# liu-wei2021/IV_INTERPOLATION

Measured on AMD Instinct MI355X. Metric: IV surfaces/sec (1M-batch, 64x16 grid), higher is better.
Workload: dtype f64

## Files before the change

### include/ivs.h

```cpp
#ifndef IVS_H
#define IVS_H

#include <stddef.h>
#include <stdint.h>

#ifdef __cplusplus
extern "C" {
#endif

#define IVS_ABI_VERSION 5

enum {
    IVS_LINEAR      = 0,
    IVS_CUBIC       = 1,
    IVS_CUBICSPLINE = 2,
    IVS_SLINEAR     = 3,
    IVS_NEAREST     = 4,
    IVS_ZERO        = 5,
    IVS_PCHIP       = 6,
    IVS_AKIMA       = 7,
    IVS_FROM_DERIVATIVES = 8,
    IVS_QUADRATIC   = 9,
    IVS_BARYCENTRIC = 10,
    IVS_KROGH       = 11,
    IVS_PAD         = 12,
    IVS_BFILL       = 13
};
#define IVS_POLY_MAX_KNOTS 32

enum {
    IVS_OK            = 0,
    IVS_EINVAL        = -22,
    IVS_ERANGE        = -34,
    IVS_ENOMEM        = -12,
    IVS_ELAUNCH       = -5
};

enum {
    IVS_ST_OK            = 0,
    IVS_ST_TOO_FEW_KNOTS = 1,
    IVS_ST_BAD_SHAPE     = 2,
    IVS_ST_ILL_CONDITIONED = 4
};

int         ivs_version(void);
const char* ivs_last_error(void);
int         ivs_device_count(void);

size_t ivs_interp1d_workspace_bytes(int64_t total_knots, int64_t n_series, int32_t n_channels);
int ivs_interp1d_batch_f64(const double* xk, const double* yk, int64_t yk_stride, const int64_t* knot_off,
                           int64_t n_series, int32_t n_channels, int64_t total_knots,
                           const double* xq, const int64_t* q_off, int64_t total_queries,
                           double* out, int64_t out_stride, int32_t* status, int32_t method,
                           void* workspace, size_t workspace_bytes, void* stream);

int ivs_interp1d_greeks_batch_f64(const double* xk, const double* yk, int64_t yk_stride, const int64_t* knot_off,
                                  int64_t n_series, int32_t n_channels, int64_t total_knots,
                                  const double* xq, const int64_t* q_off, int64_t total_queries,
                                  double* out, int64_t out_stride, int32_t* status, int32_t method,
                                  int32_t ch_iv, int32_t ch_underlying, int32_t ch_ttm,
                                  const int32_t* fill_idx, int64_t fill_stride, int32_t row_strike, int32_t row_rate,
                                  int32_t row_callput, const double* strike_src, const double* rate_src,
                                  const uint8_t* is_put_src, double* greeks, int64_t greeks_stride,
                                  void* workspace, size_t workspace_bytes, void* stream);

int ivs_ffill_index_batch(const int64_t* src_pos, const int64_t* src_off, const uint8_t* valid, int64_t valid_stride,
                          int32_t n_cols, const int64_t* q_off, int64_t n_series, int64_t total_queries,
                          int32_t* idx_out, int64_t out_stride, void* stream);

int ivs_gather_rows_f64(const double* src, int64_t src_stride, const int32_t* idx, int64_t idx_stride, const int32_t* idx_row,
                        int32_t n_cols, int64_t n, double* out, int64_t out_stride, void* stream);
int ivs_gather_rows_i32(const int32_t* src, int64_t src_stride, const int32_t* idx, int64_t idx_stride, const int32_t* idx_row,
                        int32_t n_cols, int64_t n, int32_t* out, int64_t out_stride, void* stream);

int ivs_frame_rows(const int64_t* q_off, int64_t n_series, int64_t total_queries, const int64_t* first_ns,
                   const double* chan, int64_t chan_stride, int32_t n_channels, const int32_t* sym_code,
                   const int32_t* status, const uint8_t* needs, int64_t* date_ns, uint8_t* keep, void* stream);

typedef struct ivs_frame_args {
    const int64_t* src_pos; const int64_t* src_off; const int64_t* q_off;
    int64_t n_series, total_src, total_queries;
    const double* yk; int64_t yk_stride; int32_t n_channels; int32_t method;
    double* chan_out; int64_t chan_stride; int32_t* status;
    const uint8_t* valid; int64_t valid_stride; int32_t n_valid;
    const double* fsrc; int64_t fsrc_stride; const int32_t* f_rows; int32_t n_f; double* f_out; int64_t f_stride;
    const int32_t* csrc; int64_t csrc_stride; const int32_t* c_rows; int32_t n_c; int32_t* c_out; int64_t c_stride;
    const int32_t* idx_rows; int32_t n_idx; int32_t* idx_out; int64_t idx_stride;
    const int64_t* first_ns; const uint8_t* needs; int32_t sym_col; int64_t* date_ns; uint8_t* keep;
    int32_t g_strike, g_rate, g_put; const double* strike_src; const double* rate_src; const uint8_t* put_src;
    int32_t ch_iv, ch_underlying, ch_ttm; double* greeks; int64_t greeks_stride;
} ivs_frame_args;
size_t ivs_frame_workspace_bytes(int64_t total_src, int64_t n_series, int32_t n_channels);
int ivs_frame_columns_f64(const ivs_frame_args* args , void* workspace, size_t workspace_bytes, void* stream);

enum { IVS_FLAG_FORCE_GENERIC = 1, IVS_FLAG_ONE_PASS = 2  };
#define IVS_FLAG_MAP_GROUPS(n) (((n) & 0xff) << 8)
size_t ivs_surface_workspace_bytes(int64_t B, int32_t ragged);
int ivs_surface_batch_f64(const double* K, const int64_t* k_off, int64_t k_stride, int32_t nK,
                          const double* T, int64_t t_stride, int32_t nT,
                          const double* sigma, int64_t B,
                          const double* Kq, int64_t kq_stride, int32_t mK,
                          const double* Tq, int64_t tq_stride, int32_t mT,
                          double* out, int32_t* status, int32_t method, int32_t flags,
                          void* workspace, size_t workspace_bytes, void* stream);

typedef struct ivs_snapshot_args {
    const int64_t* date_ns; const double* iv; const double* underlying; int64_t n_rows;
    const int64_t* row_off; int64_t n_contracts;
    const int32_t* cells; const double* strike; const int64_t* expiry_ns; int32_t nT, nK;
    int64_t t0_ns, n_snapshots;
    const double* moneyness; int32_t mK; double kq_empty;
    double* sigma; double* T; double* spot; int32_t* quotes; double* Kq;
} ivs_snapshot_args;
int ivs_snapshot_assemble_f64(const ivs_snapshot_args* args , void* workspace, size_t workspace_bytes, void* stream);

enum {
    IVS_SM_OK          = 0,
    IVS_SM_NO_CROSSING = 1,
    IVS_SM_AMBIGUOUS   = 2,
    IVS_SM_DEAD        = 4
};
typedef struct ivs_smile_args {
    const double* vol;
    const double* Kq; int64_t kq_stride;
    const double* Tq; int64_t tq_stride;
    const double* spot; double rate;
    const double* z;
    int32_t mK, mT, nD; int64_t B;
    double* q_vol; double* q_strike; int32_t* q_flags;
    int32_t rows_per_wave;
} ivs_smile_args;
int ivs_smile_delta_points_f64(const ivs_smile_args* args , void* workspace, size_t workspace_bytes, void* stream);

int ivs_bs_greeks_f64(const double* S, const double* K, const double* T, const double* r, const double* sigma,
                      const uint8_t* is_put, int32_t default_is_put, int64_t n, double* delta, double* gamma,
                      double* theta, double* vega, double* rho, void* stream);

int ivs_candle_aggregate_f64(const int64_t* ts_ns, const double* open, const double* high, const double* low,
                             const double* close, const double* volume, const int64_t* series_off, int64_t n_series,
                             int64_t n_rows, int64_t freq_ns, int64_t* out_ts, double* out_open, double* out_high,
                             double* out_low, double* out_close, double* out_volume, int32_t* out_count, void* stream);

size_t  ivs_bridge_workspace_bytes(int64_t total_rows);
int     ivs_mt19937_words_u32(uint32_t seed, uint32_t* words, int64_t n_words, void* stream);
int     ivs_bridge_candles_f64(const double* price, const double* volume, const int64_t* row_off, int64_t S,
                               int64_t total_rows, int32_t strategy, double base_spread_pct, double vol_factor,
                               const uint32_t* words, int64_t n_words, double* out, uint8_t* valid, int64_t* rng_tail,
                               void* workspace, size_t workspace_bytes, void* stream);

const char* ivs_last_kernel(void);

int     ivs_debug_stamps(void* device_buf, int64_t n_u64);
int64_t ivs_debug_last_grid(void);
int64_t ivs_debug_mode_offset(void);

#ifdef __cplusplus
}
#endif
#endif
```

### iv_interpolation_amd/_lib.py

```python
from __future__ import annotations

import ctypes as C
import os

LIB_PATH = os.path.join(os.path.dirname(os.path.abspath(__file__)), "libivs.so")

LINEAR, CUBIC, CUBICSPLINE, SLINEAR = 0, 1, 2, 3
ST_OK, ST_TOO_FEW_KNOTS, ST_BAD_SHAPE, ST_ILL_CONDITIONED = 0, 1, 2, 4
SM_OK, SM_NO_CROSSING, SM_AMBIGUOUS, SM_DEAD = 0, 1, 2, 4
SM_MAX_TARGETS = 16
FLAG_FORCE_GENERIC = 1
FLAG_ONE_PASS = 2


def flag_map_groups(n: int) -> int:
    return (int(n) & 0xff) << 8

ABI_VERSION = 5

NEAREST, ZERO, PCHIP, AKIMA, FROM_DERIVATIVES = 4, 5, 6, 7, 8
QUADRATIC = 9
BARYCENTRIC, KROGH = 10, 11
PAD, BFILL = 12, 13
POLY_MAX_KNOTS = 32
METHOD_CODES = {"linear": LINEAR, "index": LINEAR, "values": LINEAR,
                "cubic": CUBIC, "cubicspline": CUBICSPLINE, "slinear": SLINEAR,
                "nearest": NEAREST, "zero": ZERO, "pchip": PCHIP, "akima": AKIMA,
                "from_derivatives": FROM_DERIVATIVES, "piecewise_polynomial": FROM_DERIVATIVES, "quadratic": QUADRATIC,
                "barycentric": BARYCENTRIC, "krogh": KROGH,
                "pad": PAD, "ffill": PAD, "bfill": BFILL, "backfill": BFILL}


def method_code(name) -> int:
    if name in METHOD_CODES:
        return METHOD_CODES[name]
    if isinstance(name, str) and name.lower() in ("pad", "ffill", "bfill", "backfill"):
        return METHOD_CODES[name.lower()]
    raise KeyError(name)


class EngineUnavailable(RuntimeError):
    """libivs.so missing / not loadable / no MI355X visible.  Never swallowed by the host code."""


class EngineError(RuntimeError):
    """A C-ABI call returned a negative code."""


_p = C.c_void_p
_i64, _i32, _sz = C.c_int64, C.c_int32, C.c_size_t



class FrameArgs(C.Structure):
    _fields_ = [("src_pos", _p), ("src_off", _p), ("q_off", _p),
                ("n_series", _i64), ("total_src", _i64), ("total_queries", _i64),
                ("yk", _p), ("yk_stride", _i64), ("n_channels", _i32), ("method", _i32),
                ("chan_out", _p), ("chan_stride", _i64), ("status", _p),
                ("valid", _p), ("valid_stride", _i64), ("n_valid", _i32),
                ("fsrc", _p), ("fsrc_stride", _i64), ("f_rows", _p), ("n_f", _i32), ("f_out", _p), ("f_stride", _i64),
                ("csrc", _p), ("csrc_stride", _i64), ("c_rows", _p), ("n_c", _i32), ("c_out", _p), ("c_stride", _i64),
                ("idx_rows", _p), ("n_idx", _i32), ("idx_out", _p), ("idx_stride", _i64),
                ("first_ns", _p), ("needs", _p), ("sym_col", _i32), ("date_ns", _p), ("keep", _p),
                ("g_strike", _i32), ("g_rate", _i32), ("g_put", _i32), ("strike_src", _p), ("rate_src", _p), ("put_src", _p),
                ("ch_iv", _i32), ("ch_underlying", _i32), ("ch_ttm", _i32), ("greeks", _p), ("greeks_stride", _i64)]


class SnapshotArgs(C.Structure):
    _fields_ = [("date_ns", _p), ("iv", _p), ("underlying", _p), ("n_rows", _i64),
                ("row_off", _p), ("n_contracts", _i64),
                ("cells", _p), ("strike", _p), ("expiry_ns", _p), ("nT", _i32), ("nK", _i32),
                ("t0_ns", _i64), ("n_snapshots", _i64),
                ("moneyness", _p), ("mK", _i32), ("kq_empty", C.c_double),
                ("sigma", _p), ("T", _p), ("spot", _p), ("quotes", _p), ("Kq", _p)]


class SmileArgs(C.Structure):
    _fields_ = [("vol", _p), ("Kq", _p), ("kq_stride", _i64), ("Tq", _p), ("tq_stride", _i64),
                ("spot", _p), ("rate", C.c_double), ("z", C.POINTER(C.c_double)),
                ("mK", _i32), ("mT", _i32), ("nD", _i32), ("B", _i64),
                ("q_vol", _p), ("q_strike", _p), ("q_flags", _p), ("rows_per_wave", _i32)]


SIGNATURES = {
    "ivs_version": (C.c_int, []),
    "ivs_last_error": (C.c_char_p, []),
    "ivs_last_kernel": (C.c_char_p, []),
    "ivs_device_count": (C.c_int, []),
    "ivs_interp1d_workspace_bytes": (_sz, [_i64, _i64, _i32]),
    "ivs_interp1d_batch_f64": (C.c_int, [_p, _p, _i64, _p, _i64, _i32, _i64, _p, _p, _i64, _p, _i64, _p, _i32,
                                         _p, _sz, _p]),
    "ivs_interp1d_greeks_batch_f64": (C.c_int, [_p, _p, _i64, _p, _i64, _i32, _i64, _p, _p, _i64, _p, _i64, _p, _i32,
                                                _i32, _i32, _i32, _p, _i64, _i32, _i32, _i32, _p, _p, _p, _p, _i64,
                                                _p, _sz, _p]),
    "ivs_ffill_index_batch": (C.c_int, [_p, _p, _p, _i64, _i32, _p, _i64, _i64, _p, _i64, _p]),
    "ivs_gather_rows_f64": (C.c_int, [_p, _i64, _p, _i64, _p, _i32, _i64, _p, _i64, _p]),
    "ivs_gather_rows_i32": (C.c_int, [_p, _i64, _p, _i64, _p, _i32, _i64, _p, _i64, _p]),
    "ivs_frame_rows": (C.c_int, [_p, _i64, _i64, _p, _p, _i64, _i32, _p, _p, _p, _p, _p, _p]),
    "ivs_frame_workspace_bytes": (_sz, [_i64, _i64, _i32]),
    "ivs_frame_columns_f64": (C.c_int, [C.POINTER(FrameArgs), _p, _sz, _p]),
    "ivs_bs_greeks_f64": (C.c_int, [_p, _p, _p, _p, _p, _p, _i32, _i64, _p, _p, _p, _p, _p, _p]),
    "ivs_candle_aggregate_f64": (C.c_int, [_p] * 7 + [_i64, _i64, _i64] + [_p] * 8),
    "ivs_bridge_workspace_bytes": (C.c_size_t, [_i64]),
    "ivs_mt19937_words_u32": (C.c_int, [C.c_uint32, _p, _i64, _p]),
    "ivs_bridge_candles_f64": (C.c_int, [_p, _p, _p, _i64, _i64, _i32, C.c_double, C.c_double, _p, _i64, _p, _p, _p,
                                         _p, C.c_size_t, _p]),
    "ivs_debug_stamps": (C.c_int, [_p, _i64]),
    "ivs_debug_last_grid": (_i64, []),
    "ivs_debug_mode_offset": (_i64, []),
    "ivs_surface_workspace_bytes": (_sz, [_i64, _i32]),
    "ivs_snapshot_assemble_f64": (C.c_int, [C.POINTER(SnapshotArgs), _p, _sz, _p]),
    "ivs_smile_delta_points_f64": (C.c_int, [C.POINTER(SmileArgs), _p, _sz, _p]),
    "ivs_surface_batch_f64": (C.c_int, [_p, _p, _i64, _i32, _p, _i64, _i32, _p, _i64, _p, _i64, _i32, _p, _i64, _i32,
                                        _p, _p, _i32, _i32, _p, _sz, _p]),
}

_lib = None


def load():
    global _lib
    if _lib is not None:
        return _lib
    if not os.path.exists(LIB_PATH):
        raise EngineUnavailable(
            f"{LIB_PATH} not found: build it with `python -c 'import __graft_entry__ as g; g.build()'` "
            "(hipcc --offload-arch=gfx950). There is no CPU fallback.")
    try:
        import torch
    except ImportError:
        pass
    try:
        lib = C.CDLL(LIB_PATH)
    except OSError as e:
        raise EngineUnavailable(f"cannot load {LIB_PATH}: {e}") from e
    for name, (res, args) in SIGNATURES.items():
        try:
            fn = getattr(lib, name)
        except AttributeError as e:
            raise EngineUnavailable(f"{LIB_PATH} does not export {name}") from e
        fn.restype = res
        fn.argtypes = args
    if lib.ivs_version() != ABI_VERSION:
        raise EngineUnavailable(f"libivs.so ABI {lib.ivs_version()} != expected {ABI_VERSION}")
    _lib = lib
    return lib


def check(rc: int, what: str):
    if rc != 0:
        raise EngineError(f"{what} failed ({rc}): {load().ivs_last_error().decode()}")
```

### iv_interpolation_amd/csrc/ivs_api.hip

```cpp
#include <hip/hip_runtime.h>

#include <atomic>
#include <cstdarg>
#include <cstdio>
#include <cstring>

#include "../../include/ivs.h"
#include "ivs_bridge.hpp"
#include "ivs_candles.hpp"
#include "ivs_interp1d.hpp"
#include "ivs_frame.hpp"
#include "ivs_smile.hpp"
#include "ivs_snapshot.hpp"
#include "ivs_surface_dense.hpp"
#include "ivs_surface_dense_var2.hpp"
#include "ivs_surface_pass.hpp"
#include "ivs_surface_generic.hpp"

namespace {

thread_local char g_err[512] = "";
thread_local const char* g_last_kernel = "";
thread_local unsigned long long* g_stamp_buf = nullptr;
thread_local int64_t g_stamp_cap = 0;
thread_local int64_t g_last_grid = 0;

int fail(int code, const char* fmt, ...) {
    va_list ap;
    va_start(ap, fmt);
    vsnprintf(g_err, sizeof(g_err), fmt, ap);
    va_end(ap);
    return code;
}

int check_launch(const char* what) {
    hipError_t e = hipGetLastError();
    if (e != hipSuccess) return fail(IVS_ELAUNCH, "%s: %s", what, hipGetErrorString(e));
    return IVS_OK;
}

bool valid_method(int m) { return m >= IVS_LINEAR && m <= IVS_BFILL; }

std::atomic<int> g_cu[ivs::IVS_MAX_DEV];
void current_device(int& dev, int& cus) {
    dev = 0;
    if (hipGetDevice(&dev) != hipSuccess) { (void)hipGetLastError(); dev = 0; }
    const bool cached = dev >= 0 && dev < ivs::IVS_MAX_DEV;
    cus = cached ? g_cu[dev].load(std::memory_order_relaxed) : 0;
    if (cus <= 0) {
        int v = 0;
        if (hipDeviceGetAttribute(&v, hipDeviceAttributeMultiprocessorCount, dev) != hipSuccess) { (void)hipGetLastError(); v = 0; }
        cus = v > 0 ? v : 256;
        if (cached) g_cu[dev].store(cus, std::memory_order_relaxed);
    }
}
int num_cu() { int d, c; current_device(d, c); return c; }

}

extern "C" {

int ivs_version(void) { return IVS_ABI_VERSION; }

const char* ivs_last_error(void) { return g_err; }

const char* ivs_last_kernel(void) { return g_last_kernel; }

int ivs_debug_stamps(void* device_buf, int64_t n_u64) {
    g_stamp_buf = static_cast<unsigned long long*>(device_buf);
    g_stamp_cap = device_buf ? n_u64 : 0;
    return (int)ivs::D_NSTAMP;
}

int64_t ivs_debug_last_grid(void) { return g_last_grid; }
int64_t ivs_debug_mode_offset(void) { return (int64_t)offsetof(ivs::TqShared, mode); }

int ivs_device_count(void) {
    int n = 0;
    if (hipGetDeviceCount(&n) != hipSuccess) { (void)hipGetLastError(); return 0; }
    return n;
}

size_t ivs_interp1d_workspace_bytes(int64_t total_knots, int64_t n_series, int32_t n_channels) {
    if (total_knots < 0 || n_series < 0 || n_channels < 0) return 0;
    return ivs::interp1d_ws_bytes(total_knots, n_series, n_channels);
}

namespace {
int interp1d_impl(const char* fn, const double* xk, const double* yk, int64_t yk_stride, const int64_t* knot_off,
                  int64_t n_series, int32_t n_channels, int64_t total_knots, const double* xq, const int64_t* q_off,
                  int64_t total_queries, double* out, int64_t out_stride, int32_t* status, int32_t method, void* workspace,
                  size_t workspace_bytes, void* stream, ivs::Interp1dParams& p) {
    g_err[0] = 0;
    if (!valid_method(method)) return fail(IVS_EINVAL, "%s: unknown method %d", fn, method);
    if (n_series < 0 || n_channels < 0 || total_knots < 0 || total_queries < 0) return fail(IVS_EINVAL, "%s: negative size", fn);
    if (n_series == 0 || n_channels == 0) return IVS_OK;
    if (!knot_off || !q_off || !status) return fail(IVS_EINVAL, "%s: null offsets/status", fn);
    if (total_knots > 0 && (!xk || !yk)) return fail(IVS_EINVAL, "%s: null knots", fn);
    if (total_queries > 0 && !out) return fail(IVS_EINVAL, "%s: null out", fn);
    if (yk_stride < total_knots || out_stride < total_queries)
        return fail(IVS_EINVAL, "%s: channel stride smaller than row length", fn);
    if (n_series * (int64_t)n_channels > 0x7fffffffLL || (total_queries + 255) / 256 > 0x7fffffffLL)
        return fail(IVS_ERANGE, "%s: batch too large for one launch", fn);
    size_t need = ivs::interp1d_ws_bytes(total_knots, n_series, n_channels);
    if (!workspace || workspace_bytes < need) return fail(IVS_ENOMEM, "%s: workspace %zu < %zu bytes", fn, workspace_bytes, need);
    p.xk = xk; p.yk = yk; p.yk_stride = yk_stride; p.knot_off = knot_off;
    p.S = n_series; p.C = n_channels; p.total_knots = total_knots;
    p.xq = xq; p.q_off = q_off; p.total_q = total_queries;
    p.out = out; p.out_stride = out_stride; p.status = status; p.method = method;
    double* w = static_cast<double*>(workspace);
    size_t plane = (size_t)n_channels * (size_t)total_knots;
    p.wx = w; p.wy = w + plane; p.ws = w + 2 * plane; p.wcp = w + 3 * plane;
    p.wn = reinterpret_cast<int32_t*>(w + 4 * plane);
    hipStream_t st = static_cast<hipStream_t>(stream);
    hipLaunchKernelGGL(ivs::interp1d_prepare_kernel, dim3((unsigned)(n_series * n_channels)), dim3(256), 0, st, p);
    int rc = check_launch("interp1d_prepare_kernel");
    if (rc) return rc;
    if (total_queries > 0) {
        hipLaunchKernelGGL(ivs::interp1d_eval_kernel, dim3((unsigned)((total_queries + ivs::E1_ROWS - 1) / ivs::E1_ROWS)), dim3(256), 0, st, p);
        rc = check_launch("interp1d_eval_kernel");
    }
    return rc;
}
}

int ivs_interp1d_batch_f64(const double* xk, const double* yk, int64_t yk_stride, const int64_t* knot_off,
                           int64_t n_series, int32_t n_channels, int64_t total_knots,
                           const double* xq, const int64_t* q_off, int64_t total_queries,
                           double* out, int64_t out_stride, int32_t* status, int32_t method,
                           void* workspace, size_t workspace_bytes, void* stream) {
    ivs::Interp1dParams p{};
    p.greeks = nullptr;
    return interp1d_impl("ivs_interp1d_batch_f64", xk, yk, yk_stride, knot_off, n_series, n_channels, total_knots, xq, q_off,
                         total_queries, out, out_stride, status, method, workspace, workspace_bytes, stream, p);
}

int ivs_interp1d_greeks_batch_f64(const double* xk, const double* yk, int64_t yk_stride, const int64_t* knot_off,
                                  int64_t n_series, int32_t n_channels, int64_t total_knots,
                                  const double* xq, const int64_t* q_off, int64_t total_queries,
                                  double* out, int64_t out_stride, int32_t* status, int32_t method,
                                  int32_t ch_iv, int32_t ch_underlying, int32_t ch_ttm,
                                  const int32_t* fill_idx, int64_t fill_stride, int32_t row_strike, int32_t row_rate,
                                  int32_t row_callput, const double* strike_src, const double* rate_src,
                                  const uint8_t* is_put_src, double* greeks, int64_t greeks_stride,
                                  void* workspace, size_t workspace_bytes, void* stream) {
    const char* fn = "ivs_interp1d_greeks_batch_f64";
    g_err[0] = 0;
    if (n_series > 0 && n_channels > 0 && total_queries > 0) {
        if (!greeks || greeks_stride < total_queries) return fail(IVS_EINVAL, "%s: null / short greeks output", fn);
        if (ch_iv < 0 || ch_iv >= n_channels || ch_underlying < 0 || ch_underlying >= n_channels || ch_ttm < 0 || ch_ttm >= n_channels)
            return fail(IVS_EINVAL, "%s: channel numbers outside [0, %d)", fn, n_channels);
        if ((row_strike >= 0 || row_rate >= 0 || row_callput >= 0) && (!fill_idx || fill_stride < total_queries))
            return fail(IVS_EINVAL, "%s: null / short fill index", fn);
        if ((row_strike >= 0 && !strike_src) || (row_rate >= 0 && !rate_src) || (row_callput >= 0 && !is_put_src))
            return fail(IVS_EINVAL, "%s: a present column needs its source array", fn);
    }
    ivs::Interp1dParams p{};
    p.fidx = fill_idx; p.fidx_stride = fill_stride; p.fi_strike = row_strike; p.fi_rate = row_rate; p.fi_put = row_callput;
    p.strike_src = strike_src; p.rate_src = rate_src; p.put_src = is_put_src;
    p.ch_iv = ch_iv; p.ch_S = ch_underlying; p.ch_T = ch_ttm;
    p.greeks = greeks; p.greeks_stride = greeks_stride;
    return interp1d_impl(fn, xk, yk, yk_stride, knot_off, n_series, n_channels, total_knots, xq, q_off, total_queries, out,
                         out_stride, status, method, workspace, workspace_bytes, stream, p);
}

int ivs_ffill_index_batch(const int64_t* src_pos, const int64_t* src_off, const uint8_t* valid, int64_t valid_stride,
                          int32_t n_cols, const int64_t* q_off, int64_t n_series, int64_t total_queries,
                          int32_t* idx_out, int64_t out_stride, void* stream) {
    g_err[0] = 0;
    if (n_cols < 0 || n_series < 0 || total_queries < 0) return fail(IVS_EINVAL, "ivs_ffill_index_batch: negative size");
    if (n_cols == 0 || n_series == 0 || total_queries == 0) return IVS_OK;
    if (!src_pos || !src_off || !valid || !q_off || !idx_out) return fail(IVS_EINVAL, "ivs_ffill_index_batch: null pointer");
    if (out_stride < total_queries) return fail(IVS_EINVAL, "ivs_ffill_index_batch: out_stride < total_queries");
    if ((total_queries + 255) / 256 > 0x7fffffffLL) return fail(IVS_ERANGE, "ivs_ffill_index_batch: too many rows");
    if (valid_stride > 0x7fffffffLL) return fail(IVS_ERANGE, "ivs_ffill_index_batch: %lld source rows exceed the int32 gather index", (long long)valid_stride);
    ivs::FfillParams p{src_pos, src_off, valid, valid_stride, n_cols, q_off, n_series, total_queries, idx_out, out_stride};
    hipLaunchKernelGGL(ivs::ffill_index_kernel, dim3((unsigned)((total_queries + ivs::F1_ROWS - 1) / ivs::F1_ROWS)), dim3(256), 0,
                       static_cast<hipStream_t>(stream), p);
    return check_launch("ffill_index_kernel");
}

extern "C++" {
namespace {
template <class T>
int gather_impl(const char* fn, const void* src, int64_t src_stride, const int32_t* idx, int64_t idx_stride, const int32_t* idx_row,
                int32_t n_cols, int64_t n, void* out, int64_t out_stride, T missing, void* stream) {
    g_err[0] = 0;
    if (n_cols < 0 || n < 0) return fail(IVS_EINVAL, "%s: negative size", fn);
    if (n_cols == 0 || n == 0) return IVS_OK;
    if (!src || !idx || !idx_row || !out) return fail(IVS_EINVAL, "%s: null pointer", fn);
    if (idx_stride < n || out_stride < n) return fail(IVS_EINVAL, "%s: stride smaller than row count", fn);
    if (src_stride > 0x7fffffffLL) return fail(IVS_ERANGE, "%s: %lld source rows exceed the int32 gather index", fn, (long long)src_stride);
    ivs::GatherParams p{src, src_stride, idx, idx_stride, idx_row, n_cols, n, out, out_stride};
    int64_t blocks = (n + 255) / 256;
    const int64_t cap = (int64_t)num_cu() * 16;
    if (blocks > cap) blocks = cap;
    hipLaunchKernelGGL(ivs::gather_rows_kernel<T>, dim3((unsigned)blocks), dim3(256), 0, static_cast<hipStream_t>(stream), p, missing);
    return check_launch(fn);
}
}
}

int ivs_gather_rows_f64(const double* src, int64_t src_stride, const int32_t* idx, int64_t idx_stride, const int32_t* idx_row,
                        int32_t n_cols, int64_t n, double* out, int64_t out_stride, void* stream) {
    return gather_impl<double>("ivs_gather_rows_f64", src, src_stride, idx, idx_stride, idx_row, n_cols, n, out, out_stride,
                               __builtin_nan(""), stream);
}

int ivs_gather_rows_i32(const int32_t* src, int64_t src_stride, const int32_t* idx, int64_t idx_stride, const int32_t* idx_row,
                        int32_t n_cols, int64_t n, int32_t* out, int64_t out_stride, void* stream) {
    return gather_impl<int32_t>("ivs_gather_rows_i32", src, src_stride, idx, idx_stride, idx_row, n_cols, n, out, out_stride,
                                (int32_t)-1, stream);
}

int ivs_frame_rows(const int64_t* q_off, int64_t n_series, int64_t total_queries, const int64_t* first_ns,
                   const double* chan, int64_t chan_stride, int32_t n_channels, const int32_t* sym_code,
                   const int32_t* status, const uint8_t* needs, int64_t* date_ns, uint8_t* keep, void* stream) {
    g_err[0] = 0;
    if (n_series < 0 || total_queries < 0 || n_channels < 0) return fail(IVS_EINVAL, "ivs_frame_rows: negative size");
// ... 140 lines not shown

int ivs_smile_delta_points_f64(const ivs_smile_args* a, void* workspace, size_t workspace_bytes, void* stream) {
    const char* fn = "ivs_smile_delta_points_f64";
    (void)workspace; (void)workspace_bytes;
    g_err[0] = 0;
    g_last_kernel = "";
    if (!a) return fail(IVS_EINVAL, "%s: null args", fn);
    if (a->B < 0 || a->mT < 0 || a->mK < 0 || a->kq_stride < 0 || a->tq_stride < 0) return fail(IVS_EINVAL, "%s: negative size", fn);
    if (a->nD < 1 || a->nD > ivs::SM_MAX_D) return fail(IVS_ERANGE, "%s: nD=%d outside [1,%d]", fn, a->nD, ivs::SM_MAX_D);
    if (a->mK < 2) return fail(IVS_ERANGE, "%s: mK=%d < 2: a bracket needs two nodes", fn, a->mK);
    if (a->rows_per_wave < 0 || a->rows_per_wave > 64 / a->nD)
        return fail(IVS_ERANGE, "%s: rows_per_wave=%d outside [0,%d] for nD=%d", fn, a->rows_per_wave, 64 / a->nD, a->nD);
    if (a->B == 0 || a->mT == 0) return IVS_OK;
    if (!a->vol || !a->Kq || !a->Tq || !a->spot || !a->z || !a->q_vol || !a->q_strike || !a->q_flags)
        return fail(IVS_EINVAL, "%s: null pointer", fn);
    if ((a->kq_stride != 0 && a->kq_stride < a->mK) || (a->tq_stride != 0 && a->tq_stride < a->mT))
        return fail(IVS_EINVAL, "%s: grid stride smaller than the grid", fn);
    if (a->B > 0x7fffffffLL / a->mT)
        return fail(IVS_ERANGE, "%s: %lld x %d rows exceed one launch", fn, (long long)a->B, a->mT);
    ivs::SmileParams p{};
    p.vol = a->vol; p.Kq = a->Kq; p.Tq = a->Tq; p.spot = a->spot;
    p.kq_stride = a->kq_stride; p.tq_stride = a->tq_stride; p.rate = a->rate;
    for (int t = 0; t < a->nD; ++t) p.z[t] = a->z[t];
    p.mK = a->mK; p.mT = a->mT; p.nD = a->nD; p.rows = a->B * a->mT;
    p.q_vol = a->q_vol; p.q_strike = a->q_strike; p.q_flags = a->q_flags;
    int dev, cus;
    current_device(dev, cus);
    int64_t group = p.rows / ((int64_t)cus * 16);
    group = group < 1 ? 1 : (group > 64 / a->nD ? 64 / a->nD : group);
    if (a->rows_per_wave > 0) group = a->rows_per_wave;
    p.group = (int32_t)group;
    const int64_t waves = (p.rows + group - 1) / group;
    hipLaunchKernelGGL(ivs::smile_delta_kernel, dim3((unsigned)((waves + ivs::SM_WAVES - 1) / ivs::SM_WAVES)),
                       dim3(ivs::SM_WAVES * 64), 0, static_cast<hipStream_t>(stream), p);
    g_last_kernel = "smile_delta_kernel";
    return check_launch("smile_delta_kernel");
}

int ivs_candle_aggregate_f64(const int64_t* ts_ns, const double* open, const double* high, const double* low,
                             const double* close, const double* volume, const int64_t* series_off, int64_t n_series,
                             int64_t n_rows, int64_t freq_ns, int64_t* out_ts, double* out_open, double* out_high,
                             double* out_low, double* out_close, double* out_volume, int32_t* out_count, void* stream) {
    g_err[0] = 0;
    if (n_rows < 0 || n_series < 0 || freq_ns <= 0) return fail(IVS_EINVAL, "ivs_candle_aggregate_f64: bad size / frequency");
    if (n_rows == 0 || n_series == 0) return IVS_OK;
    if (!ts_ns || !open || !high || !low || !close || !volume || !series_off || !out_ts || !out_open || !out_high ||
        !out_low || !out_close || !out_volume || !out_count)
        return fail(IVS_EINVAL, "ivs_candle_aggregate_f64: null pointer");
    if ((n_rows + 255) / 256 > 0x7fffffffLL) return fail(IVS_ERANGE, "ivs_candle_aggregate_f64: too many rows");
    ivs::CandleParams p{ts_ns, open, high, low, close, volume, series_off, n_series, n_rows, freq_ns,
                        out_ts, out_open, out_high, out_low, out_close, out_volume, out_count};
    hipLaunchKernelGGL(ivs::candle_kernel, dim3((unsigned)((n_rows + 255) / 256)), dim3(256), 0,
                       static_cast<hipStream_t>(stream), p);
    return check_launch("candle_kernel");
}

size_t ivs_bridge_workspace_bytes(int64_t total_rows) { return ivs::bridge_ws_bytes(total_rows < 0 ? 0 : total_rows); }

int ivs_mt19937_words_u32(uint32_t seed, uint32_t* words, int64_t n_words, void* stream) {
    g_err[0] = 0;
    if (n_words < 0) return fail(IVS_EINVAL, "ivs_mt19937_words_u32: negative size");
    if (n_words == 0) return IVS_OK;
    if (!words) return fail(IVS_EINVAL, "ivs_mt19937_words_u32: null pointer");
    hipLaunchKernelGGL(ivs::mt19937_words_kernel, dim3(1), dim3(ivs::MT_THREADS), 0, static_cast<hipStream_t>(stream), seed, words, n_words);
    return check_launch("mt19937_words_kernel");
}

int ivs_bridge_candles_f64(const double* price, const double* volume, const int64_t* row_off, int64_t S,
                           int64_t total_rows, int32_t strategy, double base_spread_pct, double vol_factor,
                           const uint32_t* words, int64_t n_words, double* out, uint8_t* valid, int64_t* rng_tail,
                           void* workspace, size_t workspace_bytes, void* stream) {
    g_err[0] = 0;
    if (S < 0 || total_rows < 0 || n_words < 0) return fail(IVS_EINVAL, "ivs_bridge_candles_f64: negative size");
    if (strategy < 0 || strategy > 4) return fail(IVS_EINVAL, "ivs_bridge_candles_f64: unknown strategy %d", strategy);
    if (!rng_tail) return fail(IVS_EINVAL, "ivs_bridge_candles_f64: null rng_tail");
    hipStream_t st = static_cast<hipStream_t>(stream);
    if (S == 0 || total_rows == 0) {
        if (hipMemsetAsync(rng_tail, 0, 8, st) != hipSuccess || hipMemsetAsync(rng_tail + 3, 0, 8, st) != hipSuccess)
            return fail(IVS_ELAUNCH, "ivs_bridge_candles_f64: memset failed");
        return IVS_OK;
    }
    if (!price || !row_off || !words || !out || !valid || !workspace)
        return fail(IVS_EINVAL, "ivs_bridge_candles_f64: null pointer");
    if (workspace_bytes < ivs::bridge_ws_bytes(total_rows)) return fail(IVS_ENOMEM, "ivs_bridge_candles_f64: workspace too small");
    const int64_t nb = ivs::bridge_blocks(total_rows);
    if (nb > 0x7fffffffLL) return fail(IVS_ERANGE, "ivs_bridge_candles_f64: too many rows");
    if (n_words > 0x7fffffffLL) return fail(IVS_ERANGE, "ivs_bridge_candles_f64: %lld words exceed the int32 per-row stream offsets", (long long)n_words);
    auto align64 = [](uintptr_t a) { return (a + 63) & ~(uintptr_t)63; };
    uintptr_t w = align64(reinterpret_cast<uintptr_t>(workspace));
    ivs::BridgeParams p;
    p.price = price; p.volume = volume; p.row_off = row_off; p.S = S; p.total_rows = total_rows;
    p.strategy = strategy; p.base_spread_pct = base_spread_pct; p.vol_factor = vol_factor;
    p.words = words; p.n_words = n_words; p.out = out; p.valid = valid; p.rng_tail = rng_tail;
    p.woff = reinterpret_cast<int32_t*>(w); w = align64(w + (size_t)total_rows * 4);
    p.bbase = reinterpret_cast<int64_t*>(w); w = align64(w + (size_t)(nb + 1) * 8);
    p.gauss = reinterpret_cast<double*>(w); w = align64(w + (size_t)total_rows * 8);
    p.expu = reinterpret_cast<double*>(w); w = align64(w + (size_t)total_rows * 8);
    p.acc = reinterpret_cast<uint8_t*>(w); w = align64(w + ivs::bridge_acc_capacity(total_rows));
    p.gauss0 = reinterpret_cast<double*>(w);
    if (hipMemsetAsync(rng_tail + 3, 0, 8, st) != hipSuccess) return fail(IVS_ELAUNCH, "ivs_bridge_candles_f64: memset failed");
    if (strategy == ivs::BR_TREND) {
        int64_t nd = n_words / 2;
        const int64_t cap = (int64_t)ivs::bridge_acc_capacity(total_rows);
        if (nd > cap) { nd = cap; p.n_words = 2 * nd; }
        int64_t ab = (nd + 255) / 256;
        const int64_t abcap = (int64_t)num_cu() * 16;
        if (ab > abcap) ab = abcap;
        if (ab < 1) ab = 1;
        hipLaunchKernelGGL(ivs::bridge_accept_kernel, dim3((unsigned)ab), dim3(256), 0, st, p, nd);
        hipLaunchKernelGGL(ivs::bridge_gauss_walk_kernel, dim3(1), dim3(64), 0, st, p, nd);
    } else {
        hipLaunchKernelGGL(ivs::bridge_count_kernel, dim3((unsigned)nb), dim3(256), 0, st, p);
        hipLaunchKernelGGL(ivs::bridge_scan_blocks_kernel, dim3(1), dim3(256), 0, st, p, nb);
    }
    int64_t grid = (int64_t)num_cu() * 8;
    if (grid > S) grid = S;
    switch (strategy) {
        case ivs::BR_SPREAD: hipLaunchKernelGGL(ivs::bridge_candles_kernel<ivs::BR_SPREAD>, dim3((unsigned)grid), dim3(64), 0, st, p); break;
        case ivs::BR_MIDPOINT: hipLaunchKernelGGL(ivs::bridge_candles_kernel<ivs::BR_MIDPOINT>, dim3((unsigned)grid), dim3(64), 0, st, p); break;
        case ivs::BR_TREND: hipLaunchKernelGGL(ivs::bridge_candles_kernel<ivs::BR_TREND>, dim3((unsigned)grid), dim3(64), 0, st, p); break;
        case ivs::BR_PIPELINE: hipLaunchKernelGGL(ivs::bridge_candles_kernel<ivs::BR_PIPELINE>, dim3((unsigned)grid), dim3(64), 0, st, p); break;
        default: hipLaunchKernelGGL(ivs::bridge_candles_kernel<ivs::BR_SIMPLE>, dim3((unsigned)grid), dim3(64), 0, st, p); break;
    }
    return check_launch("bridge_candles_kernel");
}

int ivs_bs_greeks_f64(const double* S, const double* K, const double* T, const double* r, const double* sigma,
                      const uint8_t* is_put, int32_t default_is_put, int64_t n, double* delta, double* gamma,
                      double* theta, double* vega, double* rho, void* stream) {
    g_err[0] = 0;
    if (n < 0) return fail(IVS_EINVAL, "ivs_bs_greeks_f64: negative size");
    if (n == 0) return IVS_OK;
    if (!S || !K || !T || !r || !sigma || !delta || !gamma || !theta || !vega || !rho)
        return fail(IVS_EINVAL, "ivs_bs_greeks_f64: null pointer");
    ivs::GreeksParams p{S, K, T, r, sigma, is_put, default_is_put, n, delta, gamma, theta, vega, rho};
    int64_t blocks = (n + 255) / 256;
    int64_t cap = (int64_t)num_cu() * 16;
    if (blocks > cap) blocks = cap;
    hipLaunchKernelGGL(ivs::greeks_kernel, dim3((unsigned)blocks), dim3(256), 0, static_cast<hipStream_t>(stream), p);
    return check_launch("greeks_kernel");
}

size_t ivs_surface_workspace_bytes(int64_t B, int32_t ragged) { return ivs::surface_ws_bytes(B, ragged != 0); }

int ivs_surface_batch_f64(const double* K, const int64_t* k_off, int64_t k_stride, int32_t nK,
                          const double* T, int64_t t_stride, int32_t nT,
                          const double* sigma, int64_t B,
                          const double* Kq, int64_t kq_stride, int32_t mK,
                          const double* Tq, int64_t tq_stride, int32_t mT,
                          double* out, int32_t* status, int32_t method, int32_t flags,
                          void* workspace, size_t workspace_bytes, void* stream) {
    g_err[0] = 0;
    g_last_kernel = "";
    if (!valid_method(method)) return fail(IVS_EINVAL, "ivs_surface_batch_f64: unknown method %d", method);
    if (ivs::method_is_poly(method)) return fail(IVS_EINVAL, "ivs_surface_batch_f64: method %d ('barycentric' / 'krogh') is 1-D only", method);
    if (B < 0 || nK < 0 || nT < 0 || mK < 0 || mT < 0) return fail(IVS_EINVAL, "ivs_surface_batch_f64: negative size");
    if (B == 0 || mK == 0 || mT == 0) return IVS_OK;
    if (!K || !T || !sigma || !Kq || !Tq || !out) return fail(IVS_EINVAL, "ivs_surface_batch_f64: null pointer");
    if (nT < 1 || nT > ivs::GEN_NTMAX) return fail(IVS_ERANGE, "ivs_surface_batch_f64: nT=%d outside [1,%d]", nT, ivs::GEN_NTMAX);
    if (nK < 1) return fail(IVS_ERANGE, "ivs_surface_batch_f64: nK=%d < 1", nK);
    if (!k_off && k_stride != 0 && k_stride < nK) return fail(IVS_EINVAL, "ivs_surface_batch_f64: k_stride < nK");
    if (t_stride < 0 || kq_stride < 0 || tq_stride < 0 || k_stride < 0)
        return fail(IVS_EINVAL, "ivs_surface_batch_f64: negative stride");
    if (ivs::generic_lds_bytes(nK, nT, ivs::method_is_cubic(method)) > 160 * 1024)
        return fail(IVS_ERANGE, "ivs_surface_batch_f64: nK=%d x nT=%d needs %zu B of LDS (> 160 KiB)", nK, nT,
                    ivs::generic_lds_bytes(nK, nT, ivs::method_is_cubic(method)));
    const size_t need = ivs::surface_ws_bytes(B, k_off != nullptr);
    if (!workspace || workspace_bytes < need)
        return fail(IVS_ENOMEM, "ivs_surface_batch_f64: workspace %zu < %zu bytes (ivs_surface_workspace_bytes)",
                    workspace ? workspace_bytes : (size_t)0, need);
    if (reinterpret_cast<uintptr_t>(workspace) & 255)
        return fail(IVS_EINVAL, "ivs_surface_batch_f64: workspace must be 256-byte aligned");

    ivs::SurfaceParams p;
    p.K = K; p.k_off = k_off; p.k_stride = k_off ? 0 : k_stride; p.nK = nK; p.k_total = k_off ? k_stride : 0;
    p.T = T; p.t_stride = t_stride; p.nT = nT;
    p.sigma = sigma; p.B = B; p.map_groups = 1; p.tqs = nullptr; p.redo = nullptr; p.queue = nullptr; p.mode = nullptr;
    p.Kq = Kq; p.kq_stride = kq_stride; p.mK = mK;
    p.Tq = Tq; p.tq_stride = tq_stride; p.mT = mT;
    p.out = out; p.status = status; p.method = method;
    ivs::LaunchCtx cx;
    current_device(cx.dev, cx.num_cu);
    cx.st = static_cast<hipStream_t>(stream);
    cx.ws = static_cast<unsigned char*>(workspace);
    cx.ws_bytes = workspace_bytes;
    cx.map_groups = (flags >> 8) & 0xff;

    if (!(flags & IVS_FLAG_FORCE_GENERIC)) {
        const char* name = nullptr;
        int64_t need_blocks = (int64_t)cx.num_cu * 8;
        unsigned long long* dbg = (g_stamp_buf && g_stamp_cap >= need_blocks * ivs::D_NSTAMP) ? g_stamp_buf : nullptr;
        int rc = (dbg || (flags & IVS_FLAG_ONE_PASS)) ? 0 : ivs::launch_surface_pass(p, cx, &name);
        if (rc == 1) {
            g_last_kernel = name;
            return check_launch(name);
        }
        if (rc < 0) return fail(IVS_ELAUNCH, "ivs_surface_batch_f64: row-pass dispatch failed");
        rc = ivs::launch_surface_dense(p, cx, &name, dbg, &g_last_grid);
        if (rc == 1) {
            g_last_kernel = name;
            return check_launch(name);
        }
        if (rc < 0) return fail(IVS_ELAUNCH, "ivs_surface_batch_f64: dense dispatch failed");
        if (!g_stamp_buf) {
            rc = ivs::launch_surface_dense_var(p, cx, &name);
            if (rc == 1) {
                g_last_kernel = name;
                return check_launch(name);
            }
            if (rc < 0) return fail(IVS_ELAUNCH, "ivs_surface_batch_f64: dense-var dispatch failed");
        }
    }

    if (!ivs::launch_surface_generic<false>(p, cx))
        return fail(IVS_ERANGE, "ivs_surface_batch_f64: nK=%d x nT=%d needs %zu B of LDS (> 160 KiB)", nK, nT,
                    ivs::generic_lds_bytes(nK, nT, ivs::method_is_cubic(method)));
    g_last_kernel = "surface_generic_kernel";
    return check_launch("surface_generic_kernel");
}

}
```

### iv_interpolation_amd/csrc/ivs_device.hpp

```cpp
#pragma once
#include <hip/hip_runtime.h>
#include <stdint.h>

#include "../../include/ivs.h"

namespace ivs {

constexpr int WAVE = 64;

__device__ __forceinline__ double qnan() { return __builtin_nan(""); }

template <class XA>
__device__ __forceinline__ int find_interval(const XA& x, int n, double xq) {
    int lo = 0, hi = n;
    while (lo < hi) {
        int mid = (lo + hi) >> 1;
        if (x(mid) <= xq) lo = mid + 1; else hi = mid;
    }
    return lo - 1;
}

__device__ __forceinline__ double lerp_np(double xq, double x0, double y0, double x1, double y1) {
#pragma clang fp contract(off)
    if (x0 == xq) return y0;
    double slope = (y1 - y0) / (x1 - x0);
    double r = slope * (xq - x0) + y0;
    if (__builtin_isnan(r)) {
        r = slope * (xq - x1) + y1;
        if (__builtin_isnan(r) && y0 == y1) r = y0;
    }
    return r;
}

template <class XA, class YA>
__device__ __forceinline__ double eval_linear(const XA& x, const YA& y, int n, int j, double xq, bool right_hold) {
    if (j < 0) return qnan();
    if (j >= n - 1) return (right_hold || xq == x(n - 1)) ? y(n - 1) : qnan();
    return lerp_np(xq, x(j), y(j), x(j + 1), y(j + 1));
}

__device__ __forceinline__ double refined_rcp(double b) {
    double y = __builtin_amdgcn_rcp(b);
    double e = __builtin_fma(-b, y, 1.0);
    y = __builtin_fma(y, e, y);
    e = __builtin_fma(-b, y, 1.0);
    return __builtin_fma(y, e, y);
}

template <class XA, class YA, class SA>
__device__ __forceinline__ double eval_linear_slopes(const XA& x, const YA& y, const SA& slope, int n, int j, double xq,
                                                     bool right_hold) {
#pragma clang fp contract(off)
    if (j < 0) return qnan();
    if (j >= n - 1) return (right_hold || xq == x(n - 1)) ? y(n - 1) : qnan();
    const double x0 = x(j), y0 = y(j);
    if (x0 == xq) return y0;
    const double sl = slope(j);
    double r = sl * (xq - x0) + y0;
    if (__builtin_isnan(r)) {
        r = sl * (xq - x(j + 1)) + y(j + 1);
        if (__builtin_isnan(r) && y0 == y(j + 1)) r = y0;
    }
    return r;
}

__device__ __forceinline__ double hermite_eval(double x0, double x1, double y0, double y1, double s0, double s1, double xq) {
    double h = x1 - x0;
    double rh = refined_rcp(h);
    double delta = (y1 - y0) * rh;
    double t = (s0 + s1 - 2.0 * delta) * rh;
    double c0 = t * rh;
    double c1 = (delta - s0) * rh - t;
    double u = xq - x0;
    return ((c0 * u + c1) * u + s0) * u + y0;
}
template <class XA, class YA, class SA>
__device__ __forceinline__ double eval_cubic(const XA& x, const YA& y, const SA& s, int n, int j, double xq,
                                             bool extrapolate_right) {
    if (j < 0) return qnan();
    if (!extrapolate_right && !(xq <= x(n - 1))) return qnan();
    int jj = j > n - 2 ? n - 2 : j;
    return hermite_eval(x(jj), x(jj + 1), y(jj), y(jj + 1), s(jj), s(jj + 1), xq);
}

template <class XA, class YA, class SW, class CW>
__device__ __forceinline__ void nak_slopes(const XA& x, const YA& y, SW& s, CW& cp, int n) {
    if (n == 2) {
        double d = (y(1) - y(0)) / (x(1) - x(0));
        s.set(0, d); s.set(1, d);
        return;
    }
    if (n == 3) {
        double dx0 = x(1) - x(0), dx1 = x(2) - x(1);
        double d0 = (y(1) - y(0)) / dx0, d1 = (y(2) - y(1)) / dx1;
        double b0 = 2.0 * d0, b1 = 3.0 * (dx0 * d1 + dx1 * d0), b2 = 2.0 * d1;
        double s1 = (b1 - dx1 * b0 - dx0 * b2) / (2.0 * (dx0 + dx1) - dx1 - dx0);
        s.set(0, b0 - s1); s.set(1, s1); s.set(2, b2 - s1);
        return;
    }
    double xm = x(0), xc = x(1), xp = x(2);
    double ym = y(0), yc = y(1), yp = y(2);
    double dxm = xc - xm, dxc = xp - xc;
    double dlm = (yc - ym) * refined_rcp(dxm), dlc = (yp - yc) * refined_rcp(dxc);
    double d = xp - xm;
    double rhs = ((dxm + 2.0 * d) * dxc * dlm + dxm * dxm * dlc) * refined_rcp(d);
    const double rdx1 = refined_rcp(dxc);
    double cprev = d * rdx1;
    double dprev = rhs * rdx1;
    cp.set(0, cprev); s.set(0, dprev);
    for (int i = 1; i <= n - 2; ++i) {
        rhs = 3.0 * (dxc * dlm + dxm * dlc);
        const double rw = refined_rcp(2.0 * (dxm + dxc) - dxc * cprev);
        cprev = dxm * rw;
        dprev = (rhs - dxc * dprev) * rw;
        cp.set(i, cprev); s.set(i, dprev);
        if (i < n - 2) {
            xm = xc; xc = xp; xp = x(i + 2);
            ym = yc; yc = yp; yp = y(i + 2);
            dxm = dxc; dxc = xp - xc;
            dlm = dlc; dlc = (yp - yc) * refined_rcp(dxc);
        }
    }
    d = xp - xm;
    rhs = (dxc * dxc * dlm + (2.0 * d + dxc) * dxm * dlc) * refined_rcp(d);
    dprev = (rhs - d * dprev) * refined_rcp(dxm - d * cprev);
    double sn = dprev;
    s.set(n - 1, sn);
    for (int i = n - 2; i >= 0; --i) {
        sn = s(i) - cp(i) * sn;
        s.set(i, sn);
    }
}

struct View {
    double* p; int stride;
    __device__ __forceinline__ double operator()(int i) const { return p[i * stride]; }
    __device__ __forceinline__ void set(int i, double v) { p[i * stride] = v; }
};
struct CView {
    const double* p; int stride;
    __device__ __forceinline__ double operator()(int i) const { return p[i * stride]; }
};

__host__ __device__ __forceinline__ bool method_is_cubic(int m) {
    return m == IVS_CUBIC || m == IVS_CUBICSPLINE || m == IVS_PCHIP || m == IVS_AKIMA || m == IVS_QUADRATIC;
}
__device__ __forceinline__ bool method_extrapolates_right(int m) { return m == IVS_CUBICSPLINE || m == IVS_PCHIP; }
__host__ __device__ __forceinline__ bool method_is_poly(int m) { return m == IVS_BARYCENTRIC || m == IVS_KROGH; }
__device__ __forceinline__ int method_min_knots(int m) {
    switch (m) {
        case IVS_LINEAR: case IVS_PAD: case IVS_BFILL: return 0;
        case IVS_CUBIC: return 4;
        case IVS_NEAREST: case IVS_ZERO: case IVS_BARYCENTRIC: case IVS_KROGH: return 1;
        case IVS_AKIMA: return 3;
        case IVS_QUADRATIC: return 3;
        default: return 2;
    }
}

// ... 206 lines not shown
```

### iv_interpolation_amd/csrc/ivs_surface_dense.hpp

```cpp
#pragma once
#include <atomic>
#include <cstddef>
#include <cstdlib>

#include "ivs_surface_generic.hpp"

namespace ivs {

#ifndef IVS_ABLATE
#define IVS_ABLATE 0
#endif
constexpr int ABL = IVS_ABLATE;

constexpr int DK = 64, DT = 16;
constexpr int D_RS = 72;
constexpr int D_MAX_MT = 64;
constexpr unsigned long long D_SENTINEL = REDO_SENTINEL;

__device__ __forceinline__ int d_sl(int k) { return (k >> 4) * 18 + (k & 15); }

constexpr int D_WLDS_MAX_MT = 16;
__host__ __device__ inline size_t dense_lds_bytes(int mT) {
    return (size_t)(2 * DT * D_RS + 64 + 64 + 64 + (mT <= D_WLDS_MAX_MT ? 4 * D_WLDS_MAX_MT : 0)) * 8;
}
// ... 689 lines not shown
                __builtin_amdgcn_sched_barrier(0);
            }
#pragma unroll
            for (int h = 1; h >= 0; --h) {
                double cp[8];
#pragma unroll
                for (int u = 0; u < 8; ++u) cp[u] = cCP[8 * h + u];
#pragma unroll
                for (int u = 7; u >= 0; --u) { const int i = 8 * h + u; if (i <= DT - 2) s[i] = s[i] - cp[u] * s[i + 1]; }
                __builtin_amdgcn_sched_barrier(0);
            }
        } else {
            constexpr int LA = 4;
            double2 tpq[4], tac[4];
#pragma unroll
            for (int i = 0; i < LA; ++i) {
                tpq[i] = *reinterpret_cast<const double2*>(TT + i * 4);
                tac[i] = *reinterpret_cast<const double2*>(TT + i * 4 + 2);
            }
            double cpv[DT];
#pragma unroll
            for (int i = 0; i < DT; ++i) {
                const double2 pq = tpq[i & 3], ac = tac[i & 3];
                __builtin_amdgcn_sched_barrier(0);
                if (i + LA < DT) {
                    tpq[i & 3] = *reinterpret_cast<const double2*>(TT + (i + LA) * 4);
                    tac[i & 3] = *reinterpret_cast<const double2*>(TT + (i + LA) * 4 + 2);
                }
                if (!NTR) {
                    const int ia = i == 0 ? 0 : (i == DT - 1 ? DT - 3 : i - 1), ib = i == 0 ? 1 : (i == DT - 1 ? DT - 2 : i);
                    const double dA = z[ia + 1] - z[ia], dB = z[ib + 1] - z[ib];
                    prev = (pq.x * dA + pq.y * dB) - ac.x * prev;
                } else {
                    const int ia = i == 0 ? 0 : i - 1, ib = i == 0 ? 1 : (i == DT - 1 ? DT - 2 : i);
                    const double dA = z[ia + 1] - z[ia], dB = z[ib + 1] - z[ib];
                    double r = pq.x * dA + pq.y * dB;
                    if (i >= 3) r += ((i == nT - 1) ? pm_last : 0.0) * (z[i - 1] - z[i - 2]);
                    prev = r - ac.x * prev;
                }
                s[i] = prev;
                cpv[i] = ac.y;
                __builtin_amdgcn_sched_barrier(0);
            }
#pragma unroll
            for (int i = DT - 2; i >= 0; --i) s[i] = s[i] - cpv[i] * s[i + 1];
        }
        stamp(4);
#pragma unroll
        for (int jv = 0; jv < DT - 1; ++jv) {
            for (int c = 0, n = n_iv(jv); c < n; ++c, adv()) {
                if (!mine(tq)) continue;
                double a0, a1, a2, a3;
                weights(tq, a0, a1, a2, a3);
                if (QUAD) put(tq, a0 * s[jv > 0 ? jv - 1 : 0] + a1 * s[jv] + a2 * s[jv + 1] + a3 * s[jv + 2 < DT ? jv + 2 : DT - 1]);
                else put(tq, a0 * z[jv] + a1 * z[jv + 1] + a2 * s[jv] + a3 * s[jv + 1]);
            }
        }
    } else {
#pragma unroll
        for (int jv = 0; jv < DT - 1; ++jv) {
            if (!WLDS) {
#pragma clang fp contract(off)
                const int n = n_iv(jv);
                if (n == 0) continue;
                double2 tj, tr;
                if (SM) { tj = double2{cTT[jv * 4], cTT[jv * 4 + 1]}; tr = double2{cTT[jv * 4 + 2], cTT[jv * 4 + 3]}; }
                else { tj = *reinterpret_cast<const double2*>(TT + jv * 4); tr = *reinterpret_cast<const double2*>(TT + jv * 4 + 2); }
                const double a = z[jv + 1] - z[jv];
                const double q = a * tr.x;
                const double rem = __builtin_fma(-q, tr.y, a);
                const double slope = __builtin_fma(rem, tr.x, q);
                const double aa = __builtin_fabs(a);
                const bool slow_iv = !div_safe(tr.y) || !((a == 0.0) || (aa >= 0x1p-500 && aa <= 0x1p500));
                for (int c = 0; c < n; ++c, adv()) {
                    if (!mine(tq)) continue;
                    const double xt = SM ? wp[0] : readlane_f64(tt.w0, tq);
                    const double res = slope * (xt - tj.x) + z[jv];
                    const bool slow = slow_iv || __builtin_isnan(res);
                    double r = (tj.x == xt) ? z[jv] : res;
                    if (__builtin_expect(__ballot(slow) != 0ull, 0)) {
                        if (slow) r = lerp_np(xt, tj.x, z[jv], tj.y, z[jv + 1]);
                    }
                    put(tq, r);
                }
                continue;
            }
            for (int c = 0, n = n_iv(jv); c < n; ++c, adv()) {
                if (!mine(tq)) continue;
                double xt, t0, t1, rdt;
                weights(tq, xt, t0, t1, rdt);
                if (d_is_step(METHOD)) { put(tq, step_eval<METHOD>(xt, t0, t1, z[jv], z[jv + 1])); continue; }
                const double dt = t1 - t0;
                bool slow = !div_safe(dt);
                double r = lerp_fast(xt, t0, z[jv], z[jv + 1], dt, rdt, slow);
                if (__builtin_expect(__ballot(slow) != 0ull, 0)) {
                    if (slow) r = lerp_np(xt, t0, z[jv], t1, z[jv + 1]);
                }
                put(tq, r);
            }
        }
    }
    double z_last = z[DT - 1];
    if (NTR) {
#pragma unroll
        for (int i = 3; i < DT - 1; ++i) {
            z_last = (i == nT - 1) ? z[i] : z_last;
            asm volatile("" : "+v"(z_last));
        }
    }
    for (int c = 0; c < tt.n_hold; ++c, adv()) if (mine(tq)) put(tq, z_last);
    for (int c = 0; c < tt.n_nan; ++c, adv()) if (mine(tq)) put(tq, nanv);
}

template <int METHOD, bool NTR>
__global__ __launch_bounds__(64) void tq_tables_kernel(SurfaceParams p, TqShared* o) {
    __shared__ __attribute__((aligned(16))) double sm[8 * 72 + 64 + 64];
    const int lane = threadIdx.x;
    double* scratch = sm;
    double* Tsh = sm + 8 * 72;
    double* TT = Tsh + 64;
    TqTables tt;
    const bool probe = !NTR && !p.k_off && p.nK == DK && p.mK <= 64 && p.B >= 4096;
    double q[64];
    if (probe) {
#pragma unroll
        for (int s = 0; s < 64; ++s) q[s] = p.sigma[(int64_t)s * (p.B / 64) * (int64_t)(DT * DK) + (s & (DT - 1)) * DK + lane];
    }
    dense_t_phase<METHOD, false, NTR>(p.T, p.Tq, p.mT, lane, Tsh, TT, nullptr, tt, p.nT, scratch);
    if (lane < DT) {
#pragma unroll
        for (int c = 0; c < 4; ++c) o->TT[lane * 4 + c] = TT[lane * 4 + c];
        o->CP[lane] = TT[lane * 4 + 3]; o->PP[lane] = TT[lane * 4]; o->QQ[lane] = TT[lane * 4 + 1]; o->AL[lane] = TT[lane * 4 + 2];
    }
    if (lane < p.mT) { o->W[lane * 4] = tt.w0; o->W[lane * 4 + 1] = tt.w1; o->W[lane * 4 + 2] = tt.w2; o->W[lane * 4 + 3] = tt.w3; }
    int mode = 0;
    if (probe) {
        int hit = 0, tot = 0;
#pragma unroll
        for (int s = 0; s < 64; ++s) {
            const int c = __popcll(__ballot(__builtin_isnan(q[s])));
            hit += c != 0 ? 1 : 0; tot += c;
        }
        mode = (hit >= 32 || (hit >= 5 && 2 * tot <= 3 * hit)) ? 1 : 0;
    }
    if (lane == 0) {
        o->pm_last = tt.pm_last; o->iv_lo = tt.iv_lo; o->iv_hi = tt.iv_hi;
        o->n_left = tt.n_left; o->n_hold = tt.n_hold; o->n_nan = tt.n_nan; o->unsorted = tt.unsorted;
        o->redo[0] = 0; o->redo[1] = 0; o->mode = mode;
    }
    if (lane < 24) o->queue[lane * QUEUE_STRIDE] = 0ull;
}
template <bool NTR>
inline void launch_tq_tables(const SurfaceParams& p, TqShared* o, hipStream_t st) {
#define IVS_TQ_CASE(M) case M: hipLaunchKernelGGL((tq_tables_kernel<M, NTR>), dim3(1), dim3(64), 0, st, p, o); break;
    switch (p.method) {
        IVS_TQ_CASE(IVS_LINEAR) IVS_TQ_CASE(IVS_CUBIC) IVS_TQ_CASE(IVS_CUBICSPLINE) IVS_TQ_CASE(IVS_SLINEAR)
        IVS_TQ_CASE(IVS_PCHIP) IVS_TQ_CASE(IVS_AKIMA) IVS_TQ_CASE(IVS_NEAREST) IVS_TQ_CASE(IVS_ZERO) IVS_TQ_CASE(IVS_FROM_DERIVATIVES)
        IVS_TQ_CASE(IVS_QUADRATIC)
        default: break;
    }
#undef IVS_TQ_CASE
}
__device__ __forceinline__ void tq_from_shared(const void* tqs, TqTables& tt, const double*& TT, const double*& W) {
    const TqShared* g = static_cast<const TqShared*>(tqs);
    const TqShared IVS_CONST* c = (const TqShared IVS_CONST*)g;
    tt.w0 = tt.w1 = tt.w2 = tt.w3 = 0.0;
    tt.pm_last = c->pm_last; tt.iv_lo = c->iv_lo; tt.iv_hi = c->iv_hi;
    tt.n_left = c->n_left; tt.n_hold = c->n_hold; tt.n_nan = c->n_nan; tt.unsorted = c->unsorted;
    TT = g->TT; W = g->W;
}

template <int METHOD, bool TSHARED, bool WLDS, bool STAMP = false>
__global__ __launch_bounds__(64, 2) void surface_dense_kernel(SurfaceParams p, unsigned long long* dbg = nullptr) {
    if (TSHARED && p.mode && *((const int IVS_CONST*)p.mode)) return;
    constexpr bool CUB = d_is_hermite(METHOD);
    unsigned long long acc[D_NSTAMP] = {0, 0, 0, 0, 0, 0, 0, 0};
    unsigned long long tprev = 0;
    auto stamp = [&](int i) {
        if (STAMP) {
            __builtin_amdgcn_sched_barrier(0);
            unsigned long long tn = __builtin_amdgcn_s_memtime();
            __builtin_amdgcn_s_waitcnt(0xC07F);
            if (i >= 0) acc[i] += tn - tprev;
            tprev = tn;
            __builtin_amdgcn_sched_barrier(0);
        }
    };
    extern __shared__ __attribute__((aligned(16))) unsigned char smem[];
    const int lane = threadIdx.x;
    const int mT = p.mT, mK = p.mK;
    double* Y = reinterpret_cast<double*>(smem);
    double* S = Y + DT * D_RS;
    double* Ksh = S + DT * D_RS;
    double* RDX = Ksh + 64;
    double* TT = RDX + 64;
    double* W = TT + 64;
    double* Tsh = TSHARED ? Y : S;

    constexpr bool t_shared = TSHARED;
    const double nanv = __builtin_nan("");

    TqTables tt;
    auto t_phase = [&](const double* Tb, const double* Tqb) { dense_t_phase<METHOD, WLDS>(Tb, Tqb, mT, lane, Tsh, TT, W, tt); };
    const double* TTp = TT;
    const double* Wp = W;
    if (t_shared) tq_from_shared(p.tqs, tt, TTp, Wp);

    double2 pre[8];
    double pre_k;
    auto prefetch = [&](int64_t b) {
        const double2* s2 = reinterpret_cast<const double2*>(p.sigma + b * (int64_t)(DT * DK));
#pragma unroll
        for (int i = 0; i < 8; ++i) pre[i] = s2[i * 64 + lane];
        pre_k = p.K[b * p.k_stride + lane];
    };
    constexpr int XQ_REG = 4;
    double xq_reg[XQ_REG];
    auto load_xq = [&](const double* Kqb) {
#pragma unroll
        for (int i = 0; i < XQ_REG; ++i) xq_reg[i] = (i * 64 + lane < mK) ? Kqb[i * 64 + lane] : nanv;
    };
    const bool kq_shared = p.kq_stride == 0;
    if (kq_shared) load_xq(p.Kq);
    bool told = false;
    WorkQueue wq;
    wq.init(p.queue, p.map_groups, p.B, WQ_CHUNK, lane);
    int64_t b = wq.take(), b_next = b >= 0 ? wq.take() : -1;
    if (b >= 0) prefetch(b);

    while (b >= 0) {
        const bool more = b_next >= 0;
        const WorkQueue::Pending pend = wq.begin(more);
        auto advance = [&]() { const int64_t n2 = wq.finish(pend, more); b = b_next; b_next = n2; };
        __syncthreads();
        stamp(-1);
        unsigned long long bad = 0ull;
#pragma unroll
        for (int i = 0; i < 8; ++i) {
            const int t = 2 * i + (lane >> 5), k = 2 * (lane & 31);
            *reinterpret_cast<double2*>(&Y[t * D_RS + d_sl(k)]) = pre[i];
            bad |= __ballot(pre[i].x != pre[i].x) | __ballot(pre[i].y != pre[i].y);
        }
        Ksh[lane] = pre_k;
        double* outb = p.out + b * (int64_t)mT * mK;
        if (!t_shared) t_phase(p.T + b * p.t_stride, p.Tq + b * p.tq_stride);
        if (bad != 0ull || tt.unsorted) {
            if (lane == 0) { reinterpret_cast<unsigned long long*>(outb)[0] = D_SENTINEL; count_redo(p, told); }
            prefetch(more ? b_next : b);
            advance();
            continue;
        }
        __syncthreads();
        stamp(0);
        const double* Kqb = p.Kq + b * p.kq_stride;
        if (!kq_shared) load_xq(Kqb);
        {
            if (ABL != 5) prefetch(more ? b_next : b);
        }
        if (d_is_nak(METHOD) && (ABL == 1 || ABL == 6)) {
            RDX[lane] = 1.0;
            __syncthreads();
        } else if (d_is_nak(METHOD)) {
            dense_strike_slopes<STAMP>(Y, S, Ksh, RDX, lane, stamp);
            __syncthreads();
            stamp(2);
        } else if (d_is_local(METHOD)) {
            dense_strike_slopes_local<METHOD>(Y, S, Ksh, RDX, lane);
            __syncthreads();
            stamp(2);
        }
#pragma unroll 1
        for (int q0 = 0, qb = 0; q0 < mK; q0 += 64, ++qb) {
            const int q = q0 + lane;
            const bool act = q < mK;
            double xq;
            if (qb < XQ_REG) xq = qb == 0 ? xq_reg[0] : (qb == 1 ? xq_reg[1] : (qb == 2 ? xq_reg[2] : xq_reg[3]));
            else xq = act ? Kqb[q] : nanv;
            int j = 0;
#pragma unroll
            for (int m = 1; m < 8; ++m) j += (Ksh[8 * m] <= xq) ? 8 : 0;
#pragma unroll
            for (int st = 4; st >= 1; st >>= 1) if (Ksh[j + st] <= xq) j += st;
            const double xl = Ksh[DK - 1];
            const bool left = !(Ksh[0] <= xq);
            const int jj = j > DK - 2 ? DK - 2 : j;
            const double x0 = Ksh[jj], x1 = Ksh[jj + 1];
            const int o0 = d_sl(jj), o1 = d_sl(jj + 1);
            double z[DT];
            if (ABL == 2 || ABL == 6) {
#pragma unroll
                for (int r = 0; r < DT; ++r) z[r] = Y[r * D_RS + d_sl(lane)] + xq;
            } else if (CUB) {
                const bool ok = !left && ((xq <= xl) || d_extrap_right(METHOD));
                const double u = xq - x0, t = u * RDX[jj], omt = 1.0 - t;
                const double w0 = ok ? (1.0 + 2.0 * t) * omt * omt : nanv;
                const double w1 = t * t * (3.0 - 2.0 * t);
                const double w2 = u * omt * omt;
                const double w3 = u * t * (t - 1.0);
                constexpr int LA = 3;
                double g0[4], g1[4], g2[4], g3[4];
#pragma unroll
                for (int r = 0; r < LA; ++r) {
                    g0[r] = Y[r * D_RS + o0]; g1[r] = Y[r * D_RS + o1]; g2[r] = S[r * D_RS + o0]; g3[r] = S[r * D_RS + o1];
                }
#pragma unroll
                for (int r = 0; r < DT; ++r) {
                    if (r + LA < DT) {
                        const int n = r + LA;
                        g0[n & 3] = Y[n * D_RS + o0]; g1[n & 3] = Y[n * D_RS + o1];
                        g2[n & 3] = S[n * D_RS + o0]; g3[n & 3] = S[n * D_RS + o1];
                    }
                    __builtin_amdgcn_sched_barrier(0);
                    z[r] = w0 * g0[r & 3] + w1 * g1[r & 3] + w2 * g2[r & 3] + w3 * g3[r & 3];
                    __builtin_amdgcn_sched_barrier(0);
                }
            } else {
                const bool right = j >= DK - 1;
                const bool hold = right && (METHOD == IVS_LINEAR || xq == xl);
                const double dx = x1 - x0, rdx = refined_rcp(dx);
                bool slow = !div_safe(dx);
                constexpr int LA = 6;
                double g0[8], g1[8];
#pragma unroll
                for (int r = 0; r < LA; ++r) { g0[r] = Y[r * D_RS + o0]; g1[r] = Y[r * D_RS + o1]; }
#pragma unroll
                for (int r = 0; r < DT; ++r) {
                    if (r + LA < DT) { const int n = r + LA; g0[n & 7] = Y[n * D_RS + o0]; g1[n & 7] = Y[n * D_RS + o1]; }
                    __builtin_amdgcn_sched_barrier(0);
                    const double y0 = g0[r & 7], y1 = g1[r & 7];
                    double v = lerp_fast(xq, x0, y0, y1, dx, rdx, slow);
                    if (right) v = hold ? y1 : nanv;
                    if (left) v = nanv;
                    z[r] = v;
                    __builtin_amdgcn_sched_barrier(0);
                }
                if (__builtin_expect(__ballot(slow && !right && !left) != 0ull, 0)) {
                    if (slow && !right && !left) {
#pragma unroll
                        for (int r = 0; r < DT; ++r) z[r] = lerp_np(xq, x0, Y[r * D_RS + o0], x1, Y[r * D_RS + o1]);
                    }
                }
            }
            stamp(3);
            if (d_is_local(METHOD)) {
#pragma unroll
                for (int r = 0; r < DT; ++r) asm volatile("" : "+v"(z[r]));
            }
            if (act) dense_maturity_pass<METHOD, WLDS, false, false, TSHARED>(z, tt, TTp, Wp, outb, q0, lane, true, mT, mK, stamp);
            stamp(5);
        }
        if (p.status && lane == 0) p.status[b] = IVS_ST_OK;
        if (STAMP) acc[7] += 1;
        advance();
    }
    if (STAMP && dbg && lane == 0) {
#pragma unroll
        for (int i = 0; i < D_NSTAMP; ++i) dbg[(size_t)blockIdx.x * D_NSTAMP + i] = acc[i];
    }
}

struct LaunchCtx {
    int dev = 0, num_cu = 256;
    hipStream_t st = nullptr;
    unsigned char* ws = nullptr;
    size_t ws_bytes = 0;
    int map_groups = 0;
};
constexpr int IVS_MAX_DEV = 64;
constexpr size_t WS_TQ_BYTES = 8192;
constexpr size_t WS_COUNTS_BYTES = 256;
constexpr int V_NCLASS = 4;
static_assert(sizeof(TqShared) <= WS_TQ_BYTES, "TqShared must fit its workspace slot");
inline size_t surface_ws_bytes(int64_t B, bool ragged) {
    return WS_TQ_BYTES + (ragged ? WS_COUNTS_BYTES + (size_t)V_NCLASS * (size_t)(B < 0 ? 0 : B) * 16 : 0);
}

inline void ensure_max_lds(const void* fn, int slot, int dev) {
    static std::atomic<unsigned long long> done[IVS_MAX_DEV];
    const int d = (dev >= 0 && dev < IVS_MAX_DEV) ? dev : 0;
    const unsigned long long bit = 1ull << (slot & 63);
    if (dev < 0 || dev >= IVS_MAX_DEV || !(done[d].load(std::memory_order_relaxed) & bit)) {
        (void)hipFuncSetAttribute(fn, hipFuncAttributeMaxDynamicSharedMemorySize, 160 * 1024);
        done[d].fetch_or(bit, std::memory_order_relaxed);
    }
}

template <bool FILTER>
inline bool launch_surface_generic(const SurfaceParams& p, const LaunchCtx& cx) {
    if (p.nK > 65535) return false;
    const size_t lds = generic_lds_bytes(p.nK, p.nT, method_is_cubic(p.method));
    if (lds > 160 * 1024) return false;
    if (lds > 64 * 1024) ensure_max_lds(reinterpret_cast<const void*>(surface_generic_kernel<FILTER>), FILTER ? 1 : 0, cx.dev);
    int per_cu = (int)((160 * 1024) / lds);
    per_cu = per_cu < 1 ? 1 : (per_cu > 16 ? 16 : per_cu);
    int64_t grid = (int64_t)cx.num_cu * per_cu * 2;
    const int64_t work = FILTER ? (p.B + 63) / 64 : p.B;
    if (grid > work) grid = work;
    hipLaunchKernelGGL(surface_generic_kernel<FILTER>, dim3((unsigned)grid), dim3(64), lds, cx.st, p);
    return true;
}

inline int dense_map_groups(int64_t grid, int64_t B, int forced) {
    int r = forced > 0 ? forced : 8;
    if (r > 16) r = 16;
    while (r > 1 && (B < (int64_t)r * 256 || grid < r)) r >>= 1;
    return r < 1 ? 1 : r;
}

template <bool NTR>
inline bool launch_tq_or_zero_queue(SurfaceParams& p, const LaunchCtx& cx, bool tsh, bool set_mode) {
    TqShared* tq = reinterpret_cast<TqShared*>(cx.ws);
    if (tsh) {
        launch_tq_tables<NTR>(p, tq, cx.st);
        p.tqs = tq;
        p.redo = tq->redo;
        p.mode = set_mode ? &tq->mode : nullptr;
    } else {
        if (hipMemsetAsync(tq->queue, 0, sizeof(TqShared::queue), cx.st) != hipSuccess) return false;
        p.tqs = nullptr;
        p.redo = nullptr;
    }
    p.queue = tq->queue;
    return true;
}

#ifndef IVS_DIAG_MINIMAL
inline bool launch_surface_masked(const SurfaceParams& p, const LaunchCtx& cx);
inline int launch_surface_dense(const SurfaceParams& p_in, const LaunchCtx& cx, const char** name,
                                unsigned long long* dbg = nullptr, int64_t* grid_out = nullptr) {
    SurfaceParams p = p_in;
    hipStream_t st = cx.st;
    if (p.k_off || p.nK != DK || p.nT != DT) return 0;
    if (p.k_stride != 0 && p.k_stride < DK) return 0;
    if (reinterpret_cast<uintptr_t>(p.sigma) & 15) return 0;
    if (p.mT > D_MAX_MT) return 0;
    const size_t lds = dense_lds_bytes(p.mT);
    if (generic_lds_bytes(p.nK, p.nT) > 160 * 1024) return 0;
    int per_cu = (int)((160 * 1024) / lds);
    per_cu = per_cu > 8 ? 8 : per_cu;
    int64_t grid = (int64_t)cx.num_cu * per_cu;
    if (grid > p.B) grid = p.B;
    if (grid_out) *grid_out = grid;
    p.map_groups = dense_map_groups(grid, p.B, cx.map_groups);
    const bool tsh = p.t_stride == 0 && p.tq_stride == 0;
    const bool wl = p.mT <= D_WLDS_MAX_MT;
    if (!launch_tq_or_zero_queue<false>(p, cx, tsh, true)) return -1;
    if (p.map_groups > 16) p.map_groups = 16;
    if (dbg) {
        if (!tsh) return 0;
        if (p.method == IVS_CUBIC) {
            if (wl) hipLaunchKernelGGL((surface_dense_kernel<IVS_CUBIC, true, true, true>), dim3((unsigned)grid), dim3(64), lds, st, p, dbg);
            else hipLaunchKernelGGL((surface_dense_kernel<IVS_CUBIC, true, false, true>), dim3((unsigned)grid), dim3(64), lds, st, p, dbg);
        } else {
            if (wl) hipLaunchKernelGGL((surface_dense_kernel<IVS_LINEAR, true, true, true>), dim3((unsigned)grid), dim3(64), lds, st, p, dbg);
            else hipLaunchKernelGGL((surface_dense_kernel<IVS_LINEAR, true, false, true>), dim3((unsigned)grid), dim3(64), lds, st, p, dbg);
        }
        *name = "surface_dense_kernel<stamp>";
        return hipGetLastError() == hipSuccess ? 1 : -1;
    }
#define IVS_DENSE_CASE(M, NAME)                                                                            \
    case M: {                                                                                              \
        if (tsh && wl) hipLaunchKernelGGL((surface_dense_kernel<M, true, true, false>), dim3((unsigned)grid), dim3(64), lds, st, p, nullptr);        \
        else if (tsh) hipLaunchKernelGGL((surface_dense_kernel<M, true, false, false>), dim3((unsigned)grid), dim3(64), lds, st, p, nullptr);        \
        else if (wl) hipLaunchKernelGGL((surface_dense_kernel<M, false, true, false>), dim3((unsigned)grid), dim3(64), lds, st, p, nullptr);         \
        else hipLaunchKernelGGL((surface_dense_kernel<M, false, false, false>), dim3((unsigned)grid), dim3(64), lds, st, p, nullptr);                \
        *name = NAME;                                                                                      \
        break;                                                                                             \
    }
    switch (p.method) {
        IVS_DENSE_CASE(IVS_LINEAR, "surface_dense_kernel<linear>")
        IVS_DENSE_CASE(IVS_CUBIC, "surface_dense_kernel<cubic>")
        IVS_DENSE_CASE(IVS_CUBICSPLINE, "surface_dense_kernel<cubicspline>")
        IVS_DENSE_CASE(IVS_SLINEAR, "surface_dense_kernel<slinear>")
        IVS_DENSE_CASE(IVS_PCHIP, "surface_dense_kernel<pchip>")
        IVS_DENSE_CASE(IVS_AKIMA, "surface_dense_kernel<akima>")
        default: return 0;
    }
#undef IVS_DENSE_CASE
    if (hipGetLastError() != hipSuccess) return -1;
    if (launch_surface_masked(p, cx) && p.redo) ++p.redo;
    launch_surface_generic<true>(p, cx);
    return 1;
}

#endif

}
```

### iv_interpolation_amd/csrc/ivs_surface_dense_var.hpp

```cpp
#pragma once
#include "ivs_surface_dense.hpp"

namespace ivs {

constexpr int DPP_QUAD_BCAST0 = 0x00, DPP_QUAD_BCAST3 = 0xFF;

template <int NKB>
__host__ __device__ inline size_t dense_var_lds_bytes(int mT) {
    return (size_t)(2 * DT * NKB * 72 + NKB * 64 + NKB * 64 + 64 + (mT <= D_WLDS_MAX_MT ? 4 * D_WLDS_MAX_MT : 0)) * 8;
}

template <int NKB>
__device__ __forceinline__ void factor_tables_var(const double* X, int n, int lane, double* AL, double* CP, double* PP,
                                                  double* QQ, double* PM, double* PI, double* PSI, double* RDX) {
    double c00 = 1.0, c01 = 0.0, c10 = 0.0, c11 = 1.0;
    double carry_crb = 0.0, carry_rdx = 0.0, carry_rdx_prev = 0.0;
#pragma unroll
    for (int blk = 0; blk < NKB; ++blk) {
        const int ir = blk * 64 + lane;
        const bool in = ir < n;
        const int i = in ? ir : n - 1;
        const double x0 = X[i];
        const double xp = X[i + 1 < n ? i + 1 : n - 1];
        const double xpp = X[i + 2 < n ? i + 2 : n - 1];
// ... 378 lines not shown
    };

    double pre[DT * NKB], pre_k[NKB];
    int n = 0, n_next = 0;
    int64_t koff = 0, koff_next = 0;
    auto sigma_of = [&](int64_t b, int64_t ko) -> const double* {
        return p.k_off ? p.sigma + (int64_t)nT * ko : p.sigma + b * (int64_t)nT * p.nK;
    };
    auto issue_loads = [&](int64_t b, int64_t ko, int nn) {
        const double* sb = sigma_of(b, ko);
        const double* Kb = p.K + ko;
#pragma unroll
        for (int t = 0; t < DT; ++t)
#pragma unroll
            for (int blk = 0; blk < NKB; ++blk) {
                const int k = blk * 64 + lane;
                pre[t * NKB + blk] = (t < nT && k < nn) ? sb[(int64_t)t * nn + k] : 0.0;
            }
#pragma unroll
        for (int blk = 0; blk < NKB; ++blk) { const int k = blk * 64 + lane; pre_k[blk] = k < nn ? Kb[k] : inf; }
    };

    WorkQueue wq;
    wq.init(p.queue + list.qslot * 8 * QUEUE_STRIDE, 8, limit, WQ_CHUNK, lane);
    int64_t it = wq.take(), it_next = it >= 0 ? wq.take() : -1, b = 0;
    if (it >= 0) { b = at(it, n, koff); issue_loads(b, koff, n); }

    while (it >= 0) {
        const bool more = it_next >= 0;
        const WorkQueue::Pending pend = wq.begin(more);
        __syncthreads();
        unsigned long long bad = 0ull;
#pragma unroll
        for (int t = 0; t < DT; ++t)
#pragma unroll
            for (int blk = 0; blk < NKB; ++blk) {
                const double v = pre[t * NKB + blk];
                Y[t * RS + d_sl(blk * 64 + lane)] = v;
                bad |= __ballot(v != v);
            }
#pragma unroll
        for (int blk = 0; blk < NKB; ++blk) Ksh[blk * 64 + lane] = pre_k[blk];
        double* outb = p.out + b * (int64_t)mT * mK;
        const double* Kqb = p.Kq + b * p.kq_stride;
        int64_t b_next = 0;
        if (more) b_next = at(it_next, n_next, koff_next);
        if (!TSHARED) dense_t_phase<METHOD, WLDS, true>(p.T + b * p.t_stride, p.Tq + b * p.tq_stride, mT, lane, S + 600, TT, W,
                                                        tt, nT, S);
        const bool redo = bad != 0ull || tt.unsorted;
        if (redo) {
            tag(b);
        } else {
            __syncthreads();
            if (d_is_nak(METHOD)) {
                dense_strike_slopes_var<NKB>(Y, S, Ksh, RDX, n, lane);
                __syncthreads();
            } else if (d_is_local(METHOD)) {
                dense_strike_slopes_local_var<METHOD>(Y, S, Ksh, RDX, n, lane);
                __syncthreads();
            }
            if (!kq_shared) load_xq(Kqb);
        }
        if (more) issue_loads(b_next, koff_next, n_next);
        if (!redo) {
#pragma unroll 1
            for (int q0 = 0, qb = 0; q0 < mK; q0 += 64, ++qb) {
                const int q = q0 + lane;
                const bool act = q < mK;
                double xq;
                if (qb < XQ_REG) xq = qb == 0 ? xq_reg[0] : (qb == 1 ? xq_reg[1] : (qb == 2 ? xq_reg[2] : xq_reg[3]));
                else xq = act ? Kqb[q] : nanv;
                int j = 0;
#pragma unroll
                for (int m = 1; m < 8 * NKB; ++m) j += (Ksh[8 * m] <= xq) ? 8 : 0;
#pragma unroll
                for (int st = 4; st >= 1; st >>= 1) if (Ksh[j + st] <= xq) j += st;
                const double xl = Ksh[n - 1];
                const bool left = !(Ksh[0] <= xq);
                const int jj = j > n - 2 ? n - 2 : j;
                const double x0 = Ksh[jj], x1 = Ksh[jj + 1];
                const int o0 = d_sl(jj), o1 = d_sl(jj + 1);
                double z[DT];
                if (CUB) {
                    const bool ok = !left && ((xq <= xl) || d_extrap_right(METHOD));
                    const double u = xq - x0, t = u * RDX[jj], omt = 1.0 - t;
                    const double w0 = ok ? (1.0 + 2.0 * t) * omt * omt : nanv;
                    const double w1 = t * t * (3.0 - 2.0 * t);
                    const double w2 = u * omt * omt;
                    const double w3 = u * t * (t - 1.0);
                    constexpr int LA = 3;
                    double g0[4], g1[4], g2[4], g3[4];
#pragma unroll
                    for (int r = 0; r < LA; ++r) {
                        g0[r] = Y[r * RS + o0]; g1[r] = Y[r * RS + o1]; g2[r] = S[r * RS + o0]; g3[r] = S[r * RS + o1];
                    }
#pragma unroll
                    for (int r = 0; r < DT; ++r) {
                        if (r + LA < DT) {
                            const int nn = r + LA;
                            g0[nn & 3] = Y[nn * RS + o0]; g1[nn & 3] = Y[nn * RS + o1];
                            g2[nn & 3] = S[nn * RS + o0]; g3[nn & 3] = S[nn * RS + o1];
                        }
                        __builtin_amdgcn_sched_barrier(0);
                        z[r] = w0 * g0[r & 3] + w1 * g1[r & 3] + w2 * g2[r & 3] + w3 * g3[r & 3];
                        __builtin_amdgcn_sched_barrier(0);
                    }
                } else {
                    const bool right = j >= n - 1;
                    const bool hold = right && (METHOD == IVS_LINEAR || xq == xl);
                    const double dx = x1 - x0, rdx = refined_rcp(dx);
                    bool slow = !div_safe(dx);
                    constexpr int LA = 6;
                    double g0[8], g1[8];
#pragma unroll
                    for (int r = 0; r < LA; ++r) { g0[r] = Y[r * RS + o0]; g1[r] = Y[r * RS + o1]; }
#pragma unroll
                    for (int r = 0; r < DT; ++r) {
                        if (r + LA < DT) { const int nn = r + LA; g0[nn & 7] = Y[nn * RS + o0]; g1[nn & 7] = Y[nn * RS + o1]; }
                        __builtin_amdgcn_sched_barrier(0);
                        const double y0 = g0[r & 7], y1 = g1[r & 7];
                        double v = lerp_fast(xq, x0, y0, y1, dx, rdx, slow);
                        if (right) v = hold ? y1 : nanv;
                        if (left) v = nanv;
                        z[r] = v;
                        __builtin_amdgcn_sched_barrier(0);
                    }
                    if (__builtin_expect(__ballot(slow && !right && !left) != 0ull, 0)) {
                        if (slow && !right && !left) {
#pragma unroll
                            for (int r = 0; r < DT; ++r) z[r] = lerp_np(xq, x0, Y[r * RS + o0], x1, Y[r * RS + o1]);
                        }
                    }
                }
                if (d_is_local(METHOD)) {
#pragma unroll
                    for (int r = 0; r < DT; ++r) asm volatile("" : "+v"(z[r]));
                }
                if (act) dense_maturity_pass<METHOD, WLDS, false, true, TSHARED>(z, tt, TTp, Wp, outb, q0, lane, true, mT, mK, nostamp, 0, 0, nT);
            }
            if (p.status && lane == 0) p.status[b] = IVS_ST_OK;
        }
        const int64_t it_next2 = wq.finish(pend, more);
        it = it_next; it_next = it_next2; b = b_next; n = n_next; koff = koff_next;
    }
}

struct VarWork { VarList wl1, wl2; bool need1, need2; };
inline bool var_work_lists(const SurfaceParams& p, const LaunchCtx& cx, VarWork& w) {
    VarItem* lists = nullptr;
    int32_t* counts = nullptr;
    if (p.k_off) {
        counts = reinterpret_cast<int32_t*>(cx.ws + WS_TQ_BYTES);
        lists = reinterpret_cast<VarItem*>(cx.ws + WS_TQ_BYTES + WS_COUNTS_BYTES);
        if (hipMemsetAsync(counts, 0, WS_COUNTS_BYTES, cx.st) != hipSuccess) return false;
        int64_t cb = (p.B + 1023) / 1024;
        const int64_t cap = (int64_t)cx.num_cu * 8;
        if (cb > cap) cb = cap;
        hipLaunchKernelGGL(var_classify_kernel, dim3((unsigned)cb), dim3(256), 0, cx.st, p, lists, lists + p.B, counts);
    }
    w.wl1 = VarList{lists, counts, 0};
    w.wl2 = VarList{lists ? lists + p.B : nullptr, counts ? counts + 1 : nullptr, 1};
    w.need1 = p.k_off ? true : p.nK <= 64;
    w.need2 = p.nK > 64;
    return true;
}

}
```

### iv_interpolation_amd/csrc/ivs_surface_dense_var2.hpp

```cpp
#pragma once
#include <type_traits>

#include "ivs_surface_dense_var.hpp"

namespace ivs {

constexpr int V2_RS = 144;
__device__ __forceinline__ int v2_row(int t) { return t * V2_RS + 8 * (t >> 1); }
constexpr int V2_PLANE = DT * V2_RS + 64;
constexpr int V2_XCH = 64;
constexpr int X_MAT = 0;
constexpr int X_FWD = 8;
constexpr int X_BWD = 24;
constexpr int X_BAD = 40;

__host__ __device__ inline size_t dense_var2_lds_bytes(int mT) {
    return (size_t)(2 * V2_PLANE + 128 + 64 + V2_XCH + (mT <= D_WLDS_MAX_MT ? 4 * D_WLDS_MAX_MT : 0)) * 8;
}

__device__ __forceinline__ void factor_tables_var2(const double* X, int n, int lane, int w, double* AL, double* CP,
                                                   double* PP, double* QQ, double* PM, double* PI, double* PSI,
                                                   double* XCH) {
    const int ir = w * 64 + lane;
    const bool in = ir < n;
// ... 275 lines not shown
        int64_t b_next = 0;
        if (it_next < limit) b_next = at(it_next, n_next, koff_next);
        if (!TSHARED) dense_t_phase<METHOD, WLDS, true>(p.T + b * p.t_stride, p.Tq + b * p.tq_stride, mT, lane, S + 600, TT, W,
                                                        tt, nT, S);
        __syncthreads();
        const bool redo = XCH[X_BAD] != 0.0 || XCH[X_BAD + 1] != 0.0 || tt.unsorted;
        if (redo) {
            tag(b);
        } else {
            if (d_is_nak(METHOD)) {
                dense_strike_slopes_var2(Y, S, Ksh, XCH, n, lane, w);
                __syncthreads();
            } else if (d_is_local(METHOD)) {
                dense_strike_slopes_local_var2<METHOD>(Y, S, Ksh, XCH, n, lane, w);
                __syncthreads();
            }
            if (!kq_shared) load_xq(Kqb);
        }
        if (it_next < limit) issue_loads(b_next, koff_next, n_next);
        if (!redo) {
            const bool split_rows = mK <= 64;
#pragma unroll 1
            for (int q0 = 0, qb = 0; q0 < mK; q0 += 64, ++qb) {
                if (!split_rows && (qb & 1) != w) continue;
                const int q = q0 + lane;
                const bool act = q < mK;
                double xq;
                if (qb < XQ_REG) xq = qb == 0 ? xq_reg[0] : (qb == 1 ? xq_reg[1] : (qb == 2 ? xq_reg[2] : xq_reg[3]));
                else xq = act ? Kqb[q] : nanv;
                int j = 0;
#pragma unroll
                for (int m = 1; m < 16; ++m) j += (Ksh[8 * m] <= xq) ? 8 : 0;
#pragma unroll
                for (int st = 4; st >= 1; st >>= 1) if (Ksh[j + st] <= xq) j += st;
                const double xl = Ksh[n - 1];
                const bool left = !(Ksh[0] <= xq);
                const int jj = j > n - 2 ? n - 2 : j;
                const double x0 = Ksh[jj], x1 = Ksh[jj + 1];
                const int o0 = d_sl(jj), o1 = d_sl(jj + 1);
                const int r_lo = split_rows ? 8 * w : 0;
                double z[DT];
                auto strike_rows = [&](auto NR_TAG, int rbase) {
                    constexpr int NR = decltype(NR_TAG)::value;
                    const double* Yb = Y;
                    const double* Sb = S;
                    if (CUB) {
                        const bool ok = !left && ((xq <= xl) || d_extrap_right(METHOD));
                        const double u = xq - x0, t = u * refined_rcp(x1 - x0), omt = 1.0 - t;
                        const double w0 = ok ? (1.0 + 2.0 * t) * omt * omt : nanv;
                        const double w1 = t * t * (3.0 - 2.0 * t);
                        const double w2 = u * omt * omt;
                        const double w3 = u * t * (t - 1.0);
                        constexpr int LA = 3;
                        double g0[4], g1[4], g2[4], g3[4];
#pragma unroll
                        for (int r = 0; r < LA; ++r) {
                            g0[r] = Yb[v2_row(rbase + r) + o0]; g1[r] = Yb[v2_row(rbase + r) + o1]; g2[r] = Sb[v2_row(rbase + r) + o0]; g3[r] = Sb[v2_row(rbase + r) + o1];
                        }
#pragma unroll
                        for (int r = 0; r < NR; ++r) {
                            if (r + LA < NR) {
                                const int nn = r + LA;
                                g0[nn & 3] = Yb[v2_row(rbase + nn) + o0]; g1[nn & 3] = Yb[v2_row(rbase + nn) + o1];
                                g2[nn & 3] = Sb[v2_row(rbase + nn) + o0]; g3[nn & 3] = Sb[v2_row(rbase + nn) + o1];
                            }
                            __builtin_amdgcn_sched_barrier(0);
                            z[r] = w0 * g0[r & 3] + w1 * g1[r & 3] + w2 * g2[r & 3] + w3 * g3[r & 3];
                            __builtin_amdgcn_sched_barrier(0);
                        }
                    } else {
                        const bool right = j >= n - 1;
                        const bool hold = right && (METHOD == IVS_LINEAR || xq == xl);
                        const double dx = x1 - x0, rdx = refined_rcp(dx);
                        bool slow = !div_safe(dx);
                        constexpr int LA = 6;
                        double g0[8], g1[8];
#pragma unroll
                        for (int r = 0; r < LA; ++r) { g0[r] = Yb[v2_row(rbase + r) + o0]; g1[r] = Yb[v2_row(rbase + r) + o1]; }
#pragma unroll
                        for (int r = 0; r < NR; ++r) {
                            if (r + LA < NR) { const int nn = r + LA; g0[nn & 7] = Yb[v2_row(rbase + nn) + o0]; g1[nn & 7] = Yb[v2_row(rbase + nn) + o1]; }
                            __builtin_amdgcn_sched_barrier(0);
                            const double y0 = g0[r & 7], y1 = g1[r & 7];
                            double v = lerp_fast(xq, x0, y0, y1, dx, rdx, slow);
                            if (right) v = hold ? y1 : nanv;
                            if (left) v = nanv;
                            z[r] = v;
                            __builtin_amdgcn_sched_barrier(0);
                        }
                        if (__builtin_expect(__ballot(slow && !right && !left) != 0ull, 0)) {
                            if (slow && !right && !left) {
#pragma unroll
                                for (int r = 0; r < NR; ++r) z[r] = lerp_np(xq, x0, Yb[v2_row(rbase + r) + o0], x1, Yb[v2_row(rbase + r) + o1]);
                            }
                        }
                    }
                };
                if (split_rows) {
                    strike_rows(std::integral_constant<int, 8>{}, r_lo);
                    __syncthreads();
                    double* ZX = Y;
#pragma unroll
                    for (int r = 0; r < 8; ++r) ZX[(r_lo + r) * 64 + lane] = z[r];
                    __syncthreads();
#pragma unroll
                    for (int r = 0; r < DT; ++r) z[r] = ZX[r * 64 + lane];
                    if (d_is_local(METHOD)) {
#pragma unroll
                        for (int r = 0; r < DT; ++r) asm volatile("" : "+v"(z[r]));
                    }
                    const int half = (mT + 1) >> 1;
                    if (act) dense_maturity_pass<METHOD, WLDS, true, true, TSHARED>(z, tt, TTp, Wp, outb, q0, lane, true, mT, mK, nostamp,
                                                                                    w == 0 ? 0 : half, w == 0 ? half : mT, nT);
                } else {
                    strike_rows(std::integral_constant<int, DT>{}, 0);
                    if (d_is_local(METHOD)) {
#pragma unroll
                        for (int r = 0; r < DT; ++r) asm volatile("" : "+v"(z[r]));
                    }
                    if (act) dense_maturity_pass<METHOD, WLDS, false, true, TSHARED>(z, tt, TTp, Wp, outb, q0, lane, true, mT, mK, nostamp, 0, 0, nT);
                }
            }
            if (p.status && threadIdx.x == 0) p.status[b] = IVS_ST_OK;
        }
        it = it_next; b = b_next; n = n_next; koff = koff_next;
    }
}

#ifndef IVS_DIAG_MINIMAL
inline int launch_surface_dense_var(const SurfaceParams& p_in, const LaunchCtx& cx, const char** name) {
    SurfaceParams p = p_in;
    hipStream_t st = cx.st;
    if (p.nT < 4 || p.nT > DT || p.mT > D_MAX_MT) return 0;
    const bool tsh = p.t_stride == 0 && p.tq_stride == 0;
    if (p.nK < 4 || p.nK > 128) return 0;
    if (!p.k_off && p.k_stride != 0 && p.k_stride < p.nK) return 0;
    if (generic_lds_bytes(p.nK, p.nT) > 160 * 1024) return 0;
    if (!(d_is_hermite(p.method) || p.method == IVS_LINEAR || p.method == IVS_SLINEAR)) return 0;
    const bool wl = p.mT <= D_WLDS_MAX_MT;
    if (!launch_tq_or_zero_queue<true>(p, cx, tsh, false)) return -1;
    if (p.k_off && p.B > 0x7fffffffLL) return 0;
    VarWork vw;
    if (!var_work_lists(p, cx, vw)) return -1;
    auto grid_for = [&](size_t lds) {
        int per_cu = (int)((160 * 1024) / lds);
        per_cu = per_cu > 8 ? 8 : (per_cu < 1 ? 1 : per_cu);
        int64_t g = (int64_t)cx.num_cu * per_cu;
        return g > p.B ? p.B : g;
    };
#define IVS_VAR_LAUNCH1(M)                                                                                           \
    {                                                                                                                \
        const size_t lds = dense_var_lds_bytes<1>(p.mT);                                                             \
        const int64_t grid = grid_for(lds);                                                                          \
        if (wl && tsh) hipLaunchKernelGGL((surface_dense_var_kernel<M, 1, true, true>), dim3((unsigned)grid), dim3(64), lds, st, p, vw.wl1);    \
        else if (tsh) hipLaunchKernelGGL((surface_dense_var_kernel<M, 1, false, true>), dim3((unsigned)grid), dim3(64), lds, st, p, vw.wl1);    \
        else if (wl) hipLaunchKernelGGL((surface_dense_var_kernel<M, 1, true, false>), dim3((unsigned)grid), dim3(64), lds, st, p, vw.wl1);     \
        else hipLaunchKernelGGL((surface_dense_var_kernel<M, 1, false, false>), dim3((unsigned)grid), dim3(64), lds, st, p, vw.wl1);            \
    }
#define IVS_VAR_LAUNCH2(M)                                                                                           \
    {                                                                                                                \
        const size_t lds = dense_var2_lds_bytes(p.mT);                    \
        const int64_t grid = grid_for(lds);                                                                          \
        if (wl && tsh) hipLaunchKernelGGL((surface_dense_var2_kernel<M, true, true>), dim3((unsigned)grid), dim3(128), lds, st, p, vw.wl2);     \
        else if (tsh) hipLaunchKernelGGL((surface_dense_var2_kernel<M, false, true>), dim3((unsigned)grid), dim3(128), lds, st, p, vw.wl2);     \
        else if (wl) hipLaunchKernelGGL((surface_dense_var2_kernel<M, true, false>), dim3((unsigned)grid), dim3(128), lds, st, p, vw.wl2);      \
        else hipLaunchKernelGGL((surface_dense_var2_kernel<M, false, false>), dim3((unsigned)grid), dim3(128), lds, st, p, vw.wl2);             \
    }
#define IVS_VAR_CASE(M, NAME)                                                  \
    case M:                                                                    \
        if (vw.need1) IVS_VAR_LAUNCH1(M)                                        \
        if (vw.need2) IVS_VAR_LAUNCH2(M)                                        \
        *name = NAME;                                                          \
        break;
    bool known = true;
    switch (p.method) {
        IVS_VAR_CASE(IVS_LINEAR, "surface_dense_var_kernel<linear>")
        IVS_VAR_CASE(IVS_CUBIC, "surface_dense_var_kernel<cubic>")
        IVS_VAR_CASE(IVS_CUBICSPLINE, "surface_dense_var_kernel<cubicspline>")
        IVS_VAR_CASE(IVS_SLINEAR, "surface_dense_var_kernel<slinear>")
        IVS_VAR_CASE(IVS_PCHIP, "surface_dense_var_kernel<pchip>")
        IVS_VAR_CASE(IVS_AKIMA, "surface_dense_var_kernel<akima>")
        default: known = false;
    }
#undef IVS_VAR_CASE
#undef IVS_VAR_LAUNCH1
#undef IVS_VAR_LAUNCH2
    if (!known) return 0;
    const bool launched = hipGetLastError() == hipSuccess;
    if (launched) launch_surface_generic<true>(p, cx);
    return launched ? 1 : -1;
}

#endif

}
```

### iv_interpolation_amd/csrc/ivs_surface_generic.hpp

```cpp
#pragma once
#include "ivs_device.hpp"

namespace ivs {

struct SurfaceParams {
    const double* K; const int64_t* k_off; int64_t k_stride; int nK;
    int64_t k_total;
    const double* T; int64_t t_stride; int nT;
    const double* sigma; int64_t B;
    const double* Kq; int64_t kq_stride; int mK;
    const double* Tq; int64_t tq_stride; int mT;
    double* out; int32_t* status; int method;
    int map_groups;
    const void* tqs;
    unsigned long long* queue;
    const int* mode;
    int* redo;
};
constexpr int QUEUE_STRIDE = 16;

struct WorkQueue {
    unsigned long long* q; int R, g0, goff, gcur, ch, lane; int64_t region, limit, cur_i, cur_end;
    struct Pending { unsigned long long t; int g; bool need; };
    __device__ __forceinline__ void init(unsigned long long* heads, int groups, int64_t n_items, int chunk, int lane_) {
        q = heads; R = groups; limit = n_items; ch = chunk; lane = lane_;
        g0 = blockIdx.x % R; goff = 0; gcur = g0; region = (limit + R - 1) / R; cur_i = 0; cur_end = 0;
    }
    __device__ __forceinline__ unsigned long long claim(int g) const {
        unsigned long long t = 0ull;
        if (lane == 0) t = atomicAdd(q + g * QUEUE_STRIDE, 1ull);
        return t;
    }
    __device__ __forceinline__ bool resolve(unsigned long long t0, int g) {
        const unsigned lo = __builtin_amdgcn_readfirstlane((unsigned)t0), hi = __builtin_amdgcn_readfirstlane((unsigned)(t0 >> 32));
        return resolve_ticket((int64_t)(((unsigned long long)hi << 32) | lo), g);
    }
    __device__ __forceinline__ void skip_group() { ++goff; gcur = (g0 + goff) % R; }
    __device__ __forceinline__ bool resolve_ticket(int64_t t, int g) {
        int64_t gend = (int64_t)(g + 1) * region;
        gend = gend < limit ? gend : limit;
        const int64_t s0 = (int64_t)g * region + t * ch;
        if (t * ch >= region || s0 >= gend) return false;
        cur_i = s0; cur_end = s0 + ch < gend ? s0 + ch : gend;
        return true;
    }
    __device__ __forceinline__ int64_t take() {
        while (cur_i >= cur_end) {
            if (goff >= R) return -1;
            if (resolve(claim(gcur), gcur)) break;
            ++goff; gcur = (g0 + goff) % R;
        }
        return cur_i++;
    }
    __device__ __forceinline__ Pending begin(bool more) const {
        Pending pd; pd.g = gcur; pd.need = more && cur_i >= cur_end && goff < R; pd.t = pd.need ? claim(pd.g) : 0ull;
        return pd;
    }
    __device__ __forceinline__ int64_t finish(const Pending& pd, bool more) {
        if (!more) return -1;
        if (pd.need && !resolve(pd.t, pd.g)) { ++goff; gcur = (g0 + goff) % R; }
        return take();
    }
};
constexpr int WQ_CHUNK = 4;

__device__ __forceinline__ void count_redo(const SurfaceParams& p) { if (p.redo) *reinterpret_cast<volatile int*>(p.redo) = 1; }
__device__ __forceinline__ void count_redo(const SurfaceParams& p, bool& told) { if (!told) { count_redo(p); told = true; } }

constexpr int GEN_NTMAX = 32;

__host__ __device__ inline size_t generic_lds_bytes(int nKmax, int nT, bool slopes = true) {
    size_t LK = (size_t)nKmax + 1;
    size_t rows = (size_t)nT * LK;
    size_t scratch = rows > (size_t)nT * 64 ? rows : (size_t)nT * 64;
    size_t doubles = (size_t)nKmax + GEN_NTMAX
                     + rows
                     + (size_t)nT * 64;
    if (slopes) doubles += 2 * rows + scratch + (size_t)nT * 64;
    return doubles * 8 + (slopes ? 0 : ((rows * 2 + 15) & ~(size_t)15))  + (size_t)nT * 64  + GEN_NTMAX * 4 ;
}

struct RowX {
    const uint16_t* idx; const double* K;
    __device__ __forceinline__ double operator()(int i) const { return K[idx[i]]; }
};
struct ColX {
    const uint8_t* idx; const double* T;
    __device__ __forceinline__ double operator()(int i) const { return T[idx[i * 64]]; }
};

constexpr unsigned long long REDO_SENTINEL = 0x7ff8dead00000001ull;

template <bool FILTER>
__global__ __launch_bounds__(64) void surface_generic_kernel(SurfaceParams p) {
    extern __shared__ __attribute__((aligned(16))) unsigned char smem[];
    const int lane = threadIdx.x;
    const int nT = p.nT, nKmax = p.nK, LK = nKmax + 1;
    const int method = p.method;
    const bool cubic = method_is_cubic(method);
    const int minkn = method_min_knots(method);

    const size_t rows = (size_t)nT * LK;
    const size_t scratch = rows > (size_t)nT * 64 ? rows : (size_t)nT * 64;
    double* Ksh = reinterpret_cast<double*>(smem);
    double* Tsh = Ksh + nKmax;
    double* ys = Tsh + GEN_NTMAX;
    double* cz = ys + rows;
    double* xs = cz + (size_t)nT * 64;
    double* ss = xs + (cubic ? rows : 0);
    double* cps = ss + (cubic ? rows : 0);
    double* cs = cps + (cubic ? scratch : 0);
    uint16_t* xi = reinterpret_cast<uint16_t*>(cs + (cubic ? (size_t)nT * 64 : 0));
    uint8_t* ctidx = reinterpret_cast<uint8_t*>(xi) + (cubic ? 0 : ((rows * 2 + 15) & ~(size_t)15));
    int* nrow = reinterpret_cast<int*>(ctidx + (size_t)nT * 64);

    if (FILTER && p.redo && *p.redo == 0) return;
    const int64_t n_outer = FILTER ? (p.B + 63) / 64 : p.B;
    for (int64_t ob = blockIdx.x; ob < n_outer; ob += gridDim.x) {
      unsigned long long todo = 1ull;
      if (FILTER) {
          const int64_t bi = ob * 64 + lane;
          const bool tagged = bi < p.B &&
              reinterpret_cast<const unsigned long long*>(p.out + bi * (int64_t)p.mT * p.mK)[0] == REDO_SENTINEL;
          todo = __ballot(tagged);
      }
      while (todo) {
        const int bit = FILTER ? __builtin_ctzll(todo) : 0;
        todo &= todo - 1;
        const int64_t b = FILTER ? ob * 64 + bit : ob;
        int64_t koff; int nKb;
        if (p.k_off) {
            koff = p.k_off[b];
            const int64_t span = p.k_off[b + 1] - koff;
            if (span < 0 || span > nKmax || koff < 0 || (p.k_total > 0 && koff + span > p.k_total)) {
                if (p.status && lane == 0) p.status[b] = IVS_ST_BAD_SHAPE;
                continue;
            }
            nKb = (int)span;
        } else { koff = b * p.k_stride; nKb = nKmax; }
        const double* Kb = p.K + koff;
        const double* sb = p.k_off ? p.sigma + (int64_t)nT * koff : p.sigma + b * (int64_t)nT * nKmax;
        const double* Tb = p.T + b * p.t_stride;
        const double* Kqb = p.Kq + b * p.kq_stride;
        const double* Tqb = p.Tq + b * p.tq_stride;
        double* outb = p.out + b * (int64_t)p.mT * p.mK;
        int st = 0;

        __syncthreads();
        for (int k = lane; k < nKb; k += 64) Ksh[k] = Kb[k];
        if (lane < nT) Tsh[lane] = Tb[lane];
        if (lane < nT) nrow[lane] = 0;
        __syncthreads();
        for (int c0 = 0; c0 < nKb; c0 += 64) {
            const int k = c0 + lane;
            const bool in = k < nKb;
            double v[GEN_NTMAX];
            const double kx = in ? Kb[k] : 0.0;
#pragma unroll
            for (int t = 0; t < GEN_NTMAX; ++t) v[t] = (t < nT && in) ? sb[(int64_t)t * nKb + k] : qnan();
#pragma unroll
            for (int t = 0; t < GEN_NTMAX; ++t) {
                if (t < nT) {
                    const bool valid = !__builtin_isnan(v[t]);
                    const unsigned long long m = __ballot(valid);
                    const int cnt = nrow[t];
                    const int rank = cnt + __popcll(m & ((1ull << lane) - 1ull));
                    if (valid) {
                        if (cubic) xs[t * LK + rank] = kx; else xi[t * LK + rank] = (uint16_t)k;
                        ys[t * LK + rank] = v[t];
// ... 80 lines not shown
```

### iv_interpolation_amd/csrc/ivs_surface_masked.hpp

```cpp
#pragma once
#include "ivs_surface_dense.hpp"

namespace ivs {

constexpr int MK_RS = 66;
__host__ __device__ constexpr size_t masked_lds_bytes() { return (size_t)(DT * MK_RS + DK) * 8 + 2 * DT * DK + DT * 4; }

struct MaskedT { const double* T; const uint8_t* idx; __device__ __forceinline__ double operator()(int i) const { return T[idx[i]]; } };
constexpr int MK_MAXCOL = 8;
struct MaskedX { const double* Ksh; const uint8_t* idx; __device__ __forceinline__ double operator()(int i) const { return Ksh[idx[i]]; } };

template <int METHOD>
__global__ __launch_bounds__(64, 3) void surface_masked_kernel(SurfaceParams p) {
    constexpr bool STEP = d_is_step(METHOD);
    static_assert(METHOD == IVS_LINEAR || METHOD == IVS_SLINEAR || METHOD == IVS_NEAREST || METHOD == IVS_ZERO || METHOD == IVS_FROM_DERIVATIVES,
                  "linear, slinear, nearest, zero, from_derivatives (the other dense methods: surface_masked_pass_kernel)");
    constexpr int MINROW = 2;
    extern __shared__ __attribute__((aligned(16))) unsigned char smem[];
    const int lane = threadIdx.x;
    const int mT = p.mT, mK = p.mK;
    double* YC = reinterpret_cast<double*>(smem);
    double* Ksh = YC + DT * MK_RS;
    uint8_t* IDX = reinterpret_cast<uint8_t*>(Ksh + DK);
    uint8_t* RANK = IDX + DT * DK;
    int* NROW = reinterpret_cast<int*>(RANK + DT * DK);
    const double nanv = __builtin_nan("");
    auto nostamp = [](int) {};

    TqTables tt;
    const double* TTp = nullptr;
    const double* Wp = nullptr;
    tq_from_shared(p.tqs, tt, TTp, Wp);

    const bool kq_shared = p.kq_stride == 0;
    const bool act = lane < mK;
    double xq = (kq_shared && act) ? p.Kq[lane] : nanv;
    const unsigned long long lt_mask = (1ull << lane) - 1ull, le_mask = lt_mask | (1ull << lane);

    const bool all = p.mode && *p.mode != 0;
    if (!all && p.redo && *p.redo == 0) return;
    bool told = false;
    double* tag_at = nullptr;
    auto leave = [&]() {
        if (lane == 0) {
            if (all) reinterpret_cast<unsigned long long*>(tag_at)[0] = REDO_SENTINEL;
            if (p.redo && !told) { *reinterpret_cast<volatile int*>(p.redo + 1) = 1; told = true; }
        }
    };
    const int64_t n_outer = (p.B + 63) / 64;
    WorkQueue wq;
    wq.init(p.queue + 16 * QUEUE_STRIDE, 1, n_outer, 1, lane);
    for (int64_t ob = p.queue ? wq.take() : (int64_t)blockIdx.x; ob >= 0 && ob < n_outer; ob = p.queue ? wq.take() : ob + gridDim.x) {
      const int64_t bi = ob * 64 + lane;
      const bool tagged = bi < p.B &&
          (all || reinterpret_cast<const unsigned long long*>(p.out + bi * (int64_t)mT * mK)[0] == REDO_SENTINEL);
      unsigned long long todo = __ballot(tagged);
      double vn[DT], kn = 0.0;
      auto request = [&](int64_t bb) {
          const double* sb = p.sigma + bb * (int64_t)(DT * DK);
#pragma unroll
          for (int t = 0; t < DT; ++t) vn[t] = sb[t * DK + lane];
          kn = p.K[bb * p.k_stride + lane];
      };
      if (todo) request(ob * 64 + __builtin_ctzll(todo));
      while (todo) {
        const int bit = __builtin_ctzll(todo);
        todo &= todo - 1;
        const int64_t b = ob * 64 + bit;
        double* outb = p.out + b * (int64_t)mT * mK;
        tag_at = outb;
        double v[DT];
#pragma unroll
        for (int t = 0; t < DT; ++t) v[t] = vn[t];
        const double kx = kn;
        if (!kq_shared) xq = act ? p.Kq[b * p.kq_stride + lane] : nanv;
        if (todo) request(ob * 64 + __builtin_ctzll(todo));
        __syncthreads();
        Ksh[lane] = kx;
        bool give_up = tt.unsorted != 0;
#pragma unroll
        for (int t = 0; t < DT; ++t) {
            const bool valid = !__builtin_isnan(v[t]);
            const unsigned long long m = __ballot(valid);
            give_up = give_up || __ballot(__builtin_isinf(v[t])) != 0ull;
            const int rank = __popcll(m & lt_mask);
            if (valid) { YC[t * MK_RS + rank] = v[t]; IDX[t * DK + rank] = (uint8_t)lane; }
            RANK[t * DK + lane] = (uint8_t)__popcll(m & le_mask);
            const int nt = __popcll(m);
            if (lane == 0) NROW[t] = nt;
            give_up = give_up || nt < MINROW;
        }
        if (give_up) { leave(); continue; }
        __syncthreads();
        __syncthreads();
        int jf = -1;
        if (Ksh[0] <= xq) {
            jf = 0;
#pragma unroll
            for (int m = 1; m < 8; ++m) jf += (Ksh[8 * m] <= xq) ? 8 : 0;
#pragma unroll
            for (int st = 4; st >= 1; st >>= 1) if (Ksh[jf + st] <= xq) jf += st;
        }
        double z[DT];
        bool all_ok = true;
#pragma unroll
        for (int t = 0; t < DT; ++t) {
            const int n = NROW[t];
            const int j = jf >= 0 ? (int)RANK[t * DK + jf] - 1 : -1;
            const MaskedX X{Ksh, IDX + t * DK};
            const CView Y{YC + t * MK_RS, 1};
            if (METHOD == IVS_NEAREST) {
                double r = nanv;
                if (j >= 0 && xq <= X(n - 1)) {
                    const int jj = j > n - 2 ? n - 2 : j;
                    r = j > n - 2 ? Y(n - 1) : step_eval<IVS_NEAREST>(xq, X(jj), X(jj + 1), Y(jj), Y(jj + 1));
                }
                z[t] = r;
            } else if (STEP) z[t] = eval_method(METHOD, X, Y, Y, n, j, xq);
            else z[t] = eval_linear(X, Y, n, j, xq, METHOD == IVS_LINEAR);
            all_ok = all_ok && !__builtin_isnan(z[t]);
        }
        const bool col_masked = act && !all_ok;
        const unsigned long long mm = __ballot(col_masked);
        if (mm != 0ull) {
            if (__popcll(mm) > MK_MAXCOL) { leave(); continue; }
            __syncthreads();
            double* Tsh = Ksh;
            double* cz = YC;
            uint8_t* cti = IDX;
            if (lane < DT) Tsh[lane] = p.T[lane];
            const int slot = __popcll(mm & lt_mask);
            int cn = 0;
            if (col_masked) {
#pragma unroll
                for (int t = 0; t < DT; ++t)
                    if (!__builtin_isnan(z[t])) { cz[slot * DT + cn] = z[t]; cti[slot * DT + cn] = (uint8_t)t; ++cn; }
            }
            if (__ballot(col_masked && cn > 0 && cn < method_min_knots(METHOD)) != 0ull) { leave(); continue; }
            __syncthreads();
            if (col_masked) {
                const MaskedT cx{Tsh, cti + slot * DT};
                const CView cy{cz + slot * DT, 1};
                int jc = -1;
                for (int tq = 0; tq < mT; ++tq) {
                    const double x = p.Tq[tq];
                    double r = nanv;
                    if (cn > 0) {
                        while (jc + 1 < cn && cx(jc + 1) <= x) ++jc;
                        r = eval_method(METHOD, cx, cy, cy, cn, jc, x);
                    }
                    outb[(int64_t)tq * mK + lane] = r;
                }
            }
        }
        if (act && all_ok) dense_maturity_pass<METHOD, true, false, false, true>(z, tt, TTp, Wp, outb, 0, lane, true, mT, mK, nostamp);
        if (p.status && lane == 0) p.status[b] = IVS_ST_OK;
      }
    }
}

}
#include "ivs_surface_masked_pass.hpp"
namespace ivs {

#ifndef IVS_DIAG_MINIMAL
inline bool launch_surface_masked(const SurfaceParams& p, const LaunchCtx& cx) {
    if (p.k_off || p.nK != DK || p.nT != DT || p.mK > 64 || p.mT > D_MAX_MT) return false;
    if (p.t_stride != 0 || p.tq_stride != 0 || !p.tqs) return false;
    int64_t grid = (int64_t)cx.num_cu * 12;
    const int64_t work = (p.B + 63) / 64;
    if (grid > work) grid = work;
    switch (p.method) {
#define IVS_MASKED_CASE(KERNEL, LDS, M) case M: hipLaunchKernelGGL((KERNEL<M>), dim3((unsigned)grid), dim3(64), LDS, cx.st, p); break;
        IVS_MASKED_CASE(surface_masked_kernel, masked_lds_bytes(), IVS_LINEAR)
        IVS_MASKED_CASE(surface_masked_kernel, masked_lds_bytes(), IVS_SLINEAR)
        IVS_MASKED_CASE(surface_masked_kernel, masked_lds_bytes(), IVS_NEAREST)
        IVS_MASKED_CASE(surface_masked_kernel, masked_lds_bytes(), IVS_ZERO)
        IVS_MASKED_CASE(surface_masked_kernel, masked_lds_bytes(), IVS_FROM_DERIVATIVES)
        IVS_MASKED_CASE(surface_masked_pass_kernel, masked_pass_lds_bytes(), IVS_CUBIC)
        IVS_MASKED_CASE(surface_masked_pass_kernel, masked_pass_lds_bytes(), IVS_CUBICSPLINE)
        IVS_MASKED_CASE(surface_masked_pass_kernel, masked_pass_lds_bytes(), IVS_QUADRATIC)
        IVS_MASKED_CASE(surface_masked_pass_kernel, masked_pass_lds_bytes(), IVS_PCHIP)
        IVS_MASKED_CASE(surface_masked_pass_kernel, masked_pass_lds_bytes(), IVS_AKIMA)
#undef IVS_MASKED_CASE
        default: return false;
    }
    return true;
}
#endif

}
```

### iv_interpolation_amd/csrc/ivs_surface_masked_pass.hpp

```cpp
#pragma once
#include "ivs_surface_masked.hpp"

namespace ivs {

constexpr int MP_ROWS = 8;
__host__ __device__ constexpr size_t masked_pass_lds_bytes() { return (size_t)(2 * MP_ROWS * MK_RS + DK) * 8 + 2 * MP_ROWS * DK + DT * 4; }

template <bool QUAD = false>
__device__ __forceinline__ void masked_solve8(const double* YC, double* XS, const int* NROW, int lane) {
    const int r = lane >> 3, seg = lane & 7, i0 = seg * 8;
    const int n = NROW[r];
    double* xr = XS + r * MK_RS;
    const double* yr = YC + r * MK_RS;
    auto cl = [&](int i) { return i < 0 ? 0 : (i > n - 1 ? n - 1 : i); };
    double xa = xr[cl(i0 - 2)], xb = xr[cl(i0 - 1)], xc = xr[cl(i0)], xd = xr[cl(i0 + 1)], xe = xr[cl(i0 + 2)];
    double ya = yr[cl(i0 - 2)], yb = yr[cl(i0 - 1)], yc = yr[cl(i0)], yd = yr[cl(i0 + 1)], ye = yr[cl(i0 + 2)];
    double dx0 = xb - xa, dx1 = xc - xb, dx2 = xd - xc, dx3 = xe - xd;
    double dl0 = (yb - ya) * refined_rcp(dx0), dl1 = (yc - yb) * refined_rcp(dx1), dl2 = (yd - yc) * refined_rcp(dx2),
           dl3 = (ye - yd) * refined_rcp(dx3);
    double xl = xe, yl = ye;
    double u[8], l[8], rh[8];
    double m00 = 1.0, m01 = 0.0, m10 = 0.0, m11 = 1.0;
    double uF = 0.0, lF = 0.0, rF = 0.0, uL = 0.0, lL = 0.0, rL = 0.0;
    int kl = -1;
// ... 34 lines not shown
        double uu = c * rb, ll = a * rb, hh = rr * rb;
        if (!QUAD) {
            if (k == 0) { const bool first = seg == 0; uu = first ? uF : uu; ll = first ? lF : ll; hh = first ? rF : hh; }
            const bool last = k == kl;
            uu = last ? uL : uu; ll = last ? lL : ll; hh = last ? rL : hh;
        }
        u[k] = in ? uu : 0.0; l[k] = in ? ll : 0.0; rh[k] = in ? hh : 0.0;
        const double n00 = u[k] * m10, n01 = u[k] * m11, n10 = m10 - l[k] * m00, n11 = m11 - l[k] * m01;
        m00 = n00; m01 = n01; m10 = n10; m11 = n11;
        if (k < 7) {
            const int j = cl(i + 3);
            const double xn = xr[j], yn = yr[j];
            dx0 = dx1; dx1 = dx2; dx2 = dx3; dx3 = xn - xl;
            dl0 = dl1; dl1 = dl2; dl2 = dl3; dl3 = (yn - yl) * refined_rcp(dx3);
            xl = xn; yl = yn;
            if (QUAD) { qa = qb; qb = qc; qc = qd; qd = qe; qe = xn; qy0 = qy1; qy1 = qy2; qy2 = yn; }
        }
    }
#define IVS_MP_MAT_STEP(SH)                                                                                   \
    {                                                                                                         \
        const double e = dpp_f64<DPP_ROW_SHR(SH)>(1.0, m00), f = dpp_f64<DPP_ROW_SHR(SH)>(0.0, m01);          \
        const double g = dpp_f64<DPP_ROW_SHR(SH)>(0.0, m10), h = dpp_f64<DPP_ROW_SHR(SH)>(1.0, m11);          \
        const bool has = seg >= SH;                                                                           \
        const double n00 = m00 * e + m01 * g, n01 = m00 * f + m01 * h, n10 = m10 * e + m11 * g, n11 = m10 * f + m11 * h; \
        m00 = has ? n00 : m00; m01 = has ? n01 : m01; m10 = has ? n10 : m10; m11 = has ? n11 : m11;           \
    }
    IVS_MP_MAT_STEP(1) IVS_MP_MAT_STEP(2) IVS_MP_MAT_STEP(4)
#undef IVS_MP_MAT_STEP
    const double pin = dpp_f64<DPP_ROW_SHR(1)>(0.0, m01), qin = dpp_f64<DPP_ROW_SHR(1)>(1.0, m11);
    double cprev = seg == 0 ? 0.0 : pin * refined_rcp(qin);
    double dprev = 0.0, prod = 1.0;
#pragma unroll
    for (int k = 0; k < 8; ++k) {
        const double rw = refined_rcp(1.0 - l[k] * cprev);
        cprev = u[k] * rw;
        const double al = l[k] * rw;
        dprev = rh[k] * rw - al * dprev;
        prod *= -al;
        u[k] = cprev; rh[k] = dprev; l[k] = prod;
    }
    {
        double A = prod, B = dprev;
#define IVS_MP_AFF_STEP(SH)                                                                                   \
        { const double a_ = dpp_f64<DPP_ROW_SHR(SH)>(1.0, A), b_ = dpp_f64<DPP_ROW_SHR(SH)>(0.0, B);          \
          const bool has = seg >= SH; B = has ? __builtin_fma(A, b_, B) : B; A = has ? A * a_ : A; }
        IVS_MP_AFF_STEP(1) IVS_MP_AFF_STEP(2) IVS_MP_AFF_STEP(4)
#undef IVS_MP_AFF_STEP
        double din = dpp_f64<DPP_ROW_SHR(1)>(0.0, B);
        din = seg == 0 ? 0.0 : din;
#pragma unroll
        for (int k = 0; k < 8; ++k) rh[k] = __builtin_fma(l[k], din, rh[k]);
    }
    double nxt = 0.0;
    prod = 1.0;
#pragma unroll
    for (int k = 7; k >= 0; --k) {
        nxt = rh[k] - u[k] * nxt;
        prod *= -u[k];
        rh[k] = nxt; l[k] = prod;
    }
    {
        double A = prod, B = nxt;
#define IVS_MP_AFF_STEP(SH)                                                                                   \
        { const double a_ = dpp_f64<DPP_ROW_SHL(SH)>(1.0, A), b_ = dpp_f64<DPP_ROW_SHL(SH)>(0.0, B);          \
          const bool has = seg + SH <= 7; B = has ? __builtin_fma(A, b_, B) : B; A = has ? A * a_ : A; }
        IVS_MP_AFF_STEP(1) IVS_MP_AFF_STEP(2) IVS_MP_AFF_STEP(4)
#undef IVS_MP_AFF_STEP
        double sin_ = dpp_f64<DPP_ROW_SHL(1)>(0.0, B);
        sin_ = seg == 7 ? 0.0 : sin_;
#pragma unroll
        for (int k = 0; k < 8; ++k) rh[k] = __builtin_fma(l[k], sin_, rh[k]);
    }
    __builtin_amdgcn_wave_barrier();
#pragma unroll
    for (int k = 0; k < 8; ++k) if (i0 + k < n) xr[i0 + k] = rh[k];
}

template <int METHOD>
__device__ __forceinline__ void masked_local8(const double* YC, double* XS, const int* NROW, int lane) {
    constexpr bool AK = METHOD == IVS_AKIMA;
    const int r = lane >> 3, seg = lane & 7, i0 = seg * 8;
    const int n = NROW[r];
    double* xr = XS + r * MK_RS;
    const double* yr = YC + r * MK_RS;
    auto cl = [&](int i) { return i < 0 ? 0 : (i > n - 1 ? n - 1 : i); };
    double F[11], DX[11];
    {
        double xa = xr[cl(i0 - 2)], ya = yr[cl(i0 - 2)];
#pragma unroll
        for (int i = 0; i < 11; ++i) {
            const int idx = i0 - 2 + i;
            const double xb = xr[cl(idx + 1)], yb = yr[cl(idx + 1)];
            const bool in = idx >= 0 && idx <= n - 2;
            const double dx = xb - xa;
            DX[i] = in ? dx : 0.0;
            F[i] = in ? (yb - ya) * refined_rcp(dx) : 0.0;
            xa = xb; ya = yb;
        }
    }
    double d[8];
    if (AK) {
        const double x3 = xr[n - 3], x2 = xr[n - 2], x1 = xr[n - 1], y3 = yr[n - 3], y2 = yr[n - 2], y1 = yr[n - 1];
        const double mL1 = (y1 - y2) * refined_rcp(x1 - x2), mL2 = (y2 - y3) * refined_rcp(x2 - x3);
        const double en1 = 2.0 * mL1 - mL2, en = 2.0 * en1 - mL1;
        const double m0 = (yr[1] - yr[0]) * refined_rcp(xr[1] - xr[0]), m1 = (yr[2] - yr[1]) * refined_rcp(xr[2] - xr[1]);
        const double em1 = 2.0 * m0 - m1, em2 = 2.0 * em1 - m0;
#pragma unroll
        for (int i = 0; i < 11; ++i) {
            const int idx = i0 - 2 + i;
            F[i] = idx == -1 ? em1 : (idx == -2 ? em2 : (idx == n - 1 ? en1 : (idx == n ? en : F[i])));
        }
        double fmax = 0.0;
#pragma unroll
        for (int k = 0; k < 8; ++k) {
            const double f = akima_f12(F[k], F[k + 1], F[k + 2], F[k + 3]);
            fmax = (i0 + k < n) ? __builtin_fmax(fmax, f) : fmax;
        }
        fmax = __builtin_fmax(fmax, dpp_f64<DPP_QUAD_SWAP1>(fmax, fmax));
        fmax = __builtin_fmax(fmax, dpp_f64<DPP_QUAD_SWAP2>(fmax, fmax));
        fmax = __builtin_fmax(fmax, dpp_f64<0x141>(fmax, fmax));
        const double thr = 1e-9 * fmax;
#pragma unroll
        for (int k = 0; k < 8; ++k) d[k] = akima_knot(F[k], F[k + 1], F[k + 2], F[k + 3], thr);
    } else {
        double e_last = 0.0, m_only = 0.0;
        {
            const int a3 = n >= 3 ? n - 3 : 0, a2 = n >= 3 ? n - 2 : 0, a1 = n - 1;
            const double x3 = xr[a3], x2 = xr[a2], x1 = xr[a1], y3 = yr[a3], y2 = yr[a2], y1 = yr[a1];
            const double h0 = x1 - x2, h1 = x2 - x3;
            const double mp = (y1 - y2) * refined_rcp(h0), mpp = (y2 - y3) * refined_rcp(h1);
            const double rs = refined_rcp(h0 + h1);
            e_last = pchip_edge(mp, mpp, (2.0 * h0 + h1) * rs, h0 * rs);
            m_only = (yr[n - 1] - yr[0]) * refined_rcp(xr[n - 1] - xr[0]);
        }
#pragma unroll
        for (int k = 0; k < 8; ++k) {
            const int i = i0 + k;
            double v = pchip_knot(F[k + 1], F[k + 2], 2.0 * DX[k + 2] + DX[k + 1], DX[k + 2] + 2.0 * DX[k + 1]);
            if (k == 0) {
                const double h0 = DX[2], h1 = DX[3], rs = refined_rcp(h0 + h1);
                const double e = pchip_edge(F[2], F[3], (2.0 * h0 + h1) * rs, h0 * rs);
                v = seg == 0 ? e : v;
            }
            v = i == n - 1 ? e_last : v;
            d[k] = n == 2 ? m_only : v;
        }
    }
    __builtin_amdgcn_wave_barrier();
#pragma unroll
    for (int k = 0; k < 8; ++k) if (i0 + k < n) xr[i0 + k] = d[k];
}

template <int METHOD>
__global__ __launch_bounds__(64, 3) void surface_masked_pass_kernel(SurfaceParams p) {
    static_assert(METHOD == IVS_CUBIC || METHOD == IVS_CUBICSPLINE || METHOD == IVS_QUADRATIC || d_is_local(METHOD), "tridiagonal and local-slope methods");
    constexpr bool QUAD = METHOD == IVS_QUADRATIC;
    constexpr bool LOCAL = d_is_local(METHOD);
    constexpr int MINROW = LOCAL ? (METHOD == IVS_AKIMA ? 3 : 2) : (QUAD ? 3 : 4);
    extern __shared__ __attribute__((aligned(16))) unsigned char smem[];
    const int lane = threadIdx.x;
    const int mT = p.mT, mK = p.mK;
    double* YC = reinterpret_cast<double*>(smem);
    double* XS = YC + MP_ROWS * MK_RS;
    double* Ksh = XS + MP_ROWS * MK_RS;
    uint8_t* IDX = reinterpret_cast<uint8_t*>(Ksh + DK);
    uint8_t* RANK = IDX + MP_ROWS * DK;
    int* NROW = reinterpret_cast<int*>(RANK + MP_ROWS * DK);
    const double nanv = __builtin_nan("");
    auto nostamp = [](int) {};

    TqTables tt;
    const double* TTp = nullptr;
    const double* Wp = nullptr;
    tq_from_shared(p.tqs, tt, TTp, Wp);

    const bool kq_shared = p.kq_stride == 0;
    const bool act = lane < mK;
    double xq = (kq_shared && act) ? p.Kq[lane] : nanv;
    const unsigned long long lt_mask = (1ull << lane) - 1ull, le_mask = lt_mask | (1ull << lane);

    const bool all = p.mode && *p.mode != 0;
    if (!all && p.redo && *p.redo == 0) return;
    bool told = false;
    double* tag_at = nullptr;
    auto leave = [&]() {
        if (lane == 0) {
            if (all) reinterpret_cast<unsigned long long*>(tag_at)[0] = REDO_SENTINEL;
            if (p.redo && !told) { *reinterpret_cast<volatile int*>(p.redo + 1) = 1; told = true; }
        }
    };
    const int64_t n_outer = (p.B + 63) / 64;
    WorkQueue wq;
    wq.init(p.queue + 16 * QUEUE_STRIDE, 1, n_outer, 1, lane);
    for (int64_t ob = p.queue ? wq.take() : (int64_t)blockIdx.x; ob >= 0 && ob < n_outer; ob = p.queue ? wq.take() : ob + gridDim.x) {
      const int64_t bi = ob * 64 + lane;
      const bool tagged = bi < p.B &&
          (all || reinterpret_cast<const unsigned long long*>(p.out + bi * (int64_t)mT * mK)[0] == REDO_SENTINEL);
      unsigned long long todo = __ballot(tagged);
      double vn[DT], kn = 0.0;
      auto request = [&](int64_t bb) {
          const double* sb = p.sigma + bb * (int64_t)(DT * DK);
#pragma unroll
          for (int t = 0; t < DT; ++t) vn[t] = sb[t * DK + lane];
          kn = p.K[bb * p.k_stride + lane];
      };
      if (todo) request(ob * 64 + __builtin_ctzll(todo));
      while (todo) {
        const int bit = __builtin_ctzll(todo);
        todo &= todo - 1;
        const int64_t b = ob * 64 + bit;
        double* outb = p.out + b * (int64_t)mT * mK;
        tag_at = outb;
        double v[DT];
#pragma unroll
        for (int t = 0; t < DT; ++t) v[t] = vn[t];
        const double kx = kn;
        if (!kq_shared) xq = act ? p.Kq[b * p.kq_stride + lane] : nanv;
        if (todo) request(ob * 64 + __builtin_ctzll(todo));
        bool give_up = tt.unsorted != 0;
        unsigned long long vm[DT];
#pragma unroll
        for (int t = 0; t < DT; ++t) {
            vm[t] = __ballot(!__builtin_isnan(v[t]));
            give_up = give_up || __ballot(__builtin_isinf(v[t])) != 0ull || __popcll(vm[t]) < MINROW;
        }
        if (give_up) { leave(); continue; }
        __syncthreads();
        Ksh[lane] = kx;
        double z[DT];
        bool all_ok = true;
        int jf = -1;
#pragma unroll
        for (int ps = 0; ps < DT / MP_ROWS; ++ps) {
            if (ps) __syncthreads();
#pragma unroll
            for (int r = 0; r < MP_ROWS; ++r) {
                const int t = ps * MP_ROWS + r;
                const unsigned long long m = vm[t];
                const int rank = __popcll(m & lt_mask);
                if ((m >> lane) & 1ull) { YC[r * MK_RS + rank] = v[t]; XS[r * MK_RS + rank] = kx; IDX[r * DK + rank] = (uint8_t)lane; }
                RANK[r * DK + lane] = (uint8_t)__popcll(m & le_mask);
                if (lane == 0) NROW[r] = __popcll(m);
            }
            __syncthreads();
            if (ps == 0 && Ksh[0] <= xq) {
                jf = 0;
#pragma unroll
                for (int m = 1; m < 8; ++m) jf += (Ksh[8 * m] <= xq) ? 8 : 0;
#pragma unroll
                for (int st = 4; st >= 1; st >>= 1) if (Ksh[jf + st] <= xq) jf += st;
            }
            if (LOCAL) masked_local8<METHOD>(YC, XS, NROW, lane);
            else masked_solve8<QUAD>(YC, XS, NROW, lane);
            __syncthreads();
#pragma unroll
            for (int r = 0; r < MP_ROWS; ++r) {
                const unsigned long long rm = vm[ps * MP_ROWS + r];
                const int n = __popcll(rm);
                const double x_last = readlane_f64(kx, 63 - __builtin_clzll(rm));
                const int j = jf >= 0 ? (int)RANK[r * DK + jf] - 1 : -1;
                const MaskedX X{Ksh, IDX + r * DK};
                const CView Y{YC + r * MK_RS, 1}, S{XS + r * MK_RS, 1};
                double zz;
                if (QUAD) {
                    zz = nanv;
                    if (j >= 0 && xq <= x_last) {
                        const double x_first = readlane_f64(kx, __builtin_ctzll(rm));
                        const int je = j > n - 2 ? n - 2 : j;
                        auto cl = [&](int i) { return i < 0 ? 0 : (i > n - 1 ? n - 1 : i); };
                        double W[6];
#pragma unroll
                        for (int i = 0; i < 6; ++i) W[i] = X(cl(je - 2 + i));
                        int q = je - 1 + ((xq >= (W[3] + W[2]) / 2.0) ? 1 : 0);
                        q = j < n - 1 ? q : n - 3;
                        q = q < 0 ? 0 : (q > n - 3 ? n - 3 : q);
                        const bool hi = q == je;
                        const double xs0 = hi ? W[1] : W[0], xs1 = hi ? W[2] : W[1], xs2 = hi ? W[3] : W[2], xs3 = hi ? W[4] : W[3],
                                     xs4 = hi ? W[5] : W[4];
                        const double tm1 = q + 1 <= 2 ? x_first : (xs1 + xs0) / 2.0;
                        const double t0 = q + 2 <= 2 ? x_first : (xs2 + xs1) / 2.0;
                        const double t1 = q + 3 >= n ? x_last : (xs3 + xs2) / 2.0;
                        const double t2 = q + 4 >= n ? x_last : (xs4 + xs3) / 2.0;
                        double h0, h1, h2;
                        quad_basis_t(tm1, t0, t1, t2, xq, h0, h1, h2);
                        zz = h0 * S(q) + h1 * S(q + 1) + h2 * S(q + 2);
                    }
                }
                else {
                    zz = nanv;
                    if (j >= 0 && (d_extrap_right(METHOD) || xq <= x_last)) {
                        const int jj = j > n - 2 ? n - 2 : j;
                        zz = hermite_eval(X(jj), X(jj + 1), Y(jj), Y(jj + 1), S(jj), S(jj + 1), xq);
                    }
                }
                z[ps * MP_ROWS + r] = zz;
                all_ok = all_ok && !__builtin_isnan(zz);
            }
        }
        const bool col_masked = act && !all_ok;
        const unsigned long long mm = __ballot(col_masked);
        if (mm != 0ull) {
            if (__popcll(mm) > MK_MAXCOL) { leave(); continue; }
            __syncthreads();
            double* Tsh = Ksh;
            double* cz = YC; double* cs = YC + MK_MAXCOL * DT; double* ccp = YC + 2 * MK_MAXCOL * DT;
            uint8_t* cti = IDX;
            if (lane < DT) Tsh[lane] = p.T[lane];
            const int slot = __popcll(mm & lt_mask);
            int cn = 0;
            if (col_masked) {
#pragma unroll
                for (int t = 0; t < DT; ++t)
                    if (!__builtin_isnan(z[t])) { cz[slot * DT + cn] = z[t]; cti[slot * DT + cn] = (uint8_t)t; ++cn; }
            }
            if (__ballot(col_masked && cn > 0 && cn < method_min_knots(METHOD)) != 0ull) { leave(); continue; }
            __syncthreads();
            if (col_masked) {
                const MaskedT cx{Tsh, cti + slot * DT};
                const CView cy{cz + slot * DT, 1};
                View csv{cs + slot * DT, 1}, cpw{ccp + slot * DT, 1};
                if (cn >= 2) method_slopes(METHOD, cx, cy, csv, cpw, cn);
                const CView csr{cs + slot * DT, 1};
                int jc = -1;
                for (int tq = 0; tq < mT; ++tq) {
                    const double x = p.Tq[tq];
                    double r = nanv;
                    if (cn > 0) {
                        while (jc + 1 < cn && cx(jc + 1) <= x) ++jc;
                        r = eval_method(METHOD, cx, cy, csr, cn, jc, x);
                    }
                    outb[(int64_t)tq * mK + lane] = r;
                }
            }
        }
        if (act && all_ok) dense_maturity_pass<METHOD, true, false, false, true>(z, tt, TTp, Wp, outb, 0, lane, true, mT, mK, nostamp);
        if (p.status && lane == 0) p.status[b] = IVS_ST_OK;
      }
    }
}

}
```

### iv_interpolation_amd/csrc/ivs_surface_pass.hpp

```cpp
#pragma once
#include "ivs_surface_dense_var2.hpp"
#include "ivs_surface_masked.hpp"

namespace ivs {

constexpr int PASS_SL = 8;
constexpr int PASS_CAP2 = 12;
constexpr int PASS_CHUNK = 4;

template <int NKB>
struct PassGeom {
    static constexpr int SL = PASS_SL;
    static constexpr int NSEG = 64 * NKB / SL;
    static constexpr int RP = 64 / NSEG;
    static constexpr int NPASS = DT / RP;
    static constexpr int KCAP = 64 * NKB;
    static constexpr int RS = NKB == 2 ? KCAP : KCAP + 2;
    static constexpr int PLANE = RP * RS;
    static constexpr int TS = SL + 2;
    static constexpr int TN = NSEG * TS;
    static constexpr int NSCAN = NSEG == 8 ? 3 : 4;
    static_assert(NSEG == 8 || NSEG == 16, "a row's segments live in one DPP row");
};
template <int NKB> __host__ __device__ constexpr bool pass_runp() { return NKB == 2; }
constexpr int PASS_TQ_DOUBLES = DT * 4 + D_WLDS_MAX_MT * 4;
template <int NKB, int KIND = 0>
__host__ __device__ constexpr size_t pass_lds_bytes() {
    using G = PassGeom<NKB>;
    if (KIND == 0 && pass_runp<NKB>()) return (size_t)(2 * G::PLANE + 4 * G::TN + 2) * 8;
    return KIND == 1 ? (size_t)(G::PLANE + G::KCAP) * 8 : (size_t)(2 * G::PLANE + (KIND == 2 ? 3 : 6) * G::TN + G::KCAP) * 8;
}

__device__ __forceinline__ int p_tix(int k) { return (k / PASS_SL) * (PASS_SL + 2) + (k % PASS_SL); }
template <int NKB> __device__ __forceinline__ int p_swz(int k) {
    return NKB == 2 ? k ^ (((k >> 5) & 3) << 1) : k ^ (((k >> 4) & 3) << 1);
}
template <int NKB> __device__ __forceinline__ int y_swz(int k) { return NKB == 2 ? k ^ (((k >> 5) & 3) << 1) : k; }

__device__ __forceinline__ double seg_prefix_prod(double v, int lane) {
    static_assert(PASS_SL == 8, "three shift steps");
    const int i = lane & 7;
    double t = dpp_f64<DPP_ROW_SHR(1)>(1.0, v); v *= i >= 1 ? t : 1.0;
    t = dpp_f64<DPP_ROW_SHR(2)>(1.0, v); v *= i >= 2 ? t : 1.0;
    t = dpp_f64<DPP_ROW_SHR(4)>(1.0, v); v *= i >= 4 ? t : 1.0;
    return v;
}
__device__ __forceinline__ double seg_suffix_prod(double v, int lane) {
    const int i = lane & 7;
    double t = dpp_f64<DPP_ROW_SHL(1)>(1.0, v); v *= i <= 6 ? t : 1.0;
    t = dpp_f64<DPP_ROW_SHL(2)>(1.0, v); v *= i <= 5 ? t : 1.0;
    t = dpp_f64<DPP_ROW_SHL(4)>(1.0, v); v *= i <= 3 ? t : 1.0;
    return v;
}

template <int NKB, bool VAR, bool QUADM = false>
__device__ __forceinline__ void pass_factor_tables(const double* X, int n, int lane, double* TB, double* SCR = nullptr) {
    using G = PassGeom<NKB>;
    constexpr int SL = G::SL, TS = G::TS;
    constexpr int TN = G::TN, NSEG = G::NSEG;
    constexpr bool RUNP = pass_runp<NKB>();
    double* AL = TB; double* CP = TB + TN; double* PP = TB + 2 * TN; double* QQ = TB + 3 * TN;
    double* PI = TB + 4 * TN; double* PSI = TB + 5 * TN;
    double c00 = 1.0, c01 = 0.0, c10 = 0.0, c11 = 1.0;
    double carry_crb = 0.0, carry_rdx = 0.0, carry_rdx_prev = 0.0;
#pragma unroll
    for (int blk = 0; blk < NKB; ++blk) {
        const int ir = blk * 64 + lane;
        const bool in = ir < n;
        const int i = in ? ir : n - 1;
        const double x0 = X[i];
        const double xp = X[i + 1 < n ? i + 1 : n - 1];
        const double xpp = X[i + 2 < n ? i + 2 : n - 1];
        const double xm = X[i > 0 ? i - 1 : 0];
        const double xmm = X[i > 1 ? i - 2 : 0];
        const double dxc = xp - x0, dxm = x0 - xm, dxp = xpp - xp, dxmm = xm - xmm;
        const double rdxc = refined_rcp(dxc);
        const bool first = ir == 0, last = ir == n - 1;
        double a, b, c;
        if (QUADM) {
            const CView xv{X, 1};
            quad_row(xv, n, i, a, b, c);
        } else
        if (first) { a = 0.0; b = dxp; c = dxc + dxp; }
        else if (last) { a = dxmm + dxm; b = dxmm; c = 0.0; }
        else { a = dxc; b = 2.0 * (dxm + dxc); c = dxm; }
        if (!in) { a = 0.0; b = 1.0; c = 0.0; }
        const double rb = refined_rcp(b);
        const double crb = c * rb;
        double crb_prev = dpp0_f64<DPP_WAVE_SHR1>(crb);
        if (blk > 0 && lane == 0) crb_prev = carry_crb;
        const bool ident = first || !in;
        const double g = ident ? 0.0 : a * rb * crb_prev;
        double p00 = 1.0, p01 = ident ? 0.0 : -g, p10 = ident ? 0.0 : 1.0, p11 = ident ? 1.0 : 0.0;
        scan_mat2<64>(p00, p01, p10, p11, lane);
        if (blk > 0) {
            const double n00 = p00 * c00 + p01 * c10, n01 = p00 * c01 + p01 * c11;
            const double n10 = p10 * c00 + p11 * c10, n11 = p10 * c01 + p11 * c11;
            p00 = n00; p01 = n01; p10 = n10; p11 = n11;
        }
        const double num = p00 + p01, den = p10 + p11;
        const double rw = first ? rb : den * rb * refined_rcp(num);
        const double al = a * rw, cp = c * rw;
        double rdx_prev = dpp0_f64<DPP_WAVE_SHR1>(rdxc);
        if (blk > 0 && lane == 0) rdx_prev = carry_rdx;
        const double rdx_next = dpp0_f64<DPP_WAVE_SHL1>(rdxc);
        double rdxmm = dpp0_f64<DPP_WAVE_SHR1>(rdx_prev);
        if (blk > 0 && lane == 0) rdxmm = carry_rdx_prev;
        const double d = first ? dxc + dxp : dxmm + dxm;
        const double rd = refined_rcp(d);
        double pm = 0.0, pp, qq;
        if (QUADM) {
            pp = rw; qq = 0.0;
        } else
        if (first) {
            pp = (dxc + 2.0 * d) * dxp * rdxc * rd * rw;
            qq = dxc * dxc * rdx_next * rd * rw;
        } else if (last) {
            pm = dxm * dxm * rdxmm * rd * rw;
            pp = (2.0 * d + dxm) * dxmm * rdx_prev * rd * rw;
            qq = 0.0;
            if (!VAR) { qq = pp; pp = pm; }
        } else {
            pp = 3.0 * dxc * rdx_prev * rw;
            qq = 3.0 * dxm * rdxc * rw;
        }
        const double pi = seg_prefix_prod(in ? -al : 1.0, lane);
        const double psi = seg_suffix_prod(in ? -cp : 1.0, lane);
        {
            const int kl = p_tix(ir);
            AL[kl] = in ? al : -1.0; CP[kl] = in ? cp : 0.0; PP[kl] = in ? pp : 0.0; QQ[kl] = in ? qq : 0.0;
            if (RUNP) {
                if (VAR && last) TB[4 * TN] = pm;
                if ((lane & (SL - 1)) == SL - 1) SCR[ir / SL] = pi;
                if ((lane & (SL - 1)) == 0) SCR[NSEG + ir / SL] = in ? psi : 0.0;
            } else {
                if (VAR && last) PI[SL + 1] = pm;
                PI[kl] = pi; PSI[kl] = psi;
                if ((lane & (SL - 1)) == SL - 1) PI[(ir / SL) * TS + SL] = pi;
                if ((lane & (SL - 1)) == 0) PSI[(ir / SL) * TS + SL] = in ? psi : 0.0;
            }
        }
        if (blk + 1 < NKB) {
            c00 = readlane_f64(p00, 63); c01 = readlane_f64(p01, 63); c10 = readlane_f64(p10, 63); c11 = readlane_f64(p11, 63);
            carry_crb = readlane_f64(crb, 63); carry_rdx = readlane_f64(rdxc, 63); carry_rdx_prev = readlane_f64(rdx_prev, 63);
        }
    }
    __syncthreads();
    {
        const int j = lane < NSEG ? lane : NSEG - 1;
        double pw = lane < NSEG ? (RUNP ? SCR[j] : PI[j * TS + SL]) : 1.0, qw = lane < NSEG ? (RUNP ? SCR[NSEG + j] : PSI[j * TS + SL]) : 1.0;
        double fm[4], bm[4];
#pragma unroll
        for (int s = 0; s < G::NSCAN; ++s) {
            fm[s] = j >= (1 << s) ? pw : 0.0;
            bm[s] = j + (1 << s) <= NSEG - 1 ? qw : 0.0;
            if (s == 0) { pw *= dpp_f64<DPP_ROW_SHR(1)>(1.0, pw); qw *= dpp_f64<DPP_ROW_SHL(1)>(1.0, qw); }
            if (s == 1) { pw *= dpp_f64<DPP_ROW_SHR(2)>(1.0, pw); qw *= dpp_f64<DPP_ROW_SHL(2)>(1.0, qw); }
            if (s == 2) { pw *= dpp_f64<DPP_ROW_SHR(4)>(1.0, pw); qw *= dpp_f64<DPP_ROW_SHL(4)>(1.0, qw); }
        }
        if (lane < NSEG) {
            AL[j * TS + SL] = fm[0]; AL[j * TS + SL + 1] = fm[1]; CP[j * TS + SL] = fm[2];
            PP[j * TS + SL] = bm[0]; PP[j * TS + SL + 1] = bm[1]; QQ[j * TS + SL] = bm[2];
            if (NSEG > 8) { CP[j * TS + SL + 1] = fm[3]; QQ[j * TS + SL + 1] = bm[3]; }
        }
    }
    __syncthreads();
}

template <int NKB, bool VAR, bool QUADM = false>
__device__ __forceinline__ void pass_sweeps(const double* Yp, double* Sp, const double* TB, int lane, int n) {
    using G = PassGeom<NKB>;
    constexpr int SL = G::SL, TN = G::TN, NSEG = G::NSEG, RS = G::RS, TS = G::TS;
    const double* AL = TB; const double* CP = TB + TN; const double* PP = TB + 2 * TN; const double* QQ = TB + 3 * TN;
    constexpr bool RUNP = pass_runp<NKB>();
    const double* PI = TB + 4 * TN; const double* PSI = TB + 5 * TN;
    const double pm_last = VAR ? (RUNP ? TB[4 * TN] : PI[SL + 1]) : 0.0;
    const int tl = lane / NSEG, seg = lane % NSEG;
// ... 67 lines not shown
            const double dp = RUNP ? d[m] : d[m] + (u ? tpi.y : tpi.x) * din;
            nxt = dp - (u ? tcp.y : tcp.x) * nxt;
            d[m] = nxt;
        }
        if (mm == 4) __builtin_amdgcn_sched_barrier(0);
    }
    const double2 bm01 = *reinterpret_cast<const double2*>(PP + tb + SL);
    const double2 bm23 = *reinterpret_cast<const double2*>(QQ + tb + SL);
    double f = nxt;
    f = __builtin_fma(bm01.x, dpp0_f64<DPP_ROW_SHL(1)>(f), f);
    f = __builtin_fma(bm01.y, dpp0_f64<DPP_ROW_SHL(2)>(f), f);
    f = __builtin_fma(bm23.x, dpp0_f64<DPP_ROW_SHL(4)>(f), f);
    if (NSEG > 8) f = __builtin_fma(bm23.y, dpp0_f64<DPP_ROW_SHL(8)>(f), f);
    double sin_ = dpp0_f64<DPP_ROW_SHL(1)>(f);
    sin_ = s_last ? 0.0 : sin_;
    double* srow = Sp + tl * RS + kb;
    const int sx = NKB == 2 ? (seg >> 2) & 3 : (seg >> 1) & 3;
    if (RUNP) {
        double psi = 1.0;
#pragma unroll
        for (int c = SL / 2 - 1; c >= 0; --c) {
            const double2 tcp = tab2(CP, 2 * c);
            double2 v;
            psi *= -tcp.y; v.y = __builtin_fma(psi, sin_, d[2 * c + 1]);
            psi *= -tcp.x; v.x = __builtin_fma(psi, sin_, d[2 * c]);
            *reinterpret_cast<double2*>(srow + 2 * (c ^ sx)) = v;
        }
        return;
    }
#pragma unroll
    for (int c = 0; c < SL / 2; ++c) {
        const double2 tps = tab2(PSI, 2 * c);
        double2 v;
        v.x = d[2 * c] + tps.x * sin_; v.y = d[2 * c + 1] + tps.y * sin_;
        *reinterpret_cast<double2*>(srow + 2 * (c ^ sx)) = v;
    }
}

template <int NKB, bool VAR>
__device__ __forceinline__ void pass_local_tables(const double* X, int n, int lane, double* TB) {
    using G = PassGeom<NKB>;
#pragma unroll
    for (int blk = 0; blk < NKB; ++blk) {
        const int k = blk * 64 + lane;
        double r0, r1, r2;
        local_tables_rt(X, n, k, r0, r1, r2);
        const int kl = p_tix(k);
        TB[kl] = r0; TB[G::TN + kl] = r1; TB[2 * G::TN + kl] = r2;
    }
    __syncthreads();
}
template <int METHOD, int NKB, bool VAR>
__device__ __forceinline__ void pass_local_slopes(const double* Yp, double* Sp, const double* TB, int lane, int n) {
    using G = PassGeom<NKB>;
    constexpr bool AK = METHOD == IVS_AKIMA;
    constexpr int TN = G::TN, NSEG = G::NSEG, RS = G::RS, TS = G::TS;
    const double* R0 = TB; const double* R1 = TB + TN; const double* R2 = TB + 2 * TN;
    const int tl = lane / NSEG, seg = lane % NSEG;
    const int kb = seg * 8, tb = seg * TS;
    const bool s_first = seg == 0;
    const double* yrow = Yp + tl * RS;
    const double* yr = yrow + kb;
    const int fy = NKB == 2 ? (seg >> 2) & 3 : 0;
    double y[12];
#pragma unroll
    for (int c = 0; c < 4; ++c) {
        const double2 v = *reinterpret_cast<const double2*>(yr + 2 * (c ^ fy));
        y[2 + 2 * c] = v.x; y[3 + 2 * c] = v.y;
    }
    {
        const int fl = NKB == 2 ? ((seg - 1) >> 2) & 3 : 0, fn = NKB == 2 ? ((seg + 1) >> 2) & 3 : 0;
        const double2 l = *reinterpret_cast<const double2*>(s_first ? yr : yr - 8 + 2 * (3 ^ fl));
        const double2 r = *reinterpret_cast<const double2*>(yr + 8 + 2 * fn);
        y[0] = l.x; y[1] = l.y; y[10] = r.x; y[11] = r.y;
    }
    double F[11];
    {
        const double2 rl = *reinterpret_cast<const double2*>(R0 + (s_first ? tb : tb - TS + 6));
        F[0] = (y[1] - y[0]) * rl.x; F[1] = (y[2] - y[1]) * rl.y;
#pragma unroll
        for (int c = 0; c < 4; ++c) {
            const double2 rr = *reinterpret_cast<const double2*>(R0 + tb + 2 * c);
            F[2 + 2 * c] = (y[3 + 2 * c] - y[2 + 2 * c]) * rr.x; F[3 + 2 * c] = (y[4 + 2 * c] - y[3 + 2 * c]) * rr.y;
        }
        F[10] = (y[11] - y[10]) * R0[tb + TS];
    }
    double thr = 0.0;
    if (AK) {
        const double l1 = 2.0 * F[2] - F[3], l0 = 2.0 * l1 - F[2];
        F[1] = s_first ? l1 : F[1]; F[0] = s_first ? l0 : F[0];
#pragma unroll
        for (int i = 2; i < 11; ++i) {
            const int idx = kb - 2 + i;
            F[i] = (idx == n - 1 || idx == n) ? 2.0 * F[i - 1] - F[i - 2] : F[i];
        }
        double fmax = 0.0;
#pragma unroll
        for (int m = 0; m < 8; ++m) {
            const double f = akima_f12(F[m], F[m + 1], F[m + 2], F[m + 3]);
            fmax = (kb + m < n) ? __builtin_fmax(fmax, f) : fmax;
        }
        fmax = __builtin_fmax(fmax, dpp_f64<DPP_QUAD_SWAP1>(fmax, fmax));
        fmax = __builtin_fmax(fmax, dpp_f64<DPP_QUAD_SWAP2>(fmax, fmax));
        fmax = __builtin_fmax(fmax, dpp_f64<0x141>(fmax, fmax));
        if (NSEG > 8) fmax = __builtin_fmax(fmax, dpp_f64<0x140>(fmax, fmax));
        thr = 1e-9 * fmax;
    }
    const int mlast = n - 1 - kb;
    double e_last = 0.0;
    if (!AK) {
        const int k1 = y_swz<NKB>(n - 1), k2 = y_swz<NKB>(n - 2), k3 = y_swz<NKB>(n - 3);
        const int t1 = p_tix(n - 1), t2 = p_tix(n - 2), t3 = p_tix(n - 3);
        const double m2 = (yrow[k1] - yrow[k2]) * R0[t2], m3 = (yrow[k2] - yrow[k3]) * R0[t3];
        e_last = pchip_edge(m2, m3, R1[t1], R2[t1]);
    }
    double d[8];
#pragma unroll
    for (int mm = 0; mm < 8; mm += 2) {
        double2 w1 = double2{0.0, 0.0}, w2 = double2{0.0, 0.0};
        if (!AK) { w1 = *reinterpret_cast<const double2*>(R1 + tb + mm); w2 = *reinterpret_cast<const double2*>(R2 + tb + mm); }
#pragma unroll
        for (int u = 0; u < 2; ++u) {
            const int m = mm + u;
            double v;
            if (AK) v = akima_knot(F[m], F[m + 1], F[m + 2], F[m + 3], thr);
            else {
                v = pchip_knot(F[m + 1], F[m + 2], u ? w1.y : w1.x, u ? w2.y : w2.x);
                if (m == 0) { const double e = pchip_edge(F[2], F[3], w1.x, w2.x); v = s_first ? e : v; }
                v = (m == mlast) ? e_last : v;
            }
            d[m] = v;
        }
        if (mm == 2) __builtin_amdgcn_sched_barrier(0);
    }
    double* srow = Sp + tl * RS + kb;
    const int sx = NKB == 2 ? (seg >> 2) & 3 : (seg >> 1) & 3;
#pragma unroll
    for (int c = 0; c < 4; ++c) {
        double2 v; v.x = d[2 * c]; v.y = d[2 * c + 1];
        *reinterpret_cast<double2*>(srow + 2 * (c ^ sx)) = v;
    }
}

#ifdef IVS_PASS_ENDSTAMP
__device__ unsigned long long* d_pass_ends = nullptr;
#endif

template <int METHOD, int NKB, bool VAR, bool TSH = true, bool NT16 = false>
__global__ __launch_bounds__(64, (d_is_local(METHOD) && VAR && !NT16) ? 2 : 3)
void surface_pass_kernel(SurfaceParams p, VarList list) {
#ifdef IVS_PASS_ENDSTAMP
    if (threadIdx.x == 0 && d_pass_ends) d_pass_ends[blockIdx.x * 2] = wall_clock64();
#endif
    if (!VAR && p.mode && *((const int IVS_CONST*)p.mode)) return;
    using G = PassGeom<NKB>;
    constexpr int RP = G::RP, NPASS = G::NPASS, KCAP = G::KCAP, RS = G::RS, TN = G::TN;
    constexpr int PFP = (NKB > 1 || d_is_local(METHOD)) ? 1 : NPASS;
    constexpr int PPL = RP * NKB;
    static_assert(NPASS % PFP == 0, "prefetch slots rotate with the passes");
    constexpr bool STEP = d_is_step(METHOD);
    constexpr bool LERP = METHOD == IVS_LINEAR || METHOD == IVS_SLINEAR || STEP;
    constexpr bool LOCAL = d_is_local(METHOD);
    constexpr bool QUADK = d_is_quad(METHOD);
    static_assert(LERP || LOCAL || QUADK || METHOD == IVS_CUBIC || METHOD == IVS_CUBICSPLINE, "methods of the dense kernels");
    extern __shared__ __attribute__((aligned(16))) unsigned char smem[];
    const int lane = threadIdx.x;
    const int mT = p.mT, mK = p.mK;
    double* Yp = reinterpret_cast<double*>(smem);
    double* Sp = Yp + G::PLANE;
    double* TB = Sp + G::PLANE;
    constexpr bool RUNP = !LERP && !LOCAL && pass_runp<NKB>();
    double* Ksh = LERP ? Yp + G::PLANE : (RUNP ? Sp : TB + (LOCAL ? 3 : 6) * TN);
    const double nanv = __builtin_nan(""), inf = __builtin_inf();
    auto nostamp = [](int) {};

    static_assert(TSH || METHOD == IVS_LINEAR, "per-surface maturities: linear only (the not-a-knot instantiations spilled 70-80 registers)");
    double* TTl = (LERP ? Ksh + KCAP : (RUNP ? TB + 4 * TN + 2 : Ksh + KCAP));
    double* Wl = TTl + DT * 4;
    TqTables tt;
    const double* TTp = nullptr;
    const double* Wp = nullptr;
    if (TSH) tq_from_shared(p.tqs, tt, TTp, Wp);
    constexpr bool NTR = VAR && !NT16;
    const int nT = NTR ? p.nT : DT;

    for (int i = lane; i < (LERP ? 1 : 2) * G::PLANE; i += 64) Yp[i] = 0.0;

    const bool kq_shared = p.kq_stride == 0;
    const bool act = lane < mK;
    double xq = (kq_shared && act) ? p.Kq[lane] : nanv;

    bool told = false;
    WorkQueue wq;
    if (!VAR) wq.init(p.queue, p.map_groups, p.B, PASS_CHUNK, lane);
    else wq.init(p.queue + list.qslot * 8 * QUEUE_STRIDE, 8, list.items ? (int64_t)*list.count : p.B, PASS_CHUNK, lane);
    auto at = [&](int64_t i, int& n, int64_t& koff) -> int64_t {
        if (VAR && list.items) { const VarItem v = list.items[i]; n = v.n; koff = v.koff; return v.b; }
        n = p.nK; koff = i * p.k_stride; return i;
    };

    double pre[PFP * PPL], pre_k[NKB];
    auto issue_pass = [&](int64_t b, int64_t ko, int nn, int ps) {
        const int slot = ps % PFP;
        if (!VAR) {
            const double2* s2 = reinterpret_cast<const double2*>(p.sigma + b * (int64_t)(DT * DK));
#pragma unroll
            for (int c = 0; c < RP / 2; ++c) {
                const double2 v = s2[(ps * (RP / 2) + c) * 64 + lane];
                pre[slot * RP + 2 * c] = v.x; pre[slot * RP + 2 * c + 1] = v.y;
            }
        } else {
            const double* sb = p.k_off ? p.sigma + (int64_t)nT * ko : p.sigma + b * (int64_t)nT * p.nK;
#pragma unroll
            for (int r = 0; r < RP; ++r)
#pragma unroll
                for (int blk = 0; blk < NKB; ++blk) {
                    const int t = ps * RP + r, k = blk * 64 + lane;
                    pre[(slot * RP + r) * NKB + blk] = (t < nT && k < nn) ? sb[(int64_t)t * nn + k] : 0.0;
                }
        }
        if (ps == 0) {
#pragma unroll
            for (int blk = 0; blk < NKB; ++blk) {
                const int k = blk * 64 + lane;
                pre_k[blk] = VAR ? (k < nn ? p.K[ko + k] : inf) : p.K[b * p.k_stride + k];
            }
        }
    };

    int n = KCAP, n_next = KCAP;
    int64_t koff = 0, koff_next = 0, b = 0, b_next = 0;
    int64_t it = wq.take();
    int64_t it_next = it >= 0 ? wq.take() : -1;
    if (it >= 0) {
        b = at(it, n, koff);
#pragma unroll
        for (int ps = 0; ps < PFP; ++ps) issue_pass(b, koff, n, ps);
    }

    int j = 0, jj = 0;
    double w0 = 0.0, w1 = 0.0, w2 = 0.0, w3 = 0.0;
    bool l_left = false, l_right = false, l_hold = false, l_slow = false;
    double kprev[NKB];
#pragma unroll
    for (int blk = 0; blk < NKB; ++blk) kprev[blk] = nanv;
    int n_prev = -1;
    bool tables_ok = false;

    while (it >= 0) {
        double* outb = p.out + b * (int64_t)mT * mK;
        const bool more = it_next >= 0;
        if (more) b_next = at(it_next, n_next, koff_next);
        const WorkQueue::Pending pend = wq.begin(more);
        if (!kq_shared) xq = act ? p.Kq[b * p.kq_stride + lane] : nanv;
        if (!TSH) {
            __syncthreads();
            dense_t_phase<METHOD, true, NTR>(p.T + b * p.t_stride, p.Tq + b * p.tq_stride, mT, lane, LERP ? Yp : Yp + 600, TTl, Wl, tt, nT, Yp);
            if (NKB == 1 && !LERP && lane < 2 * RP) { Yp[(lane >> 1) * RS + KCAP + (lane & 1)] = 0.0; Sp[(lane >> 1) * RS + KCAP + (lane & 1)] = 0.0; }
        }
        bool ok = !tt.unsorted;
        double z[DT];
        bool same_k = false;
#pragma unroll
        for (int ps = 0; ps < NPASS; ++ps) {
            const int slot = ps % PFP;
            __syncthreads();
            double acc = 0.0;
            if (!VAR) {
#pragma unroll
                for (int c = 0; c < RP / 2; ++c) {
                    const int tl = 2 * c + (lane >> 5), k = 2 * (lane & 31);
                    double2 v; v.x = pre[slot * RP + 2 * c]; v.y = pre[slot * RP + 2 * c + 1];
                    *reinterpret_cast<double2*>(&Yp[tl * RS + k]) = v;
                }
#pragma unroll
                for (int c = 0; c < RP; ++c) acc = __builtin_fma(pre[slot * RP + c], 0.0, acc);
            } else {
#pragma unroll
                for (int r = 0; r < RP; ++r)
#pragma unroll
                    for (int blk = 0; blk < NKB; ++blk) {
                        const double v = pre[(slot * RP + r) * NKB + blk];
                        Yp[r * RS + y_swz<NKB>(blk * 64 + lane)] = v;
                        acc = __builtin_fma(v, 0.0, acc);
                    }
            }
            if (ps == 0) {
                bool same = tables_ok && n == n_prev;
#pragma unroll
                for (int blk = 0; blk < NKB; ++blk) {
                    Ksh[blk * 64 + lane] = pre_k[blk];
                    same = same && __ballot(pre_k[blk] != kprev[blk]) == 0ull;
                    kprev[blk] = pre_k[blk];
                }
                n_prev = n;
                same_k = same;
            }
            ok = ok && __ballot(acc != 0.0) == 0ull;
            if (ps == 0) tables_ok = ok;
            {
                const int nx = ps + PFP;
                if (nx < NPASS) issue_pass(b, koff, n, nx);
                else if (more) issue_pass(b_next, koff_next, n_next, nx - NPASS);
            }
            __syncthreads();
            if (ok) {
                if (ps == 0 && !same_k) {
                    if (LOCAL) pass_local_tables<NKB, VAR>(Ksh, n, lane, TB);
                    else if (!LERP && ABL != 1 && ABL != 6) pass_factor_tables<NKB, VAR, QUADK>(Ksh, n, lane, TB, Sp + KCAP);
                }
                if (ps == 0 && !(same_k && kq_shared)) {
                    j = 0;
#pragma unroll
                    for (int m = 1; m < 8 * NKB; ++m) j += (Ksh[8 * m] <= xq) ? 8 : 0;
#pragma unroll
                    for (int st = 4; st >= 1; st >>= 1) if (Ksh[j + st] <= xq) j += st;
                    const double xl = Ksh[n - 1];
                    const bool left = !(Ksh[0] <= xq);
                    jj = j > n - 2 ? n - 2 : j;
                    const double x0 = Ksh[jj], x1 = Ksh[jj + 1];
                    if (LERP) {
                        l_left = left; l_right = j >= n - 1;
                        l_hold = l_right && (METHOD == IVS_LINEAR || xq == xl);
                        w0 = x0; w1 = x1; w2 = x1 - x0; w3 = refined_rcp(w2);
                        l_slow = !STEP && !div_safe(w2);
                    } else if (QUADK) {
                        const CView kx{Ksh, 1};
                        quad_weights(kx, n, j, xq, w0, w1, w2, w3);
                        if (left || !(xq <= xl)) w0 = nanv;
                    } else {
                        const bool okq = !left && ((xq <= xl) || d_extrap_right(METHOD));
                        const double u = xq - x0, t = u * refined_rcp(x1 - x0), omt = 1.0 - t;
                        w0 = okq ? (1.0 + 2.0 * t) * omt * omt : nanv;
                        w1 = t * t * (3.0 - 2.0 * t);
                        w2 = u * omt * omt;
                        w3 = u * t * (t - 1.0);
                    }
                }
                const int o0 = y_swz<NKB>(jj), o1 = y_swz<NKB>(jj + 1), q0 = p_swz<NKB>(jj), q1 = p_swz<NKB>(jj + 1);
                if (LERP) {
                    double g0[RP], g1[RP];
#pragma unroll
                    for (int r = 0; r < RP; ++r) { g0[r] = Yp[r * RS + o0]; g1[r] = Yp[r * RS + o1]; }
                    bool slow = l_slow;
#pragma unroll
                    for (int r = 0; r < RP; ++r) {
                        double v;
                        if (STEP) {
                            v = step_eval<METHOD>(xq, w0, w1, g0[r], g1[r]);
                            if (l_right && !l_hold) v = nanv;
                        } else {
                            v = lerp_fast(xq, w0, g0[r], g1[r], w2, w3, slow);
                            if (l_right) v = l_hold ? g1[r] : nanv;
                        }
                        if (l_left) v = nanv;
                        z[ps * RP + r] = v;
                    }
                    if (STEP) continue;
                    if (__builtin_expect(__ballot(slow && !l_right && !l_left) != 0ull, 0)) {
                        if (slow && !l_right && !l_left) {
#pragma unroll
                            for (int r = 0; r < RP; ++r) z[ps * RP + r] = lerp_np(xq, w0, Yp[r * RS + o0], w1, Yp[r * RS + o1]);
                        }
                    }
                    continue;
                }
                if (LOCAL) pass_local_slopes<METHOD, NKB, VAR>(Yp, Sp, TB, lane, n);
                else if (ABL != 1 && ABL != 6) pass_sweeps<NKB, VAR, QUADK>(Yp, Sp, TB, lane, n);
                __syncthreads();
                if (ABL == 2 || ABL == 6) {
#pragma unroll
                    for (int r = 0; r < RP; ++r) z[ps * RP + r] = Yp[r * RS + lane] + w0;
                    continue;
                }
                constexpr int LA = RP < 4 ? RP - 1 : 3;
                double g0[4], g1[4], g2[4], g3[4];
                const double* PA = QUADK ? Sp : Yp;
                const int a0i = QUADK ? p_swz<NKB>(jj > 0 ? jj - 1 : 0) : o0, a1i = QUADK ? q0 : o1;
                const int b0i = QUADK ? q1 : q0, b1i = QUADK ? p_swz<NKB>(jj + 2 < KCAP ? jj + 2 : KCAP - 1) : q1;
#pragma unroll
                for (int r = 0; r < LA; ++r) {
                    g0[r] = PA[r * RS + a0i]; g1[r] = PA[r * RS + a1i]; g2[r] = Sp[r * RS + b0i]; g3[r] = Sp[r * RS + b1i];
                }
#pragma unroll
                for (int r = 0; r < RP; ++r) {
                    if (r + LA < RP) {
                        const int nn = r + LA;
                        g0[nn & 3] = PA[nn * RS + a0i]; g1[nn & 3] = PA[nn * RS + a1i];
                        g2[nn & 3] = Sp[nn * RS + b0i]; g3[nn & 3] = Sp[nn * RS + b1i];
                    }
                    __builtin_amdgcn_sched_barrier(0);
                    z[ps * RP + r] = w0 * g0[r & 3] + w1 * g1[r & 3] + w2 * g2[r & 3] + w3 * g3[r & 3];
                    __builtin_amdgcn_sched_barrier(0);
                }
            }
        }
        if (ok) {
            if (LOCAL) {
#pragma unroll
                for (int r = 0; r < DT; ++r) asm volatile("" : "+v"(z[r]));
            }
            if (act) dense_maturity_pass<METHOD, true, false, NTR, TSH>(z, tt, TSH ? TTp : TTl, TSH ? Wp : Wl, outb, 0, lane, true, mT, mK,
                                                                        nostamp, 0, 0, nT);
            if (p.status && lane == 0) p.status[b] = IVS_ST_OK;
        } else if (lane == 0) {
            reinterpret_cast<unsigned long long*>(outb)[0] = D_SENTINEL;
            count_redo(p, told);
        }
        const int64_t it_next2 = wq.finish(pend, more);
        it = it_next; it_next = it_next2; b = b_next; n = n_next; koff = koff_next;
    }
#ifdef IVS_PASS_ENDSTAMP
    if (threadIdx.x == 0 && d_pass_ends) d_pass_ends[blockIdx.x * 2 + 1] = wall_clock64();
#endif
}

template <int METHOD, int NKB, bool VAR>
inline void launch_pass_nt(bool nt16, int64_t grid, size_t lds, hipStream_t st, const SurfaceParams& p, const VarList& list) {
    if constexpr (VAR) {
        if (nt16) { hipLaunchKernelGGL((surface_pass_kernel<METHOD, NKB, true, true, true>), dim3((unsigned)grid), dim3(64), lds, st, p, list); return; }
    }
    hipLaunchKernelGGL((surface_pass_kernel<METHOD, NKB, VAR, true, false>), dim3((unsigned)grid), dim3(64), lds, st, p, list);
}
inline int launch_surface_pass(const SurfaceParams& p_in, const LaunchCtx& cx, const char** name) {
    SurfaceParams p = p_in;
    hipStream_t st = cx.st;
    const bool lerp = p.method == IVS_LINEAR || p.method == IVS_SLINEAR || d_is_step(p.method);
    const bool local = d_is_local(p.method);
    if (!(p.method == IVS_CUBIC || p.method == IVS_CUBICSPLINE || p.method == IVS_QUADRATIC || lerp || local)) return 0;
    const bool tsh = p.t_stride == 0 && p.tq_stride == 0;
    if (!tsh && !(p.method == IVS_LINEAR && p.mT <= D_WLDS_MAX_MT)) return 0;
    if (p.mK > 64 || p.mT > D_MAX_MT) return 0;
    if (p.nT < 4 || p.nT > DT || p.nK < 4 || p.nK > 128) return 0;
    if (!p.k_off && p.k_stride != 0 && p.k_stride < p.nK) return 0;
    if (p.k_off && p.B > 0x7fffffffLL) return 0;
    const bool fixed64 = !p.k_off && p.nK == DK && p.nT == DT && !(reinterpret_cast<uintptr_t>(p.sigma) & 15);
    const bool nt16 = p.nT == DT;
    if (!(fixed64 || nt16 ? launch_tq_or_zero_queue<false>(p, cx, tsh, fixed64)
                          : launch_tq_or_zero_queue<true>(p, cx, tsh, fixed64))) return -1;
    auto grid_for = [&](size_t lds, int64_t work, int wg_cap = 12) {
        int per_cu = (int)((160 * 1024) / (((lds + 1279) / 1280) * 1280));
        per_cu = per_cu > wg_cap ? wg_cap : (per_cu < 1 ? 1 : per_cu);
#ifdef IVS_PASS_PER_CU
        per_cu = IVS_PASS_PER_CU;
#endif
        const int64_t g = (int64_t)cx.num_cu * per_cu;
        return g > work ? work : g;
    };
    const VarList none{nullptr, nullptr};
    static const char* const names[2][10] = {
        {"surface_pass_kernel<cubic>", "surface_pass_kernel<cubicspline>", "surface_pass_kernel<linear>", "surface_pass_kernel<slinear>",
         "surface_pass_kernel<pchip>", "surface_pass_kernel<akima>", "surface_pass_kernel<nearest>", "surface_pass_kernel<zero>",
         "surface_pass_kernel<from_derivatives>", "surface_pass_kernel<quadratic>"},
        {"surface_pass_var_kernel<cubic>", "surface_pass_var_kernel<cubicspline>", "surface_pass_var_kernel<linear>",
         "surface_pass_var_kernel<slinear>", "surface_pass_var_kernel<pchip>", "surface_pass_var_kernel<akima>",
         "surface_pass_var_kernel<nearest>", "surface_pass_var_kernel<zero>", "surface_pass_var_kernel<from_derivatives>",
         "surface_pass_var_kernel<quadratic>"}};
    int mi = 0;
    switch (p.method) {
        case IVS_CUBIC: mi = 0; break; case IVS_CUBICSPLINE: mi = 1; break; case IVS_LINEAR: mi = 2; break; case IVS_SLINEAR: mi = 3; break;
        case IVS_PCHIP: mi = 4; break; case IVS_AKIMA: mi = 5; break; case IVS_NEAREST: mi = 6; break; case IVS_ZERO: mi = 7; break;
        case IVS_QUADRATIC: mi = 9; break;
        default: mi = 8; break;
    }
#ifdef IVS_DIAG_MINIMAL
#define IVS_PASS_LAUNCH(NKB_, VAR_, CAP, LIST)                                                                                           \
    {                                                                                                                                    \
        const size_t lds = pass_lds_bytes<NKB_, 0>();                                                                                    \
        const int64_t grid = grid_for(lds, p.B, CAP);                                                                                    \
        if (!(VAR_)) p.map_groups = dense_map_groups(grid, p.B, cx.map_groups);                                                          \
        hipLaunchKernelGGL((surface_pass_kernel<IVS_CUBIC, NKB_, VAR_>), dim3((unsigned)grid), dim3(64), lds, st, p, LIST);              \
    }
#else
#define IVS_PASS_LAUNCH(NKB_, VAR_, CAP, LIST)                                                                                           \
    {                                                                                                                                    \
        size_t lds = lerp ? pass_lds_bytes<NKB_, 1>() : (local ? pass_lds_bytes<NKB_, 2>() : pass_lds_bytes<NKB_, 0>());                 \
        if (!tsh) lds += PASS_TQ_DOUBLES * 8;                                                                                            \
        const int64_t grid = grid_for(lds, p.B, (local && (VAR_) && !nt16) ? 8 : (CAP));                      \
        if (!(VAR_)) p.map_groups = dense_map_groups(grid, p.B, cx.map_groups);                                                          \
        if (!tsh) {                                                                                                                      \
            hipLaunchKernelGGL((surface_pass_kernel<IVS_LINEAR, NKB_, VAR_, false>), dim3((unsigned)grid), dim3(64), lds, st, p, LIST);  \
        } else                                                                                                                           \
        switch (p.method) {                                                                                                              \
            case IVS_CUBIC: launch_pass_nt<IVS_CUBIC, NKB_, VAR_>(nt16, grid, lds, st, p, LIST); break;                                  \
            case IVS_CUBICSPLINE: launch_pass_nt<IVS_CUBICSPLINE, NKB_, VAR_>(nt16, grid, lds, st, p, LIST); break;                      \
            case IVS_LINEAR: launch_pass_nt<IVS_LINEAR, NKB_, VAR_>(nt16, grid, lds, st, p, LIST); break;                                \
            case IVS_NEAREST: launch_pass_nt<IVS_NEAREST, NKB_, VAR_>(nt16, grid, lds, st, p, LIST); break;                              \
            case IVS_ZERO: launch_pass_nt<IVS_ZERO, NKB_, VAR_>(nt16, grid, lds, st, p, LIST); break;                                    \
            case IVS_FROM_DERIVATIVES: launch_pass_nt<IVS_FROM_DERIVATIVES, NKB_, VAR_>(nt16, grid, lds, st, p, LIST); break;            \
            case IVS_QUADRATIC: launch_pass_nt<IVS_QUADRATIC, NKB_, VAR_>(nt16, grid, lds, st, p, LIST); break;                          \
            case IVS_PCHIP: launch_pass_nt<IVS_PCHIP, NKB_, VAR_>(nt16, grid, lds, st, p, LIST); break;                                  \
            case IVS_AKIMA: launch_pass_nt<IVS_AKIMA, NKB_, VAR_>(nt16, grid, lds, st, p, LIST); break;                                  \
            default: launch_pass_nt<IVS_SLINEAR, NKB_, VAR_>(nt16, grid, lds, st, p, LIST); break;                                       \
        }                                                                                                                                \
    }
#endif
    if (fixed64) {
        IVS_PASS_LAUNCH(1, false, 12, none)
        *name = names[0][mi];
    } else {
        VarWork vw;
        if (!var_work_lists(p, cx, vw)) return -1;
        if (vw.need1) IVS_PASS_LAUNCH(1, true, 12, vw.wl1)
        if (vw.need2) IVS_PASS_LAUNCH(2, true, PASS_CAP2, vw.wl2)
        *name = names[1][mi];
    }
#undef IVS_PASS_LAUNCH
    if (hipGetLastError() != hipSuccess) return -1;
#ifndef IVS_DIAG_MINIMAL
    if (fixed64 && launch_surface_masked(p, cx) && p.redo) ++p.redo;
#endif
    launch_surface_generic<true>(p, cx);
    return 1;
}

}
```

Before: 325.0 million.

## Fuse masked redo pass into dense pass kernel via per-block linked list

Rows that fail the fast pass are chained into a per-block linked list stored in their output slot. The same block then reprocesses them with the masked redo routine before it exits, so the separate masked-kernel launch is dropped for fixed 64x16 surfaces. This removes one kernel launch and the global scan for sentinel tags. The cost is that LDS may grow to the masked kernel's requirement, which can lower occupancy. A launch counter instrumentation API is also added.

```diff
diff --git a/include/ivs.h b/include/ivs.h
--- a/include/ivs.h
+++ b/include/ivs.h
@@ -149,6 +149,7 @@
                                void* workspace, size_t workspace_bytes, void* stream);
 
 const char* ivs_last_kernel(void);
+int         ivs_last_launch_count(void);
 
 int     ivs_debug_stamps(void* device_buf, int64_t n_u64);
 int64_t ivs_debug_last_grid(void);
diff --git a/iv_interpolation_amd/_lib.py b/iv_interpolation_amd/_lib.py
--- a/iv_interpolation_amd/_lib.py
+++ b/iv_interpolation_amd/_lib.py
@@ -86,6 +86,7 @@
     "ivs_version": (C.c_int, []),
     "ivs_last_error": (C.c_char_p, []),
     "ivs_last_kernel": (C.c_char_p, []),
+    "ivs_last_launch_count": (C.c_int, []),
     "ivs_device_count": (C.c_int, []),
     "ivs_interp1d_workspace_bytes": (_sz, [_i64, _i64, _i32]),
     "ivs_interp1d_batch_f64": (C.c_int, [_p, _p, _i64, _p, _i64, _i32, _i64, _p, _p, _i64, _p, _i64, _p, _i32,
diff --git a/iv_interpolation_amd/csrc/ivs_api.hip b/iv_interpolation_amd/csrc/ivs_api.hip
--- a/iv_interpolation_amd/csrc/ivs_api.hip
+++ b/iv_interpolation_amd/csrc/ivs_api.hip
@@ -65,6 +65,7 @@
 const char* ivs_last_error(void) { return g_err; }
 
 const char* ivs_last_kernel(void) { return g_last_kernel; }
+int ivs_last_launch_count(void) { return ivs::g_launch_count; }
 
 int ivs_debug_stamps(void* device_buf, int64_t n_u64) {
     g_stamp_buf = static_cast<unsigned long long*>(device_buf);
@@ -511,6 +512,7 @@
                           void* workspace, size_t workspace_bytes, void* stream) {
     g_err[0] = 0;
     g_last_kernel = "";
+    ivs::g_launch_count = 0;
     if (!valid_method(method)) return fail(IVS_EINVAL, "ivs_surface_batch_f64: unknown method %d", method);
     if (ivs::method_is_poly(method)) return fail(IVS_EINVAL, "ivs_surface_batch_f64: method %d ('barycentric' / 'krogh') is 1-D only", method);
     if (B < 0 || nK < 0 || nT < 0 || mK < 0 || mT < 0) return fail(IVS_EINVAL, "ivs_surface_batch_f64: negative size");
@@ -534,7 +536,7 @@
     ivs::SurfaceParams p;
     p.K = K; p.k_off = k_off; p.k_stride = k_off ? 0 : k_stride; p.nK = nK; p.k_total = k_off ? k_stride : 0;
     p.T = T; p.t_stride = t_stride; p.nT = nT;
-    p.sigma = sigma; p.B = B; p.map_groups = 1; p.tqs = nullptr; p.redo = nullptr; p.queue = nullptr; p.mode = nullptr;
+    p.sigma = sigma; p.B = B; p.map_groups = 1; p.tqs = nullptr; p.redo = nullptr; p.queue = nullptr; p.mode = nullptr; p.inline_redo = 0;
     p.Kq = Kq; p.kq_stride = kq_stride; p.mK = mK;
     p.Tq = Tq; p.tq_stride = tq_stride; p.mT = mT;
     p.out = out; p.status = status; p.method = method;
diff --git a/iv_interpolation_amd/csrc/ivs_device.hpp b/iv_interpolation_amd/csrc/ivs_device.hpp
--- a/iv_interpolation_amd/csrc/ivs_device.hpp
+++ b/iv_interpolation_amd/csrc/ivs_device.hpp
@@ -5,6 +5,9 @@
 #include "../../include/ivs.h"
 
 namespace ivs {
+
+inline thread_local int g_launch_count = 0;
+#define IVS_LAUNCH(...) do { ++ivs::g_launch_count; hipLaunchKernelGGL(__VA_ARGS__); } while (0)
 
 constexpr int WAVE = 64;
 
diff --git a/iv_interpolation_amd/csrc/ivs_surface_dense.hpp b/iv_interpolation_amd/csrc/ivs_surface_dense.hpp
--- a/iv_interpolation_amd/csrc/ivs_surface_dense.hpp
+++ b/iv_interpolation_amd/csrc/ivs_surface_dense.hpp
@@ -865,7 +865,7 @@
 }
 template <bool NTR>
 inline void launch_tq_tables(const SurfaceParams& p, TqShared* o, hipStream_t st) {
-#define IVS_TQ_CASE(M) case M: hipLaunchKernelGGL((tq_tables_kernel<M, NTR>), dim3(1), dim3(64), 0, st, p, o); break;
+#define IVS_TQ_CASE(M) case M: IVS_LAUNCH((tq_tables_kernel<M, NTR>), dim3(1), dim3(64), 0, st, p, o); break;
     switch (p.method) {
         IVS_TQ_CASE(IVS_LINEAR) IVS_TQ_CASE(IVS_CUBIC) IVS_TQ_CASE(IVS_CUBICSPLINE) IVS_TQ_CASE(IVS_SLINEAR)
         IVS_TQ_CASE(IVS_PCHIP) IVS_TQ_CASE(IVS_AKIMA) IVS_TQ_CASE(IVS_NEAREST) IVS_TQ_CASE(IVS_ZERO) IVS_TQ_CASE(IVS_FROM_DERIVATIVES)
@@ -1109,7 +1109,7 @@
     int64_t grid = (int64_t)cx.num_cu * per_cu * 2;
     const int64_t work = FILTER ? (p.B + 63) / 64 : p.B;
     if (grid > work) grid = work;
-    hipLaunchKernelGGL(surface_generic_kernel<FILTER>, dim3((unsigned)grid), dim3(64), lds, cx.st, p);
+    IVS_LAUNCH(surface_generic_kernel<FILTER>, dim3((unsigned)grid), dim3(64), lds, cx.st, p);
     return true;
 }
 
@@ -1129,7 +1129,7 @@
         p.redo = tq->redo;
         p.mode = set_mode ? &tq->mode : nullptr;
     } else {
-        if (hipMemsetAsync(tq->queue, 0, sizeof(TqShared::queue), cx.st) != hipSuccess) return false;
+        if (++g_launch_count, hipMemsetAsync(tq->queue, 0, sizeof(TqShared::queue), cx.st) != hipSuccess) return false;
         p.tqs = nullptr;
         p.redo = nullptr;
     }
@@ -1162,21 +1162,21 @@
     if (dbg) {
         if (!tsh) return 0;
         if (p.method == IVS_CUBIC) {
-            if (wl) hipLaunchKernelGGL((surface_dense_kernel<IVS_CUBIC, true, true, true>), dim3((unsigned)grid), dim3(64), lds, st, p, dbg);
-            else hipLaunchKernelGGL((surface_dense_kernel<IVS_CUBIC, true, false, true>), dim3((unsigned)grid), dim3(64), lds, st, p, dbg);
+            if (wl) IVS_LAUNCH((surface_dense_kernel<IVS_CUBIC, true, true, true>), dim3((unsigned)grid), dim3(64), lds, st, p, dbg);
+            else IVS_LAUNCH((surface_dense_kernel<IVS_CUBIC, true, false, true>), dim3((unsigned)grid), dim3(64), lds, st, p, dbg);
         } else {
-            if (wl) hipLaunchKernelGGL((surface_dense_kernel<IVS_LINEAR, true, true, true>), dim3((unsigned)grid), dim3(64), lds, st, p, dbg);
-            else hipLaunchKernelGGL((surface_dense_kernel<IVS_LINEAR, true, false, true>), dim3((unsigned)grid), dim3(64), lds, st, p, dbg);
+            if (wl) IVS_LAUNCH((surface_dense_kernel<IVS_LINEAR, true, true, true>), dim3((unsigned)grid), dim3(64), lds, st, p, dbg);
+            else IVS_LAUNCH((surface_dense_kernel<IVS_LINEAR, true, false, true>), dim3((unsigned)grid), dim3(64), lds, st, p, dbg);
         }
         *name = "surface_dense_kernel<stamp>";
         return hipGetLastError() == hipSuccess ? 1 : -1;
     }
 #define IVS_DENSE_CASE(M, NAME)                                                                            \
     case M: {                                                                                              \
-        if (tsh && wl) hipLaunchKernelGGL((surface_dense_kernel<M, true, true, false>), dim3((unsigned)grid), dim3(64), lds, st, p, nullptr);        \
-        else if (tsh) hipLaunchKernelGGL((surface_dense_kernel<M, true, false, false>), dim3((unsigned)grid), dim3(64), lds, st, p, nullptr);        \
-        else if (wl) hipLaunchKernelGGL((surface_dense_kernel<M, false, true, false>), dim3((unsigned)grid), dim3(64), lds, st, p, nullptr);         \
-        else hipLaunchKernelGGL((surface_dense_kernel<M, false, false, false>), dim3((unsigned)grid), dim3(64), lds, st, p, nullptr);                \
+        if (tsh && wl) IVS_LAUNCH((surface_dense_kernel<M, true, true, false>), dim3((unsigned)grid), dim3(64), lds, st, p, nullptr);        \
+        else if (tsh) IVS_LAUNCH((surface_dense_kernel<M, true, false, false>), dim3((unsigned)grid), dim3(64), lds, st, p, nullptr);        \
+        else if (wl) IVS_LAUNCH((surface_dense_kernel<M, false, true, false>), dim3((unsigned)grid), dim3(64), lds, st, p, nullptr);         \
+        else IVS_LAUNCH((surface_dense_kernel<M, false, false, false>), dim3((unsigned)grid), dim3(64), lds, st, p, nullptr);                \
         *name = NAME;                                                                                      \
         break;                                                                                             \
     }
diff --git a/iv_interpolation_amd/csrc/ivs_surface_dense_var.hpp b/iv_interpolation_amd/csrc/ivs_surface_dense_var.hpp
--- a/iv_interpolation_amd/csrc/ivs_surface_dense_var.hpp
+++ b/iv_interpolation_amd/csrc/ivs_surface_dense_var.hpp
@@ -554,11 +554,11 @@
     if (p.k_off) {
         counts = reinterpret_cast<int32_t*>(cx.ws + WS_TQ_BYTES);
         lists = reinterpret_cast<VarItem*>(cx.ws + WS_TQ_BYTES + WS_COUNTS_BYTES);
-        if (hipMemsetAsync(counts, 0, WS_COUNTS_BYTES, cx.st) != hipSuccess) return false;
+        if (++g_launch_count, hipMemsetAsync(counts, 0, WS_COUNTS_BYTES, cx.st) != hipSuccess) return false;
         int64_t cb = (p.B + 1023) / 1024;
         const int64_t cap = (int64_t)cx.num_cu * 8;
         if (cb > cap) cb = cap;
-        hipLaunchKernelGGL(var_classify_kernel, dim3((unsigned)cb), dim3(256), 0, cx.st, p, lists, lists + p.B, counts);
+        IVS_LAUNCH(var_classify_kernel, dim3((unsigned)cb), dim3(256), 0, cx.st, p, lists, lists + p.B, counts);
     }
     w.wl1 = VarList{lists, counts, 0};
     w.wl2 = VarList{lists ? lists + p.B : nullptr, counts ? counts + 1 : nullptr, 1};
diff --git a/iv_interpolation_amd/csrc/ivs_surface_dense_var2.hpp b/iv_interpolation_amd/csrc/ivs_surface_dense_var2.hpp
--- a/iv_interpolation_amd/csrc/ivs_surface_dense_var2.hpp
+++ b/iv_interpolation_amd/csrc/ivs_surface_dense_var2.hpp
@@ -451,19 +451,19 @@
     {                                                                                                                \
         const size_t lds = dense_var_lds_bytes<1>(p.mT);                                                             \
         const int64_t grid = grid_for(lds);                                                                          \
-        if (wl && tsh) hipLaunchKernelGGL((surface_dense_var_kernel<M, 1, true, true>), dim3((unsigned)grid), dim3(64), lds, st, p, vw.wl1);    \
-        else if (tsh) hipLaunchKernelGGL((surface_dense_var_kernel<M, 1, false, true>), dim3((unsigned)grid), dim3(64), lds, st, p, vw.wl1);    \
-        else if (wl) hipLaunchKernelGGL((surface_dense_var_kernel<M, 1, true, false>), dim3((unsigned)grid), dim3(64), lds, st, p, vw.wl1);     \
-        else hipLaunchKernelGGL((surface_dense_var_kernel<M, 1, false, false>), dim3((unsigned)grid), dim3(64), lds, st, p, vw.wl1);            \
+        if (wl && tsh) IVS_LAUNCH((surface_dense_var_kernel<M, 1, true, true>), dim3((unsigned)grid), dim3(64), lds, st, p, vw.wl1);    \
+        else if (tsh) IVS_LAUNCH((surface_dense_var_kernel<M, 1, false, true>), dim3((unsigned)grid), dim3(64), lds, st, p, vw.wl1);    \
+        else if (wl) IVS_LAUNCH((surface_dense_var_kernel<M, 1, true, false>), dim3((unsigned)grid), dim3(64), lds, st, p, vw.wl1);     \
+        else IVS_LAUNCH((surface_dense_var_kernel<M, 1, false, false>), dim3((unsigned)grid), dim3(64), lds, st, p, vw.wl1);            \
     }
 #define IVS_VAR_LAUNCH2(M)                                                                                           \
     {                                                                                                                \
         const size_t lds = dense_var2_lds_bytes(p.mT);                    \
         const int64_t grid = grid_for(lds);                                                                          \
-        if (wl && tsh) hipLaunchKernelGGL((surface_dense_var2_kernel<M, true, true>), dim3((unsigned)grid), dim3(128), lds, st, p, vw.wl2);     \
-        else if (tsh) hipLaunchKernelGGL((surface_dense_var2_kernel<M, false, true>), dim3((unsigned)grid), dim3(128), lds, st, p, vw.wl2);     \
-        else if (wl) hipLaunchKernelGGL((surface_dense_var2_kernel<M, true, false>), dim3((unsigned)grid), dim3(128), lds, st, p, vw.wl2);      \
-        else hipLaunchKernelGGL((surface_dense_var2_kernel<M, false, false>), dim3((unsigned)grid), dim3(128), lds, st, p, vw.wl2);             \
+        if (wl && tsh) IVS_LAUNCH((surface_dense_var2_kernel<M, true, true>), dim3((unsigned)grid), dim3(128), lds, st, p, vw.wl2);     \
+        else if (tsh) IVS_LAUNCH((surface_dense_var2_kernel<M, false, true>), dim3((unsigned)grid), dim3(128), lds, st, p, vw.wl2);     \
+        else if (wl) IVS_LAUNCH((surface_dense_var2_kernel<M, true, false>), dim3((unsigned)grid), dim3(128), lds, st, p, vw.wl2);      \
+        else IVS_LAUNCH((surface_dense_var2_kernel<M, false, false>), dim3((unsigned)grid), dim3(128), lds, st, p, vw.wl2);             \
     }
 #define IVS_VAR_CASE(M, NAME)                                                  \
     case M:                                                                    \
diff --git a/iv_interpolation_amd/csrc/ivs_surface_generic.hpp b/iv_interpolation_amd/csrc/ivs_surface_generic.hpp
--- a/iv_interpolation_amd/csrc/ivs_surface_generic.hpp
+++ b/iv_interpolation_amd/csrc/ivs_surface_generic.hpp
@@ -15,6 +15,7 @@
     const void* tqs;
     unsigned long long* queue;
     const int* mode;
+    int inline_redo;
     int* redo;
 };
 constexpr int QUEUE_STRIDE = 16;
diff --git a/iv_interpolation_amd/csrc/ivs_surface_masked.hpp b/iv_interpolation_amd/csrc/ivs_surface_masked.hpp
--- a/iv_interpolation_amd/csrc/ivs_surface_masked.hpp
+++ b/iv_interpolation_amd/csrc/ivs_surface_masked.hpp
@@ -11,12 +11,12 @@
 struct MaskedX { const double* Ksh; const uint8_t* idx; __device__ __forceinline__ double operator()(int i) const { return Ksh[idx[i]]; } };
 
 template <int METHOD>
-__global__ __launch_bounds__(64, 3) void surface_masked_kernel(SurfaceParams p) {
+__device__ __forceinline__ void masked_redo(const SurfaceParams& p, unsigned char* smem, const bool list, const int64_t head) {
     constexpr bool STEP = d_is_step(METHOD);
     static_assert(METHOD == IVS_LINEAR || METHOD == IVS_SLINEAR || METHOD == IVS_NEAREST || METHOD == IVS_ZERO || METHOD == IVS_FROM_DERIVATIVES,
                   "linear, slinear, nearest, zero, from_derivatives (the other dense methods: surface_masked_pass_kernel)");
     constexpr int MINROW = 2;
-    extern __shared__ __attribute__((aligned(16))) unsigned char smem[];
+    if (list && head < 0) return;
     const int lane = threadIdx.x;
     const int mT = p.mT, mK = p.mK;
     double* YC = reinterpret_cast<double*>(smem);
@@ -37,8 +37,8 @@
     double xq = (kq_shared && act) ? p.Kq[lane] : nanv;
     const unsigned long long lt_mask = (1ull << lane) - 1ull, le_mask = lt_mask | (1ull << lane);
 
-    const bool all = p.mode && *p.mode != 0;
-    if (!all && p.redo && *p.redo == 0) return;
+    const bool all = !list && p.mode && *p.mode != 0;
+    if (!list && !all && p.redo && *p.redo == 0) return;
     bool told = false;
     double* tag_at = nullptr;
     auto leave = [&]() {
@@ -47,26 +47,37 @@
             if (p.redo && !told) { *reinterpret_cast<volatile int*>(p.redo + 1) = 1; told = true; }
         }
     };
-    const int64_t n_outer = (p.B + 63) / 64;
+    const int64_t n_outer = list ? 1 : (p.B + 63) / 64;
     WorkQueue wq;
     wq.init(p.queue + 16 * QUEUE_STRIDE, 1, n_outer, 1, lane);
-    for (int64_t ob = p.queue ? wq.take() : (int64_t)blockIdx.x; ob >= 0 && ob < n_outer; ob = p.queue ? wq.take() : ob + gridDim.x) {
+    for (int64_t ob = list ? 0 : (p.queue ? wq.take() : (int64_t)blockIdx.x); ob >= 0 && ob < n_outer;
+         ob = list ? 1 : (p.queue ? wq.take() : ob + gridDim.x)) {
       const int64_t bi = ob * 64 + lane;
-      const bool tagged = bi < p.B &&
+      const bool tagged = !list && bi < p.B &&
           (all || reinterpret_cast<const unsigned long long*>(p.out + bi * (int64_t)mT * mK)[0] == REDO_SENTINEL);
-      unsigned long long todo = __ballot(tagged);
+      unsigned long long todo = list ? 1ull : __ballot(tagged);
+      int64_t nb = head;
+      int lkn = -1;
       double vn[DT], kn = 0.0;
       auto request = [&](int64_t bb) {
           const double* sb = p.sigma + bb * (int64_t)(DT * DK);
 #pragma unroll
           for (int t = 0; t < DT; ++t) vn[t] = sb[t * DK + lane];
           kn = p.K[bb * p.k_stride + lane];
+          if (list) lkn = lane == 0 ? reinterpret_cast<const int*>(p.out + bb * (int64_t)mT * mK)[2] : -1;
       };
-      if (todo) request(ob * 64 + __builtin_ctzll(todo));
+      if (todo) request(list ? nb : ob * 64 + __builtin_ctzll(todo));
       while (todo) {
-        const int bit = __builtin_ctzll(todo);
-        todo &= todo - 1;
-        const int64_t b = ob * 64 + bit;
+        int64_t b;
+        if (list) {
+            b = nb;
+            nb = (int64_t)__builtin_amdgcn_readfirstlane(lkn);
+            todo = nb >= 0 ? 1ull : 0ull;
+        } else {
+            const int bit = __builtin_ctzll(todo);
+            todo &= todo - 1;
+            b = ob * 64 + bit;
+        }
         double* outb = p.out + b * (int64_t)mT * mK;
         tag_at = outb;
         double v[DT];
@@ -74,7 +85,7 @@
         for (int t = 0; t < DT; ++t) v[t] = vn[t];
         const double kx = kn;
         if (!kq_shared) xq = act ? p.Kq[b * p.kq_stride + lane] : nanv;
-        if (todo) request(ob * 64 + __builtin_ctzll(todo));
+        if (todo) request(list ? nb : ob * 64 + __builtin_ctzll(todo));
         __syncthreads();
         Ksh[lane] = kx;
         bool give_up = tt.unsorted != 0;
@@ -158,6 +169,11 @@
       }
     }
 }
+template <int METHOD>
+__global__ __launch_bounds__(64, 3) void surface_masked_kernel(SurfaceParams p) {
+    extern __shared__ __attribute__((aligned(16))) unsigned char smem[];
+    masked_redo<METHOD>(p, smem, false, -1);
+}
 
 }
 #include "ivs_surface_masked_pass.hpp"
@@ -171,7 +187,7 @@
     const int64_t work = (p.B + 63) / 64;
     if (grid > work) grid = work;
     switch (p.method) {
-#define IVS_MASKED_CASE(KERNEL, LDS, M) case M: hipLaunchKernelGGL((KERNEL<M>), dim3((unsigned)grid), dim3(64), LDS, cx.st, p); break;
+#define IVS_MASKED_CASE(KERNEL, LDS, M) case M: IVS_LAUNCH((KERNEL<M>), dim3((unsigned)grid), dim3(64), LDS, cx.st, p); break;
         IVS_MASKED_CASE(surface_masked_kernel, masked_lds_bytes(), IVS_LINEAR)
         IVS_MASKED_CASE(surface_masked_kernel, masked_lds_bytes(), IVS_SLINEAR)
         IVS_MASKED_CASE(surface_masked_kernel, masked_lds_bytes(), IVS_NEAREST)
diff --git a/iv_interpolation_amd/csrc/ivs_surface_masked_pass.hpp b/iv_interpolation_amd/csrc/ivs_surface_masked_pass.hpp
--- a/iv_interpolation_amd/csrc/ivs_surface_masked_pass.hpp
+++ b/iv_interpolation_amd/csrc/ivs_surface_masked_pass.hpp
@@ -210,12 +210,12 @@
 }
 
 template <int METHOD>
-__global__ __launch_bounds__(64, 3) void surface_masked_pass_kernel(SurfaceParams p) {
+__device__ __forceinline__ void masked_pass_redo(const SurfaceParams& p, unsigned char* smem, const bool list, const int64_t head) {
     static_assert(METHOD == IVS_CUBIC || METHOD == IVS_CUBICSPLINE || METHOD == IVS_QUADRATIC || d_is_local(METHOD), "tridiagonal and local-slope methods");
     constexpr bool QUAD = METHOD == IVS_QUADRATIC;
     constexpr bool LOCAL = d_is_local(METHOD);
     constexpr int MINROW = LOCAL ? (METHOD == IVS_AKIMA ? 3 : 2) : (QUAD ? 3 : 4);
-    extern __shared__ __attribute__((aligned(16))) unsigned char smem[];
+    if (list && head < 0) return;
     const int lane = threadIdx.x;
     const int mT = p.mT, mK = p.mK;
     double* YC = reinterpret_cast<double*>(smem);
@@ -237,8 +237,8 @@
     double xq = (kq_shared && act) ? p.Kq[lane] : nanv;
     const unsigned long long lt_mask = (1ull << lane) - 1ull, le_mask = lt_mask | (1ull << lane);
 
-    const bool all = p.mode && *p.mode != 0;
-    if (!all && p.redo && *p.redo == 0) return;
+    const bool all = !list && p.mode && *p.mode != 0;
+    if (!list && !all && p.redo && *p.redo == 0) return;
     bool told = false;
     double* tag_at = nullptr;
     auto leave = [&]() {
@@ -247,26 +247,37 @@
             if (p.redo && !told) { *reinterpret_cast<volatile int*>(p.redo + 1) = 1; told = true; }
         }
     };
-    const int64_t n_outer = (p.B + 63) / 64;
+    const int64_t n_outer = list ? 1 : (p.B + 63) / 64;
     WorkQueue wq;
     wq.init(p.queue + 16 * QUEUE_STRIDE, 1, n_outer, 1, lane);
-    for (int64_t ob = p.queue ? wq.take() : (int64_t)blockIdx.x; ob >= 0 && ob < n_outer; ob = p.queue ? wq.take() : ob + gridDim.x) {
+    for (int64_t ob = list ? 0 : (p.queue ? wq.take() : (int64_t)blockIdx.x); ob >= 0 && ob < n_outer;
+         ob = list ? 1 : (p.queue ? wq.take() : ob + gridDim.x)) {
       const int64_t bi = ob * 64 + lane;
-      const bool tagged = bi < p.B &&
+      const bool tagged = !list && bi < p.B &&
           (all || reinterpret_cast<const unsigned long long*>(p.out + bi * (int64_t)mT * mK)[0] == REDO_SENTINEL);
-      unsigned long long todo = __ballot(tagged);
+      unsigned long long todo = list ? 1ull : __ballot(tagged);
+      int64_t nb = head;
+      int lkn = -1;
       double vn[DT], kn = 0.0;
       auto request = [&](int64_t bb) {
           const double* sb = p.sigma + bb * (int64_t)(DT * DK);
 #pragma unroll
           for (int t = 0; t < DT; ++t) vn[t] = sb[t * DK + lane];
           kn = p.K[bb * p.k_stride + lane];
+          if (list) lkn = lane == 0 ? reinterpret_cast<const int*>(p.out + bb * (int64_t)mT * mK)[2] : -1;
       };
-      if (todo) request(ob * 64 + __builtin_ctzll(todo));
+      if (todo) request(list ? nb : ob * 64 + __builtin_ctzll(todo));
       while (todo) {
-        const int bit = __builtin_ctzll(todo);
-        todo &= todo - 1;
-        const int64_t b = ob * 64 + bit;
+        int64_t b;
+        if (list) {
+            b = nb;
+            nb = (int64_t)__builtin_amdgcn_readfirstlane(lkn);
+            todo = nb >= 0 ? 1ull : 0ull;
+        } else {
+            const int bit = __builtin_ctzll(todo);
+            todo &= todo - 1;
+            b = ob * 64 + bit;
+        }
         double* outb = p.out + b * (int64_t)mT * mK;
         tag_at = outb;
         double v[DT];
@@ -274,7 +285,7 @@
         for (int t = 0; t < DT; ++t) v[t] = vn[t];
         const double kx = kn;
         if (!kq_shared) xq = act ? p.Kq[b * p.kq_stride + lane] : nanv;
-        if (todo) request(ob * 64 + __builtin_ctzll(todo));
+        if (todo) request(list ? nb : ob * 64 + __builtin_ctzll(todo));
         bool give_up = tt.unsorted != 0;
         unsigned long long vm[DT];
 #pragma unroll
@@ -396,5 +407,17 @@
       }
     }
 }
-
-}
+template <int METHOD>
+__global__ __launch_bounds__(64, 3) void surface_masked_pass_kernel(SurfaceParams p) {
+    extern __shared__ __attribute__((aligned(16))) unsigned char smem[];
+    masked_pass_redo<METHOD>(p, smem, false, -1);
+}
+
+template <int METHOD>
+__device__ __forceinline__ void masked_redo_any(const SurfaceParams& p, unsigned char* smem, bool list, int64_t head) {
+    if constexpr (METHOD == IVS_LINEAR || METHOD == IVS_SLINEAR || d_is_step(METHOD)) masked_redo<METHOD>(p, smem, list, head);
+    else masked_pass_redo<METHOD>(p, smem, list, head);
+}
+__host__ __device__ constexpr size_t masked_any_lds_bytes(bool lerp) { return lerp ? masked_lds_bytes() : masked_pass_lds_bytes(); }
+
+}
diff --git a/iv_interpolation_amd/csrc/ivs_surface_pass.hpp b/iv_interpolation_amd/csrc/ivs_surface_pass.hpp
--- a/iv_interpolation_amd/csrc/ivs_surface_pass.hpp
+++ b/iv_interpolation_amd/csrc/ivs_surface_pass.hpp
@@ -23,6 +23,7 @@
     static_assert(NSEG == 8 || NSEG == 16, "a row's segments live in one DPP row");
 };
 template <int NKB> __host__ __device__ constexpr bool pass_runp() { return NKB == 2; }
+__host__ __device__ constexpr bool pass_inline_redo(int m) { return m != IVS_QUADRATIC && m != IVS_AKIMA; }
 constexpr int PASS_TQ_DOUBLES = DT * 4 + D_WLDS_MAX_MT * 4;
 template <int NKB, int KIND = 0>
 __host__ __device__ constexpr size_t pass_lds_bytes() {
@@ -396,7 +397,9 @@
 #ifdef IVS_PASS_ENDSTAMP
     if (threadIdx.x == 0 && d_pass_ends) d_pass_ends[blockIdx.x * 2] = wall_clock64();
 #endif
-    if (!VAR && p.mode && *((const int IVS_CONST*)p.mode)) return;
+    constexpr bool INL_K = !VAR && TSH && pass_inline_redo(METHOD);
+    const bool mqf = !VAR && p.mode && *((const int IVS_CONST*)p.mode);
+    if (mqf && !(INL_K && p.inline_redo)) return;
     using G = PassGeom<NKB>;
     constexpr int RP = G::RP, NPASS = G::NPASS, KCAP = G::KCAP, RS = G::RS, TN = G::TN;
     constexpr int PFP = (NKB > 1 || d_is_local(METHOD)) ? 1 : NPASS;
@@ -474,7 +477,7 @@
 
     int n = KCAP, n_next = KCAP;
     int64_t koff = 0, koff_next = 0, b = 0, b_next = 0;
-    int64_t it = wq.take();
+    int64_t it = mqf ? -1 : wq.take();
     int64_t it_next = it >= 0 ? wq.take() : -1;
     if (it >= 0) {
         b = at(it, n, koff);
@@ -490,6 +493,7 @@
     for (int blk = 0; blk < NKB; ++blk) kprev[blk] = nanv;
     int n_prev = -1;
     bool tables_ok = false;
+    int64_t redo_head = -1;
 
     while (it >= 0) {
         double* outb = p.out + b * (int64_t)mT * mK;
@@ -649,10 +653,15 @@
             if (p.status && lane == 0) p.status[b] = IVS_ST_OK;
         } else if (lane == 0) {
             reinterpret_cast<unsigned long long*>(outb)[0] = D_SENTINEL;
+            if (INL_K && p.inline_redo) reinterpret_cast<int*>(outb)[2] = (int)redo_head;
             count_redo(p, told);
         }
+        if (INL_K && !ok) redo_head = b;
         const int64_t it_next2 = wq.finish(pend, more);
         it = it_next; it_next = it_next2; b = b_next; n = n_next; koff = koff_next;
+    }
+    if constexpr (INL_K) {
+        if (p.inline_redo) masked_redo_any<METHOD>(p, smem, !mqf, redo_head);
     }
 #ifdef IVS_PASS_ENDSTAMP
     if (threadIdx.x == 0 && d_pass_ends) d_pass_ends[blockIdx.x * 2 + 1] = wall_clock64();
@@ -662,9 +671,9 @@
 template <int METHOD, int NKB, bool VAR>
 inline void launch_pass_nt(bool nt16, int64_t grid, size_t lds, hipStream_t st, const SurfaceParams& p, const VarList& list) {
     if constexpr (VAR) {
-        if (nt16) { hipLaunchKernelGGL((surface_pass_kernel<METHOD, NKB, true, true, true>), dim3((unsigned)grid), dim3(64), lds, st, p, list); return; }
-    }
-    hipLaunchKernelGGL((surface_pass_kernel<METHOD, NKB, VAR, true, false>), dim3((unsigned)grid), dim3(64), lds, st, p, list);
+        if (nt16) { IVS_LAUNCH((surface_pass_kernel<METHOD, NKB, true, true, true>), dim3((unsigned)grid), dim3(64), lds, st, p, list); return; }
+    }
+    IVS_LAUNCH((surface_pass_kernel<METHOD, NKB, VAR, true, false>), dim3((unsigned)grid), dim3(64), lds, st, p, list);
 }
 inline int launch_surface_pass(const SurfaceParams& p_in, const LaunchCtx& cx, const char** name) {
     SurfaceParams p = p_in;
@@ -680,6 +689,10 @@
     if (p.k_off && p.B > 0x7fffffffLL) return 0;
     const bool fixed64 = !p.k_off && p.nK == DK && p.nT == DT && !(reinterpret_cast<uintptr_t>(p.sigma) & 15);
     const bool nt16 = p.nT == DT;
+    p.inline_redo = fixed64 && tsh && pass_inline_redo(p.method) && (int64_t)p.mT * p.mK >= 2 && p.B <= 0x7fffffffLL ? 1 : 0;
+#ifdef IVS_DIAG_MINIMAL
+    p.inline_redo = 0;
+#endif
     if (!(fixed64 || nt16 ? launch_tq_or_zero_queue<false>(p, cx, tsh, fixed64)
                           : launch_tq_or_zero_queue<true>(p, cx, tsh, fixed64))) return -1;
     auto grid_for = [&](size_t lds, int64_t work, int wg_cap = 12) {
@@ -713,17 +726,18 @@
         const size_t lds = pass_lds_bytes<NKB_, 0>();                                                                                    \
         const int64_t grid = grid_for(lds, p.B, CAP);                                                                                    \
         if (!(VAR_)) p.map_groups = dense_map_groups(grid, p.B, cx.map_groups);                                                          \
-        hipLaunchKernelGGL((surface_pass_kernel<IVS_CUBIC, NKB_, VAR_>), dim3((unsigned)grid), dim3(64), lds, st, p, LIST);              \
+        IVS_LAUNCH((surface_pass_kernel<IVS_CUBIC, NKB_, VAR_>), dim3((unsigned)grid), dim3(64), lds, st, p, LIST);              \
     }
 #else
 #define IVS_PASS_LAUNCH(NKB_, VAR_, CAP, LIST)                                                                                           \
     {                                                                                                                                    \
         size_t lds = lerp ? pass_lds_bytes<NKB_, 1>() : (local ? pass_lds_bytes<NKB_, 2>() : pass_lds_bytes<NKB_, 0>());                 \
         if (!tsh) lds += PASS_TQ_DOUBLES * 8;                                                                                            \
+        if (!(VAR_) && p.inline_redo && lds < masked_any_lds_bytes(lerp)) lds = masked_any_lds_bytes(lerp);            \
         const int64_t grid = grid_for(lds, p.B, (local && (VAR_) && !nt16) ? 8 : (CAP));                      \
         if (!(VAR_)) p.map_groups = dense_map_groups(grid, p.B, cx.map_groups);                                                          \
         if (!tsh) {                                                                                                                      \
-            hipLaunchKernelGGL((surface_pass_kernel<IVS_LINEAR, NKB_, VAR_, false>), dim3((unsigned)grid), dim3(64), lds, st, p, LIST);  \
+            IVS_LAUNCH((surface_pass_kernel<IVS_LINEAR, NKB_, VAR_, false>), dim3((unsigned)grid), dim3(64), lds, st, p, LIST);  \
         } else                                                                                                                           \
         switch (p.method) {                                                                                                              \
             case IVS_CUBIC: launch_pass_nt<IVS_CUBIC, NKB_, VAR_>(nt16, grid, lds, st, p, LIST); break;                                  \
@@ -752,7 +766,7 @@
 #undef IVS_PASS_LAUNCH
     if (hipGetLastError() != hipSuccess) return -1;
 #ifndef IVS_DIAG_MINIMAL
-    if (fixed64 && launch_surface_masked(p, cx) && p.redo) ++p.redo;
+    if (fixed64 && (p.inline_redo || launch_surface_masked(p, cx)) && p.redo) ++p.redo;
 #endif
     launch_surface_generic<true>(p, cx);
     return 1;
```

Result: no change. 325.2 million (median of 2 runs) (+0.1%).
